# liuyuan-pal/Gen6D

Hardware: AMD Instinct MI355X
Metric: query images/sec (detect+select+3x refine), 64 ref views (higher is better)
Workload: dtype f32

## Files before the change

gen6d_amd/csrc/conv16_direct.hip:

```cpp
#include "g6d_common.h"
#include "conv16w_geom.h"
#include <type_traits>

namespace {

constexpr int C16_BM = 128, C16_BN = 128, C16_BK = 64;
constexpr int C16_STAGE = (C16_BM + C16_BN) * C16_BK * 2;
constexpr int C16_LDS = 2 * C16_STAGE;
constexpr int C16_EP_LD = 68;
constexpr unsigned C16_OOB = 0x80000000u;

struct C16Seg : c16g::Tiling {
  const char* in; char* full; char* pool;
  int H, W, DH;
  int rows;
  int ld_in, ld_full, ld_pool;
  int tw_log2, tiles_x, tile0;
  unsigned in_bytes;
  int back;
};
struct C16Params {
  C16Seg seg[4];
  int nseg, Cin, Cout, kd, D, relu, full_type, pool_type;
  const char* w; unsigned w_bytes; const float* bias;
// ... 383 lines not shown
    const int g = g0 + (r >> tw_log2), x = x0 + (r & (TW - 1));
    unsigned m = 0;
    if (g < sg.rows && x < W) {
      const int y = g % H, z = (g / H) % D;
      unsigned my = (y > 0 ? 1u : 0u) | 2u | (y < H - 1 ? 4u : 0u);
      unsigned mx = (x > 0 ? 1u : 0u) | 2u | (x < W - 1 ? 4u : 0u);
      unsigned m9 = 0;
#pragma unroll
      for (int ky = 0; ky < 3; ++ky) if (my >> ky & 1) m9 |= mx << (3 * ky);
      if (p.kd == 3) {
        if (z > 0) m |= m9;
        m |= m9 << 9;
        if (z < D - 1) m |= m9 << 18;
      } else m = m9;
    }
    a_mask[i] = m;
    a_off[i] = (unsigned)(((long)g * W + x) * sg.ld_in * 2) + slot * 16;
  }
  const __amdgpu_buffer_rsrc_t rs_in = c16_rsrc(sg.in - sg.back, sg.in_bytes);
  typedef __attribute__((address_space(3))) void* lds_ptr;
  const int nchunk = p.Cin / R::BK, nk = nchunk * ntaps;
  const int plane_bytes = p.Cin * 2;

  auto issue_a = [&](int k, int stage) {
    const int c = k / ntaps, tap = k - c * ntaps;
    const int kz = tap / 9, r9 = tap - 9 * kz, ky = r9 / 3, kx = r9 - 3 * ky;
    const unsigned a_k = (unsigned)(((kz * H + ky) * W + kx) * sg.ld_in * 2 + c * (R::BK * 2));
    char* sa = lds + stage * R::STAGE;
#pragma unroll
    for (int i = 0; i < 4; ++i) {
      const int ri = i % NR, pl = i / NR;
      const unsigned vo = (a_mask[ri] >> tap & 1u) ? a_off[ri] + a_k + pl * plane_bytes : C16_OOB;
      __builtin_amdgcn_raw_ptr_buffer_load_lds(rs_in, (lds_ptr)(sa + pl * (C16_BM * R::ROWB) + (32 * wv + R::RPI * ri) * R::ROWB), 16, vo, 0, 0, 0);
    }
  };
  const int wm = wv >> 1, wn = wv & 1;
  constexpr int NB = R::KS * R::NP * 2;
  constexpr int STEP_B = R::KS * R::NP * 4 * 1024;
  const char* wtile = p.w + (long)nt * nk * STEP_B;
  const unsigned b_voff = (2 * wn) * 1024 + lane * 16;
  auto load_b = [&](int k, V8 (&b)[NB]) {
    const char* ws = wtile + (long)k * STEP_B;
#pragma unroll
    for (int q = 0; q < R::KS * R::NP; ++q) {
      const char* wq = ws + q * 4096;
      asm volatile("global_load_dwordx4 %0, %1, %2" : "=v"(b[2 * q]) : "v"(b_voff), "s"(wq) : "memory");
      asm volatile("global_load_dwordx4 %0, %1, %2 offset:1024" : "=v"(b[2 * q + 1]) : "v"(b_voff), "s"(wq) : "memory");
    }
  };

  f32x16 acc[2][2];
#pragma unroll
  for (int a = 0; a < 2; ++a)
#pragma unroll
    for (int b = 0; b < 2; ++b)
#pragma unroll
      for (int r = 0; r < 16; ++r) acc[a][b][r] = 0.f;
  const int frow = lane & 31, fhalf = lane >> 5;
  const int fsw = R::SL == 8 ? (frow >> 1) & 7 : (frow >> 2) & 3;
  const int a_rd = (64 * wm + frow) * R::ROWB;

  auto compute = [&](int stage, const V8 (&b)[NB]) {
    const char* st = lds + stage * R::STAGE;
#pragma unroll
    for (int ks = 0; ks < R::KS; ++ks) {
      const int sl = ((2 * ks + fhalf) ^ fsw) * 16;
      V8 a[R::NP][2];
#pragma unroll
      for (int pl = 0; pl < R::NP; ++pl) {
        a[pl][0] = *reinterpret_cast<const V8*>(st + pl * (C16_BM * R::ROWB) + a_rd + sl);
        a[pl][1] = *reinterpret_cast<const V8*>(st + pl * (C16_BM * R::ROWB) + a_rd + 32 * R::ROWB + sl);
      }
#pragma unroll
      for (int mt = 0; mt < 2; ++mt)
#pragma unroll
        for (int n2 = 0; n2 < 2; ++n2) {
          acc[mt][n2] = c16_mfma<MM>(a[0][mt], b[(ks * R::NP) * 2 + n2], acc[mt][n2]);
          if constexpr (MM == 3) {
            acc[mt][n2] = c16_mfma<MM>(a[0][mt], b[(ks * R::NP + 1) * 2 + n2], acc[mt][n2]);
            acc[mt][n2] = c16_mfma<MM>(a[1][mt], b[(ks * R::NP) * 2 + n2], acc[mt][n2]);
          }
        }
    }
  };

  static_assert(NSTAGE == 3, "the stage arithmetic below assumes three stages");
  V8 b0[NB], b1[NB];
  load_b(0, b0);
  issue_a(0, 0);
  if (nk > 1) { issue_a(1, 1); asm volatile("s_waitcnt vmcnt(4)" ::: "memory"); }
  else asm volatile("s_waitcnt vmcnt(0)" ::: "memory");
  __builtin_amdgcn_s_barrier();
  __builtin_amdgcn_sched_barrier(0);
  int stage = 0;
  auto step = [&](int k, const V8 (&bc)[NB], V8 (&bn)[NB]) {
    if (k + 1 < nk && !((p.ablate & 2) && k > 1)) load_b(k + 1, bn);
    const int s2 = stage >= 1 ? stage - 1 : 2;
    if (k + 2 < nk && !((p.ablate & 1) && k > 1)) issue_a(k + 2, s2);
    compute(stage, bc);
    if (k + 2 < nk && !p.ablate) asm volatile("s_waitcnt vmcnt(4)" ::: "memory");
    else asm volatile("s_waitcnt vmcnt(0)" ::: "memory");
    asm volatile("s_waitcnt lgkmcnt(0)" ::: "memory");
    __builtin_amdgcn_s_barrier();
    __builtin_amdgcn_sched_barrier(0);
    stage = stage == 2 ? 0 : stage + 1;
  };
#pragma unroll 1
  for (int k = 0; k < nk; k += 2) {
    step(k, b0, b1);
    if (k + 1 < nk) step(k + 1, b1, b0);
  }
  c16_epilogue<MM == 3 ? 2 : MM>(p, sg, lds, tid, nt, g0, x0, tw_log2, C16_BM >> tw_log2,
                                 [&](int h, float* ep, int cbase) { c16_write22(p, acc, lane, wv, h, ep, cbase); });
}


#ifndef C16W_ABLATE
#define C16W_ABLATE 0
#endif
template <int MM> struct C16W {
  static constexpr int NP = MM == 3 ? 2 : 1, KS = 2, NI_MAX = 18;
  static constexpr int PLANE = NI_MAX * 1024;
  static constexpr int NT2 = MM == 3 ? 1 : 2;
  static constexpr int NBL = KS * NP * NT2;
  static constexpr int NPX = 64;
  static constexpr int EPW = NPX * C16_EP_LD * 4;
};

struct C16Geom {
  int si, ni;
  c16g::Tile t;
};
__device__ __forceinline__ C16Geom c16w_geom(const C16Params& p, int ptile) {
  C16Geom o;
  int si = 0;
#pragma unroll
  for (int i = 1; i < 4; ++i) if (i < p.nseg && ptile >= p.seg[i].h_tile0) si = i;
  const C16Seg& sg = p.seg[si];
  o.si = si; o.ni = (sg.h_P + 15) >> 4;
  o.t = c16g::tile_of(sg, sg.H, sg.W, ptile - sg.h_tile0);
  return o;
}

template <int BASE, int HI>
__device__ __forceinline__ void c16_wait_vm(int n) {
  if constexpr (HI == 0) {
    asm volatile("s_waitcnt vmcnt(%0)" ::"n"(BASE) : "memory");
  } else {
    if (n >= HI) asm volatile("s_waitcnt vmcnt(%0)" ::"n"(BASE + HI) : "memory");
    else c16_wait_vm<BASE, HI - 1>(n);
  }
}

template <int MM, int WM, int NT2 = C16W<MM>::NT2>
__global__ __launch_bounds__(256, 2) void conv16w_kernel(const C16Params p) {
  typedef typename C16T3<MM>::V V8;
  typedef C16W<MM> R;
  constexpr int WN = 4 / WM, NP = R::NP, KS = R::KS, NBL = KS * NP * NT2, CW = 32 * NT2;
  constexpr bool SINGLE = MM == 3 && WM == 2;
  constexpr int TILE_B = NP * R::PLANE, STAGE = WM * TILE_B;
  extern __shared__ __attribute__((aligned(16))) char lds[];
  const int tid = threadIdx.x, lane = tid & 63, wv = __builtin_amdgcn_readfirstlane(tid >> 6);
  const int xcd = blockIdx.x & 7, jj = blockIdx.x >> 3;
  const int cb = jj % p.nN, tg = (jj / p.nN) * 8 + xcd;
  if (tg * WM >= p.ptiles) return;
  const int wm = wv / WN, wn = wv % WN;
  const int nchunk = p.Cin >> 5;
  typedef __attribute__((address_space(3))) void* lds_ptr;

  constexpr int NPJ = (R::NI_MAX + 3) / 4;
  unsigned poff[WM][NPJ], pmask[WM];
  C16Geom gms[WM];
#pragma unroll
  for (int tl = 0; tl < WM; ++tl) {
    gms[tl] = c16w_geom(p, min(tg * WM + tl, p.ptiles - 1));
    const C16Geom& gm = gms[tl];
    const C16Seg& sg = p.seg[gm.si];
    const unsigned base = c16g::tile_base(sg.W, sg.ld_in, gm.t);
    unsigned pm = 0;
    if (gm.t.interior) {
#pragma unroll
      for (int j = 0; j < NPJ; ++j) {
        const c16g::Piece pc = c16g::piece_of(sg, wv + 4 * j, lane);
        poff[tl][j] = pc.in_patch ? c16g::piece_offset(sg, sg.W, sg.ld_in, base, pc) : C16_OOB;
        if (wv + 4 * j < gm.ni) pm |= 1u << j;
      }
    } else {
#pragma unroll
      for (int j = 0; j < NPJ; ++j) {
        const int ii = wv + 4 * j;
        const c16g::Piece pc = c16g::piece_of(sg, ii, lane);
        const bool ok = c16g::piece_valid(sg, sg.H, sg.W, sg.rows, gm.t, pc);
        poff[tl][j] = ok ? c16g::piece_offset(sg, sg.W, sg.ld_in, base, pc) : C16_OOB;
        if (ii < gm.ni) {
          if (__builtin_amdgcn_ballot_w64(ok) != 0) pm |= 1u << j;
          else {
            const f32x4 z = {0.f, 0.f, 0.f, 0.f};
#pragma unroll
            for (int pl = 0; pl < NP; ++pl) {
              char* dst = lds + tl * TILE_B + pl * R::PLANE + ii * 1024 + lane * 16;
              *reinterpret_cast<f32x4*>(dst) = z;
              if constexpr (!SINGLE) *reinterpret_cast<f32x4*>(dst + STAGE) = z;
            }
          }
        }
      }
    }
    pmask[tl] = __builtin_amdgcn_readfirstlane(pm);
  }
  const unsigned plane_b = (unsigned)(p.Cin * 2);
  auto issue_patch = [&](int c, int stage) {
    if (c >= nchunk) return;
    const unsigned ck = (unsigned)(c * 64);
#pragma unroll
    for (int tl = 0; tl < WM; ++tl) {
      const C16Seg& sg = p.seg[gms[tl].si];
      const __amdgpu_buffer_rsrc_t rs_in = c16_rsrc(sg.in, sg.in_bytes - sg.back);
#pragma unroll
      for (int j = 0; j < NPJ; ++j) {
        if (pmask[tl] >> j & 1) {
          const unsigned vo = poff[tl][j] == C16_OOB ? C16_OOB : poff[tl][j] + ck;
#pragma unroll
          for (int pl = 0; pl < NP; ++pl)
            __builtin_amdgcn_raw_ptr_buffer_load_lds(rs_in, (lds_ptr)(lds + stage * STAGE + tl * TILE_B + pl * R::PLANE + (wv + 4 * j) * 1024), 16,
                                                     vo + pl * plane_b, 0, 0, 0);
        }
      }
    }
  };
  const C16Geom gm = WM == 1 ? gms[0] : gms[wm ? WM - 1 : 0];
  const C16Seg& sgw = p.seg[gm.si];
  const int f_tw_log2 = sgw.h_tw_log2, f_PW = (1 << f_tw_log2) + 2;

  const int chan0 = (cb * WN + wn) * CW;
  const int nkp = (MM == 3 ? nchunk : nchunk >> 1) * 9;
  const char* wtile = p.w + (long)(chan0 >> 7) * nkp * 16384;
  unsigned bvo[KS * NP];
  if constexpr (MM == 3) {
#pragma unroll
    for (int q = 0; q < KS * NP; ++q)
      bvo[q] = ((lane >> 5) * NP + q % NP) * 4096 + ((chan0 >> 5) & 3) * 1024 + (32 * ((lane >> 4) & 1) + 16 * (q / NP) + (lane & 15)) * 16;
  } else {
#pragma unroll
    for (int q = 0; q < KS * NP; ++q) bvo[q] = q * 4096 + ((chan0 >> 5) & 3) * 1024 + lane * 16;
  }
  const char* wp = wtile;
  int wleft = nchunk * 9;
  auto load_b = [&](int c, int t, V8 (&b)[NBL]) {
    const unsigned long wa = (unsigned long)(wleft > 0 ? wp : wtile);
    const char* ws = reinterpret_cast<const char*>((unsigned long)(unsigned)__builtin_amdgcn_readfirstlane((unsigned)wa) |
                                                   ((unsigned long)(unsigned)__builtin_amdgcn_readfirstlane((unsigned)(wa >> 32)) << 32));
#pragma unroll
    for (int q = 0; q < KS * NP; ++q) {
      asm volatile("global_load_dwordx4 %0, %1, %2" : "=v"(b[NT2 * q]) : "v"(bvo[q]), "s"(ws) : "memory");
      if constexpr (NT2 == 2) asm volatile("global_load_dwordx4 %0, %1, %2 offset:1024" : "=v"(b[NT2 * q + 1]) : "v"(bvo[q]), "s"(ws) : "memory");
    }
    --wleft;
    if (t < 8 || MM == 3) wp += 16384;
    else wp += (c & 1) ? 8192 : 8192 - 8 * 16384;
  };

  if constexpr (MM == 3) {
    int qb[8], xs[3];
#pragma unroll
    for (int mt = 0; mt < 8; ++mt) qb[mt] = c16g::frag_pixel(sgw, 16 * mt + (lane & 15)) * 64 + wm * TILE_B;
#pragma unroll
    for (int kx = 0; kx < 3; ++kx) xs[kx] = ((lane >> 4) ^ ((((lane & 15 & ((1 << f_tw_log2) - 1)) + kx) >> sgw.h_swa) & 3)) << 4;
    const int PW64 = f_PW * 64;
    auto tap_off = [&](int t, int stg) { return xs[t % 3] + (stg * STAGE + (t / 3) * PW64 + (t % 3) * 64); };
    auto read_pair = [&](int mp, int off, V8 (&a)[2][NP]) {
#pragma unroll
      for (int i = 0; i < 2; ++i) {
        const int addr = qb[2 * mp + i] + off;
#pragma unroll
        for (int pl = 0; pl < NP; ++pl) a[i][pl] = *reinterpret_cast<const V8*>(lds + pl * R::PLANE + addr);
      }
    };
    f32x4 acc[8][2];
#pragma unroll
    for (int a = 0; a < 8; ++a)
#pragma unroll
      for (int b = 0; b < 2; ++b)
#pragma unroll
        for (int r = 0; r < 4; ++r) acc[a][b][r] = 0.f;
    auto mfmas = [&](int mp, const V8 (&a)[2][NP], const V8 (&b)[NBL]) {
#pragma unroll
      for (int term = 0; term < 3; ++term) {
        const int pa = term == 2 ? 1 : 0, pb = term == 1 ? 1 : 0;
#pragma unroll
        for (int n2 = 0; n2 < 2; ++n2)
#pragma unroll
          for (int i = 0; i < 2; ++i)
            acc[2 * mp + i][n2] = __builtin_amdgcn_mfma_f32_16x16x32_f16(a[i][pa], b[n2 * NP + pb], acc[2 * mp + i][n2], 0, 0, 0);
      }
    };

    V8 bs[3][NBL];
    V8 fa[3][2][NP];
    issue_patch(0, 0);
    load_b(0, 0, bs[0]);
    load_b(0, 1, bs[1]);
    asm volatile("s_waitcnt vmcnt(0) lgkmcnt(0)" ::: "memory");
    __builtin_amdgcn_s_barrier();
    __builtin_amdgcn_sched_barrier(0);
#pragma unroll
    for (int mp = 0; mp < 3; ++mp) read_pair(mp, tap_off(0, 0), fa[mp]);
    int stage = 0;
#pragma unroll 1
    for (int c = 0; c < ((C16W_ABLATE & 8) ? 0 : nchunk); ++c) {
#pragma unroll
      for (int mt = 0; mt < 8; ++mt) asm volatile("" : "+v"(qb[mt]));
#pragma unroll
      for (int kx = 0; kx < 3; ++kx) asm volatile("" : "+v"(xs[kx]));
#pragma unroll
      for (int t = 0; t < 9; ++t) {
        const int t2 = (t + 2) % 9, c2 = c + (t + 2) / 9;
        if (!((C16W_ABLATE & 2) && c > 0)) load_b(c2, t2, bs[(t + 2) % 3]);
        if (t == 0 && !SINGLE && !((C16W_ABLATE & 1) && c > 0)) issue_patch(c + 1, stage ^ 1);
        if (C16W_ABLATE) asm volatile("s_waitcnt vmcnt(0)" ::: "memory");
        else asm volatile("s_waitcnt vmcnt(%0)" ::"n"(2 * NBL) : "memory");
        __builtin_amdgcn_sched_barrier(0);
        const int off = tap_off(t, stage), noff = tap_off(t < 8 ? t + 1 : 0, stage);
#pragma unroll
        for (int mp = 0; mp < 4; ++mp) {
          const int g = 4 * t + mp, gn = g + 3;
          mfmas(mp, fa[g % 3], bs[t % 3]);
          if (gn < 36 && !((C16W_ABLATE & 4) && c > 0)) read_pair(gn % 4, gn / 4 == t ? off : noff, fa[g % 3]);
          __builtin_amdgcn_sched_barrier(0);
        }
        if (t == 8) {
          asm volatile("s_waitcnt vmcnt(0) lgkmcnt(0)" ::: "memory");
          __builtin_amdgcn_s_barrier();
          __builtin_amdgcn_sched_barrier(0);
          if constexpr (SINGLE) {
            issue_patch(c + 1, 0);
            asm volatile("s_waitcnt vmcnt(0)" ::: "memory");
            __builtin_amdgcn_s_barrier();
            __builtin_amdgcn_sched_barrier(0);
          } else stage ^= 1;
          if (c + 1 < nchunk) {
#pragma unroll
            for (int mp = 0; mp < 3; ++mp) read_pair(mp, tap_off(0, stage), fa[mp]);
          }
        }
      }
    }
    asm volatile("s_waitcnt vmcnt(0)" ::: "memory");
    __builtin_amdgcn_s_barrier();
    __builtin_amdgcn_sched_barrier(0);

    if (tg * WM + wm >= p.ptiles) return;
    const C16Seg& sg = p.seg[gm.si];
    float* ep = reinterpret_cast<float*>(lds + wv * R::EPW);
    float bv[2];
#pragma unroll
    for (int n2 = 0; n2 < 2; ++n2) bv[n2] = p.bias ? p.bias[chan0 + 16 * n2 + (lane & 15)] : 0.f;
    constexpr int MTP = R::NPX / 16;
    const float as = ldexpf(p.acc_scale, g6d_exp_in(p.rng));
    unsigned amax = 0;
    double wst[2] = {0.0, 0.0};
    const bool per_pass = c16w_stats_per_pass(p, sg, f_tw_log2);
    auto passes = [&](auto ftc, auto ptc, auto stc, auto spc) {
#pragma unroll
      for (int ps = 0; ps < 8 / MTP; ++ps) {
#pragma unroll
        for (int m = 0; m < MTP; ++m)
#pragma unroll
          for (int n2 = 0; n2 < 2; ++n2)
#pragma unroll
            for (int r = 0; r < 4; ++r) {
              const int px = 16 * m + 4 * (lane >> 4) + r;
              float v = fmaf(acc[ps * MTP + m][n2][r], as, bv[n2]);
              if (p.relu) v = fmaxf(v, 0.f);
              ep[px * C16_EP_LD + 16 * n2 + (lane & 15)] = v;
            }
        c16_epilogue_pass<2, 64, R::NPX, CW, decltype(ftc)::value, decltype(ptc)::value, decltype(stc)::value>(
            p, sg, ep, nullptr, lane, chan0, gm.t.g0, gm.t.x0, f_tw_log2, gm.t.ylim, ps * R::NPX, amax, wst);
        if (decltype(spc)::value > 0 || (decltype(spc)::value < 0 && per_pass))
          c16_stats_flush_pass<CW>(p, sg, lane, chan0, gm.t.g0 + ((ps * R::NPX) >> f_tw_log2), wst);
      }
    };
    typedef std::integral_constant<int, -1> any_;
    typedef std::integral_constant<int, 0> c0_;
    typedef std::integral_constant<int, 1> c1_;
    if (!p.stats && p.full_type == 3 && p.pool_type == 0) passes(std::integral_constant<int, 3>{}, c0_{}, c0_{}, c0_{});
    else if (!p.stats && p.full_type == 0 && p.pool_type == 3) passes(c0_{}, std::integral_constant<int, 3>{}, c0_{}, c0_{});
    else if (!p.stats && p.full_type == 3 && p.pool_type == 3) passes(std::integral_constant<int, 3>{}, std::integral_constant<int, 3>{}, c0_{}, c0_{});
    else if (p.stats && p.full_type == 2 && p.pool_type == 0 && !per_pass) passes(std::integral_constant<int, 2>{}, c0_{}, c1_{}, c0_{});
    else if (p.stats && p.full_type == 2 && p.pool_type == 0) passes(std::integral_constant<int, 2>{}, c0_{}, c1_{}, c1_{});
    else passes(any_{}, any_{}, any_{}, any_{});
    if (p.stats && !per_pass) c16_stats_flush<CW>(p, sg, lane, chan0, gm.t.g0, wst);
    g6d_range_record(p.rng, amax);
  } else {
    const int fhalf = lane >> 5;
    int qb[4], fe[4];
    const int PW64 = f_PW * 64, swa = sgw.h_swa, swd = sgw.h_swd;
#pragma unroll
    for (int mt = 0; mt < 4; ++mt) {
      const int r = 32 * mt + (lane & 31);
      qb[mt] = c16g::frag_pixel(sgw, r) * 64 + wm * TILE_B; fe[mt] = (r & ((1 << f_tw_log2) - 1)) + c16g::frag_row(sgw, r) * swd;
    }
    auto tap_addr = [&](int ky, int kx, int stage, int (&tb)[4]) {
      const int so = stage * STAGE + (ky * PW64 + kx * 64);
#pragma unroll
      for (int mt = 0; mt < 4; ++mt) {
        const int sw = ((fe[mt] + kx) >> swa) + ky * swd;
        tb[mt] = qb[mt] + so + (((fhalf ^ sw) & 3) << 4);
      }
    };
    auto frag_read = [&](int addr, V8 (&a)[NP]) {
#pragma unroll
      for (int pl = 0; pl < NP; ++pl) a[pl] = *reinterpret_cast<const V8*>(lds + pl * R::PLANE + addr);
    };
    f32x16 acc[4][NT2];
#pragma unroll
    for (int a = 0; a < 4; ++a)
#pragma unroll
      for (int b = 0; b < NT2; ++b)
#pragma unroll
        for (int r = 0; r < 16; ++r) acc[a][b][r] = 0.f;
    auto mfmas = [&](int mt, const V8 (&a)[NP], const V8 (&b)[NBL], int ks) {
#pragma unroll
      for (int n2 = 0; n2 < NT2; ++n2) acc[mt][n2] = c16_mfma<MM>(a[0], b[ks * NT2 + n2], acc[mt][n2]);
    };

    V8 bs[3][NBL];
    V8 fa[4][NP];
    int tb[4], ntb[4];
    issue_patch(0, 0);
    load_b(0, 0, bs[0]);
    load_b(0, 1, bs[1]);
    asm volatile("s_waitcnt vmcnt(0) lgkmcnt(0)" ::: "memory");
    __builtin_amdgcn_s_barrier();
    __builtin_amdgcn_sched_barrier(0);
    tap_addr(0, 0, 0, tb);
#pragma unroll
    for (int mt = 0; mt < 4; ++mt) frag_read(tb[mt], fa[mt]);
    int stage = 0;
#pragma unroll 1
    for (int c = 0; c < ((C16W_ABLATE & 8) ? 0 : nchunk); ++c) {
#pragma unroll
      for (int mt = 0; mt < 4; ++mt) asm volatile("" : "+v"(fe[mt]), "+v"(qb[mt]));
#pragma unroll
      for (int t = 0; t < 9; ++t) {
        const int t2 = (t + 2) % 9, c2 = c + (t + 2) / 9;
        if (!((C16W_ABLATE & 2) && c > 0)) load_b(c2, t2, bs[(t + 2) % 3]);
        if (t == 0 && !((C16W_ABLATE & 1) && c > 0)) issue_patch(c + 1, stage ^ 1);
        if (C16W_ABLATE) asm volatile("s_waitcnt vmcnt(0)" ::: "memory");
        else asm volatile("s_waitcnt vmcnt(%0)" ::"n"(2 * NBL) : "memory");
        __builtin_amdgcn_sched_barrier(0);
        if (t < 8) tap_addr((t + 1) / 3, (t + 1) % 3, stage, ntb);
        else tap_addr(0, 0, stage ^ 1, ntb);
#pragma unroll
        for (int mt = 0; mt < 4; ++mt) {
          mfmas(mt, fa[mt], bs[t % 3], 0);
          if (!((C16W_ABLATE & 4) && c > 0)) frag_read(tb[mt] ^ 32, fa[mt]);
          __builtin_amdgcn_sched_barrier(0);
        }
#pragma unroll
        for (int mt = 0; mt < 4; ++mt) {
          mfmas(mt, fa[mt], bs[t % 3], 1);
          if (t < 8 && !((C16W_ABLATE & 4) && c > 0)) frag_read(ntb[mt], fa[mt]);
          __builtin_amdgcn_sched_barrier(0);
        }
#pragma unroll
        for (int mt = 0; mt < 4; ++mt) tb[mt] = ntb[mt];
        if (t == 8) {
          asm volatile("s_waitcnt vmcnt(0) lgkmcnt(0)" ::: "memory");
          __builtin_amdgcn_s_barrier();
          __builtin_amdgcn_sched_barrier(0);
          stage ^= 1;
          if (c + 1 < nchunk) {
#pragma unroll
            for (int mt = 0; mt < 4; ++mt) frag_read(tb[mt], fa[mt]);
          }
        }
      }
    }
    asm volatile("s_waitcnt vmcnt(0)" ::: "memory");
    __builtin_amdgcn_s_barrier();
    __builtin_amdgcn_sched_barrier(0);

    if (tg * WM + wm >= p.ptiles) return;
    const C16Seg& sg = p.seg[gm.si];
    float* ep = reinterpret_cast<float*>(lds + wv * R::EPW);
    float bv[NT2];
#pragma unroll
    for (int n2 = 0; n2 < NT2; ++n2) bv[n2] = p.bias ? p.bias[chan0 + 32 * n2 + (lane & 31)] : 0.f;
    constexpr int MTP = R::NPX / 32;
    const float as = ldexpf(p.acc_scale, g6d_exp_in(p.rng));
    unsigned amax = 0;
    double wst[2] = {0.0, 0.0};
    const bool per_pass = c16w_stats_per_pass(p, sg, f_tw_log2);
// ... 317 lines not shown
        }
    };
    issue_patch(0, 0);
    asm volatile("s_waitcnt vmcnt(0)" ::: "memory");
    __builtin_amdgcn_s_barrier();
#pragma unroll 1
    for (int c = 0; c < nslice; ++c) {
      if (c + 1 < nslice) issue_patch(c + 1, (c + 1) & 1);
      asm volatile("s_waitcnt vmcnt(0)" ::: "memory");
      __builtin_amdgcn_s_barrier();
    }
  } else {
  const int T = K * K;
  const int ntw = (T - wv + NW - 1) / NW;
  const char* wp = p.w + (long)wv * 2048;
  int wtap = wv, wleft = nslice * ntw;
  const unsigned bvo = lane * 16;
  auto load_b = [&](V8 (&b)[2]) {
    const unsigned long wa = (unsigned long)(wleft > 0 ? wp : p.w);
    const char* ws = reinterpret_cast<const char*>((unsigned long)(unsigned)__builtin_amdgcn_readfirstlane((unsigned)wa) |
                                                   ((unsigned long)(unsigned)__builtin_amdgcn_readfirstlane((unsigned)(wa >> 32)) << 32));
    asm volatile("global_load_dwordx4 %0, %1, %2" : "=v"(b[0]) : "v"(bvo), "s"(ws) : "memory");
    asm volatile("global_load_dwordx4 %0, %1, %2 offset:1024" : "=v"(b[1]) : "v"(bvo), "s"(ws) : "memory");
    --wleft;
    wtap += NW;
    if (wtap < T) wp += NW * 2048;
    else { wp += (long)(T - wtap + NW + wv) * 2048; wtap = wv; }
  };

  const int fhalf = lane >> 5;
  int qb[4], fe[4];
#pragma unroll
  for (int mt = 0; mt < 4; ++mt) {
    const int r = 32 * mt + (lane & 31), py = r >> tw_log2, px = r & (TW - 1);
    qb[mt] = (py * PW + px) * 64; fe[mt] = px + py * swd;
  }
  const int PW64 = PW * 64;
  auto tap_addr = [&](int ky, int kx, int stage, int (&tb)[4]) {
    const int so = stage * CORR16_STAGE + ky * PW64 + kx * 64;
#pragma unroll
    for (int mt = 0; mt < 4; ++mt) {
      const int sw = ((fe[mt] + kx) >> swa) + ky * swd;
      tb[mt] = qb[mt] + so + (((fhalf ^ sw) & 3) << 4);
    }
  };
  V8 bs[3][2];
  V8 fa[4][2];
  int tb[4], ntb[4];
  load_b(bs[0]);
  load_b(bs[1]);
  asm volatile("s_waitcnt vmcnt(0)" ::: "memory");
  __builtin_amdgcn_s_barrier();
  __builtin_amdgcn_sched_barrier(0);
  const int ky0 = wv / K, kx0 = wv - ky0 * K;
  int ky = ky0, kx = kx0;
  tap_addr(ky, kx, 0, tb);
#pragma unroll
  for (int mt = 0; mt < 4; ++mt) {
    fa[mt][0] = *reinterpret_cast<const V8*>(lds + tb[mt]);
    fa[mt][1] = *reinterpret_cast<const V8*>(lds + (tb[mt] ^ 32));
  }
  int stage = 0, it = 0, c = 0;
  auto step = [&](const V8 (&bc)[2], V8 (&bfar)[2]) {
    const bool live = c < nslice, last = it == ntw - 1;
    load_b(bfar);
    asm volatile("s_waitcnt vmcnt(4)" ::: "memory");
    __builtin_amdgcn_sched_barrier(0);
    if (!live) return;
    int nky = ky, nkx = kx + NW;
    while (nkx >= K) { nkx -= K; ++nky; }
    if (last) { nky = ky0; nkx = kx0; }
    tap_addr(nky, nkx, last ? stage ^ 1 : stage, ntb);
#pragma unroll
    for (int mt = 0; mt < 4; ++mt) {
      if constexpr (MM == 3) {
        acc[mt] = c16_mfma<MM>(fa[mt][0], bc[0], acc[mt]);
        acc[mt] = c16_mfma<MM>(fa[mt][0], bc[1], acc[mt]);
        acc[mt] = c16_mfma<MM>(fa[mt][1], bc[0], acc[mt]);
      } else {
        acc[mt] = c16_mfma<MM>(fa[mt][0], bc[0], acc[mt]);
        acc[mt] = c16_mfma<MM>(fa[mt][1], bc[1], acc[mt]);
      }
      if (!last) {
        fa[mt][0] = *reinterpret_cast<const V8*>(lds + ntb[mt]);
        fa[mt][1] = *reinterpret_cast<const V8*>(lds + (ntb[mt] ^ 32));
      }
      __builtin_amdgcn_sched_barrier(0);
    }
    ky = nky; kx = nkx;
#pragma unroll
    for (int mt = 0; mt < 4; ++mt) tb[mt] = ntb[mt];
    ++it;
    if (last) {
      asm volatile("s_waitcnt lgkmcnt(0)" ::: "memory");
      __builtin_amdgcn_s_barrier();
      __builtin_amdgcn_sched_barrier(0);
      stage ^= 1; it = 0; ++c;
      if (c < nslice) {
#pragma unroll
        for (int mt = 0; mt < 4; ++mt) {
          fa[mt][0] = *reinterpret_cast<const V8*>(lds + tb[mt]);
          fa[mt][1] = *reinterpret_cast<const V8*>(lds + (tb[mt] ^ 32));
        }
      }
    }
  };
  const int nsteps = nslice * ntw;
#pragma unroll 1
  for (int s_ = 0; s_ < nsteps; s_ += 3) {
    asm volatile("" : "+v"(fe[0]), "+v"(fe[1]), "+v"(fe[2]), "+v"(fe[3]));
    step(bs[0], bs[2]);
    step(bs[1], bs[0]);
    step(bs[2], bs[1]);
  }
  asm volatile("s_waitcnt vmcnt(0)" ::: "memory");
  }
  __builtin_amdgcn_s_barrier();
  __builtin_amdgcn_sched_barrier(0);

  float* red = reinterpret_cast<float*>(lds);
  float sum[8];
#pragma unroll
  for (int e = 0; e < 8; ++e) sum[e] = 0.f;
#pragma unroll 1
  for (int rd = 0; rd < (NW + 3) / 4; ++rd) {
    if (wv < NW && (wv >> 2) == rd) {
      float* mine = red + (wv & 3) * (128 * 33);
#pragma unroll
      for (int mt = 0; mt < 4; ++mt)
#pragma unroll
        for (int r = 0; r < 16; ++r) mine[(32 * mt + (r & 3) + 8 * (r >> 2) + 4 * (lane >> 5)) * 33 + (lane & 31)] = acc[mt][r];
    }
    __syncthreads();
    if (wv < 8)
#pragma unroll
    for (int e = 0; e < 8; ++e) {
      const int o = tid + 512 * e, px = o >> 5, ch = o & 31;
      const int ns = NW - 4 * rd < 4 ? NW - 4 * rd : 4;
      for (int sl = 0; sl < ns; ++sl) sum[e] += red[sl * 128 * 33 + px * 33 + ch];
    }
    __syncthreads();
  }
  const float as = ldexpf(p.acc_scale, g6d_exp_in(p.rng));
  if (wv < 8)
#pragma unroll
  for (int e = 0; e < 8; ++e) {
    const int o = tid + 512 * e, px = o >> 5, ch = o & 31;
    const int y = y0 + (px >> tw_log2), x = x0 + (px & (TW - 1));
    if (y < sg.H && x < sg.W) sg.out[(((long)n * sg.H + y) * sg.W + x) * sg.ld_out + ch] = sum[e] * as;
  }
}


bool c16_halo_tiling(const G6dConv16Seg& s, C16Seg& o, int& tiles, bool pairs) {
  double best = 1e30;
  bool found = false;
  for (int tw = 32; tw >= 4; tw >>= 1) {
    const int th = C16_BM / tw, tx = (s.W + tw - 1) / tw;
    long nt; int tpi, segh, bands;
    if (s.H >= th) { tpi = tx * ((s.H + th - 1) / th); nt = (long)s.N * tpi; segh = th; bands = 1; }
    else {
      if (th % s.H) continue;
      tpi = 0; nt = (long)tx * (((long)s.N * s.H + th - 1) / th); segh = s.H; bands = th / s.H;
    }
    if (bands * (segh + 2) * (tw + 2) > 288) continue;
    const double waste = (double)nt * C16_BM / ((double)s.N * s.H * s.W);
    if (waste < best - 1e-9) {
      best = waste; found = true;
      int l2 = 0; while ((1 << l2) < tw) ++l2;
      int sl2 = 0; while ((1 << sl2) < segh) ++sl2;
      o.h_tw_log2 = l2; o.h_tiles_x = tx; o.h_tpi = tpi; o.h_segh_log2 = sl2; o.h_bands = bands;
      tiles = (int)nt;
      if (pairs) { o.h_swa = tw >= 16 ? 1 : 0; o.h_swd = 0; }
      else { o.h_swa = tw == 32 ? 2 : (tw == 16 ? 1 : 0); o.h_swd = tw <= 8 ? 1 : 0; }
    }
  }
  return found && c16g::finish(o, tiles);
}

int c16_pick_tw(int W, int pool) {
  int best = 8; double bw = 1e9;
  for (int tw = 64; tw >= (pool ? 4 : 4); tw >>= 1) {
    const double waste = (double)((W + tw - 1) / tw * tw) / W;
    if (waste < bw - 1e-9) { bw = waste; best = tw; }
  }
  return best;
}

}

namespace {
int c16_direct(const G6dConv16Seg* segs, int nseg, int Cin, const void* W16, int w_layout, float acc_scale, const float* bias, int Cout, int kd, int relu,
               int full_type, int pool_type, int math_mode, double* stats, int stat_rows_per_group, const G6dRange16* range, g6d_stream_t stream,
               bool plan_only) {
  if (!segs || nseg < 1 || nseg > 4 || !W16) { g6d_set_error("conv16_direct: 1..4 segments and filters expected"); return G6D_EINVAL; }
  if (math_mode < 1 || math_mode > 3 || (w_layout != 0 && w_layout != 1) || (math_mode == 3 && w_layout != 1)) {
    g6d_set_error("conv16_direct: math_mode 1 (bf16) / 2 (fp16) / 3 (fp16 hi-lo pairs, fragment-major filters only)"); return G6D_EINVAL;
  }
  const int bk = math_mode == 3 ? 32 : C16_BK, planes = math_mode == 3 ? 2 : 1;
  const bool half_tile = Cout == 64 && w_layout == 1 && kd == 1;
  if (Cin % bk || (Cout % C16_BN && !half_tile) || (kd != 1 && kd != 3)) { g6d_set_error("conv16_direct: Cin % 64 (32 for pairs), Cout % 128 (64: fragment-major 2-D layers), kd in {1,3} expected"); return G6D_EINVAL; }
  const int t16 = math_mode == 3 ? 3 : 1;
  auto type_ok = [&](int t) { return t == 0 || t == 2 || t == t16; };
  if (!type_ok(full_type) || !type_ok(pool_type) || (!full_type && !pool_type && !stats)) { g6d_set_error("conv16_direct: output types"); return G6D_EINVAL; }
  if (pool_type && kd != 1) { g6d_set_error("conv16_direct: pooling is 2-D only"); return G6D_EINVAL; }
  C16Params p = {};
  p.nseg = nseg; p.Cin = Cin; p.Cout = Cout; p.kd = kd; p.relu = relu; p.full_type = full_type; p.pool_type = pool_type;
  p.w = static_cast<const char*>(W16); p.bias = bias; p.stats = stats; p.stat_rows_per_group = stat_rows_per_group;
  p.acc_scale = acc_scale != 0.f ? acc_scale : 1.f;
  p.ablate = (int)g6d_knob(G6D_KNOB_C16_ABLATE);
  if (range) p.rng = *range;
  const long wb = (long)(half_tile ? 128 : Cout) * 9 * kd * Cin * 2 * planes;
  if (wb >= (1L << 31)) { g6d_set_error("conv16_direct: filters beyond 2 GB"); return G6D_EINVAL; }
  p.w_bytes = (unsigned)wb;
  p.nN = Cout / C16_BN;
  int tiles = 0, D0 = segs[0].D;
  bool pertap_stats_ok = true;
  for (int i = 0; i < nseg; ++i) {
    const G6dConv16Seg& s = segs[i];
    C16Seg& o = p.seg[i];
    if (!s.in || s.N < 1 || s.D < 1 || s.H < 1 || s.W < 1 || s.ld_in < planes * Cin || s.D != D0 || (kd == 1 && s.D != 1)) { g6d_set_error("conv16_direct: bad segment"); return G6D_EINVAL; }
    const int need_full = full_type == 3 ? 2 * Cout : Cout, need_pool = pool_type == 3 ? 2 * Cout : Cout;
    if ((full_type && (!s.out_full || s.ld_full < need_full)) || (pool_type && (!s.out_pool || s.ld_pool < need_pool || (s.H & 1) || (s.W & 1)))) {
      g6d_set_error("conv16_direct: outputs missing / odd map with pooling"); return G6D_EINVAL;
    }
    if (!g6d_aligned16(s.in) || (s.ld_in & 7) || (full_type && (!g6d_aligned16(s.out_full) || (s.ld_full & 7))) || (pool_type && (!g6d_aligned16(s.out_pool) || (s.ld_pool & 7)))) {
      g6d_set_error("conv16_direct: 16-byte aligned rows expected"); return G6D_EINVAL;
    }
    if (32L * s.W * (s.ld_full > s.ld_pool ? s.ld_full : s.ld_pool) * 4 >= (1L << 32)) { g6d_set_error("conv16_direct: 32 output rows beyond 4 GB"); return G6D_EINVAL; }
    o.in = static_cast<const char*>(s.in); o.full = static_cast<char*>(s.out_full); o.pool = static_cast<char*>(s.out_pool);
    o.H = s.H; o.W = s.W; o.DH = s.D * s.H; o.rows = s.N * s.D * s.H;
    o.ld_in = s.ld_in; o.ld_full = s.ld_full; o.ld_pool = s.ld_pool;
    const int tw = c16_pick_tw(s.W, pool_type != 0);
    int l2 = 0; while ((1 << l2) < tw) ++l2;
    o.tw_log2 = l2; o.tiles_x = (s.W + tw - 1) / tw; o.tile0 = tiles;
    const int th = C16_BM / tw;
    if (stats && stat_rows_per_group > 0 && ((long)stat_rows_per_group % ((long)th * s.W) != 0)) pertap_stats_ok = false;
    tiles += o.tiles_x * ((o.rows + th - 1) / th);
    const long back = ((long)(kd == 3 ? s.H * s.W : 0) + s.W + 1) * s.ld_in * 2;
    const long ext = (long)o.rows * s.W * s.ld_in * 2 + back;
    if (ext >= (1L << 31)) { g6d_set_error("conv16_direct: a segment's input beyond 2 GB"); return G6D_EINVAL; }
    o.back = (int)back; o.in_bytes = (unsigned)ext;
  }
  p.D = D0;
  p.ptiles = tiles;
  hipStream_t st = static_cast<hipStream_t>(stream);
  if (w_layout == 1 && kd == 1 && g6d_knob(G6D_KNOB_CONV16_HALO) != 0) {
    bool ok = true, per_pass = false;
    int htiles = 0;
    for (int i = 0; i < nseg && ok; ++i) {
      int nt_ = 0;
      ok = c16_halo_tiling(segs[i], p.seg[i], nt_, math_mode == 3);
      p.seg[i].h_tile0 = htiles; htiles += nt_;
      if (stats && stat_rows_per_group > 0 && ok) {
        const C16Seg& o = p.seg[i];
        const int th = C16_BM >> o.h_tw_log2;
        const long tile_px = (long)th * segs[i].W, pass_px = (long)(C16W<3>::NPX >> o.h_tw_log2) * segs[i].W;
        static_assert(C16W<1>::NPX == C16W<3>::NPX && C16W<2>::NPX == C16W<3>::NPX, "one pass size in every mode");
        ok = (stat_rows_per_group % (segs[i].H * segs[i].W) == 0) &&
             (o.h_tpi > 0 || stat_rows_per_group % tile_px == 0 || (stat_rows_per_group < tile_px && stat_rows_per_group % pass_px == 0));
        per_pass = per_pass || (ok && stat_rows_per_group < tile_px);
      }
    }
    if (!ok && half_tile) { g6d_set_error("conv16_direct: Cout = 64 needs a halo tiling for every segment"); return G6D_EINVAL; }
    if (ok) {
      const int cw = half_tile ? 32 : 32 * (math_mode == 3 ? C16W<3>::NT2 : C16W<2>::NT2);
      const int wm = Cout % (4 * cw) == 0 ? 1 : 2;
      p.ptiles = htiles;
      p.nN = Cout / (cw * (4 / wm));
      if (plan_only) return per_pass ? 2 : 1;
      const int hblocks = ((htiles + wm - 1) / wm + 7) / 8 * 8 * p.nN;
      auto launch = [&](auto kern, int main_lds, int ep_lds) {
        const int bytes = main_lds > ep_lds ? main_lds : ep_lds;
        g6d_allow_lds(reinterpret_cast<const void*>(kern), bytes);
        hipLaunchKernelGGL(kern, dim3(hblocks), dim3(256), bytes, st, p);
      };
#define C16W_LAUNCH(MM_, WM_) launch(&conv16w_kernel<MM_, WM_>, ((MM_ == 3 && WM_ == 2) ? 1 : 2) * WM_ * C16W<MM_>::NP * C16W<MM_>::PLANE, 4 * C16W<MM_>::EPW)
      if (half_tile && math_mode != 3) {
        if (math_mode == 1) launch(&conv16w_kernel<1, 2, 1>, 2 * 2 * C16W<1>::PLANE, 4 * C16W<1>::EPW);
        else launch(&conv16w_kernel<2, 2, 1>, 2 * 2 * C16W<2>::PLANE, 4 * C16W<2>::EPW);
      }
      else if (math_mode == 1) { if (wm == 1) C16W_LAUNCH(1, 1); else C16W_LAUNCH(1, 2); }
      else if (math_mode == 2) { if (wm == 1) C16W_LAUNCH(2, 1); else C16W_LAUNCH(2, 2); }
      else { if (wm == 1) C16W_LAUNCH(3, 1); else C16W_LAUNCH(3, 2); }
#undef C16W_LAUNCH
      return g6d_check_launch("conv16w_direct");
    }
  }
  if (half_tile) { g6d_set_error("conv16_direct: Cout = 64 runs on the halo-patch kernel only (knob conv16_halo, tile shapes)"); return G6D_EINVAL; }
  if (!pertap_stats_ok) { g6d_set_error("conv16_direct: statistics groups must be whole tile rows (small maps: whole 64-pixel epilogue passes)"); return G6D_EINVAL; }
  if (plan_only) return 0;
  const int blocks = (tiles + 7) / 8 * 8 * p.nN;
  if (w_layout == 0) {
    if (math_mode == 1) {
      g6d_allow_lds(reinterpret_cast<const void*>(&conv16_kernel<1>), C16_LDS);
      hipLaunchKernelGGL(conv16_kernel<1>, dim3(blocks), dim3(256), C16_LDS, st, p);
    } else {
      g6d_allow_lds(reinterpret_cast<const void*>(&conv16_kernel<2>), C16_LDS);
      hipLaunchKernelGGL(conv16_kernel<2>, dim3(blocks), dim3(256), C16_LDS, st, p);
    }
    return g6d_check_launch("conv16_direct");
  }
  constexpr int NST = 3, LDSR = NST * 16384;
  if (math_mode == 1) {
    g6d_allow_lds(reinterpret_cast<const void*>(&conv16r_kernel<1, NST>), LDSR);
    hipLaunchKernelGGL((conv16r_kernel<1, NST>), dim3(blocks), dim3(256), LDSR, st, p);
  } else if (math_mode == 2) {
    g6d_allow_lds(reinterpret_cast<const void*>(&conv16r_kernel<2, NST>), LDSR);
    hipLaunchKernelGGL((conv16r_kernel<2, NST>), dim3(blocks), dim3(256), LDSR, st, p);
  } else {
    g6d_allow_lds(reinterpret_cast<const void*>(&conv16r_kernel<3, NST>), LDSR);
    hipLaunchKernelGGL((conv16r_kernel<3, NST>), dim3(blocks), dim3(256), LDSR, st, p);
  }
  return g6d_check_launch("conv16r_direct");
}
}

extern "C" int g6d_conv16_direct_multi_ex(const G6dConv16Seg* segs, int nseg, int Cin, const void* W16, int w_layout, float acc_scale,
                                          const float* bias, int Cout, int kd, int relu, int full_type, int pool_type, int math_mode, double* stats,
                                          int stat_rows_per_group, const G6dRange16* range, g6d_stream_t stream) {
  return c16_direct(segs, nseg, Cin, W16, w_layout, acc_scale, bias, Cout, kd, relu, full_type, pool_type, math_mode, stats, stat_rows_per_group, range,
                    stream, false);
}

extern "C" int g6d_conv16_direct_plan(const G6dConv16Seg* segs, int nseg, int Cin, const void* W16, int w_layout, int Cout, int kd, int full_type,
                                      int pool_type, int math_mode, double* stats, int stat_rows_per_group) {
  return c16_direct(segs, nseg, Cin, W16, w_layout, 1.f, nullptr, Cout, kd, 0, full_type, pool_type, math_mode, stats, stat_rows_per_group, nullptr,
                    nullptr, true);
}

extern "C" int g6d_conv16_direct_multi(const G6dConv16Seg* segs, int nseg, int Cin, const void* W16, int w_layout, float acc_scale,
                                       const float* bias, int Cout, int kd, int relu, int full_type, int pool_type, int math_mode, double* stats,
                                       int stat_rows_per_group, g6d_stream_t stream) {
  return g6d_conv16_direct_multi_ex(segs, nseg, Cin, W16, w_layout, acc_scale, bias, Cout, kd, relu, full_type, pool_type, math_mode, stats,
                                    stat_rows_per_group, nullptr, stream);
}

extern "C" int g6d_corr16_multi_ex(const G6dConv16Seg* segs, int nseg, int Cin, const void* W16, float acc_scale, int Cout, int k, int math_mode,
                                   const G6dRange16* range, g6d_stream_t stream) {
  if (!segs || nseg < 1 || nseg > 4 || !W16) { g6d_set_error("corr16: 1..4 segments and filters expected"); return G6D_EINVAL; }
  if (math_mode < 1 || math_mode > 3 || Cout != 32 || (k != 15 && k != 7) || Cin % 32) {
    g6d_set_error("corr16: math_mode 1 (bf16) / 2 (fp16) / 3 (fp16 pairs), Cout = 32, k in {7, 15}, Cin % 32 == 0 expected"); return G6D_EINVAL;
  }
  const int planes = math_mode == 3 ? 2 : 1;
  Corr16Params p = {};
  p.nseg = nseg; p.Cin = Cin; p.K = k; p.w = static_cast<const char*>(W16); p.acc_scale = acc_scale != 0.f ? acc_scale : 1.f;
  p.nslice = Cin / (math_mode == 3 ? 16 : 32);
  if (range) p.rng = *range;
  int tiles = 0;
  for (int i = 0; i < nseg; ++i) {
    const G6dConv16Seg& s = segs[i];
    Corr16Seg& o = p.seg[i];
    if (!s.in || !s.out_full || s.N < 1 || s.D != 1 || s.H < 1 || s.W < 1 || s.ld_in < planes * Cin || s.ld_full < Cout || (s.ld_in & 7) ||
        !g6d_aligned16(s.in) || !g6d_aligned16(s.out_full)) { g6d_set_error("corr16: bad segment"); return G6D_EINVAL; }
    double best = 1e30; int btw = 0;
    for (int tw = 32; tw >= 4; tw >>= 1) {
      const int th = C16_BM / tw;
      if ((th + k - 1) * (tw + k - 1) > CORR16_STAGE / 64) continue;
      const double waste = (double)((s.W + tw - 1) / tw * tw) * ((s.H + th - 1) / th * th) / ((double)s.W * s.H);
      if (waste < best - 1e-9) { best = waste; btw = tw; }
    }
    if (!btw) { g6d_set_error("corr16: no tile shape fits"); return G6D_EINVAL; }
    int l2 = 0; while ((1 << l2) < btw) ++l2;
    const int th = C16_BM / btw;
    o.in = static_cast<const char*>(s.in); o.out = static_cast<float*>(s.out_full);
    o.H = s.H; o.W = s.W; o.rows = s.N * s.H; o.ld_in = s.ld_in; o.ld_out = s.ld_full;
    o.tw_log2 = l2; o.tiles_x = (s.W + btw - 1) / btw; o.tpi = o.tiles_x * ((s.H + th - 1) / th); o.tile0 = tiles;
    o.swa = btw == 32 ? 2 : (btw == 16 ? 1 : 0); o.swd = btw <= 8 ? 1 : 0;
    const long ext = (long)s.N * s.H * s.W * s.ld_in * 2;
    if (ext >= (1L << 31)) { g6d_set_error("corr16: a segment's input beyond 2 GB"); return G6D_EINVAL; }
    o.in_bytes = (unsigned)ext;
    tiles += s.N * o.tpi;
  }
  p.ptiles = tiles;
  hipStream_t st = static_cast<hipStream_t>(stream);
  constexpr int LDSB = 2 * CORR16_STAGE;
  if (math_mode == 1) {
    g6d_allow_lds(reinterpret_cast<const void*>(&corr16_kernel<1>), LDSB);
    hipLaunchKernelGGL(corr16_kernel<1>, dim3(tiles), dim3(64 * (CORR16_NW + 1)), LDSB, st, p);
  } else if (math_mode == 2) {
    g6d_allow_lds(reinterpret_cast<const void*>(&corr16_kernel<2>), LDSB);
    hipLaunchKernelGGL(corr16_kernel<2>, dim3(tiles), dim3(64 * (CORR16_NW + 1)), LDSB, st, p);
  } else {
    g6d_allow_lds(reinterpret_cast<const void*>(&corr16_kernel<3>), LDSB);
    hipLaunchKernelGGL(corr16_kernel<3>, dim3(tiles), dim3(64 * (CORR16_NW + 1)), LDSB, st, p);
  }
  return g6d_check_launch("corr16");
}

extern "C" int g6d_corr16_multi(const G6dConv16Seg* segs, int nseg, int Cin, const void* W16, float acc_scale, int Cout, int k, int math_mode,
                                g6d_stream_t stream) {
  return g6d_corr16_multi_ex(segs, nseg, Cin, W16, acc_scale, Cout, k, math_mode, nullptr, stream);
}

extern "C" int g6d_product_split16_ex(const float* ref, const float* que, const float* scale, const float* shift, void* out, int qn, int D, int P,
                                      int C, int math_mode, const G6dRange16* range, g6d_stream_t stream) {
  if (!ref || !que || !scale || !shift || !out || qn < 1 || D < 1 || P < 1 || C < 8 || (C & 7) || math_mode < 1 || math_mode > 3 ||
      !g6d_aligned16(ref) || !g6d_aligned16(que) || !g6d_aligned16(scale) || !g6d_aligned16(shift) || !g6d_aligned16(out)) {
    g6d_set_error("product_split16: bad args (C % 8 == 0, 16-byte aligned pointers, math_mode 1..3)"); return G6D_EINVAL;
  }
  const long total = (long)qn * ((D + 7) / 8) * P * (C >> 3);
  const int blocks = (int)((total + 255) / 256 < 256 * 64 ? (total + 255) / 256 : 256 * 64);
  hipStream_t st = static_cast<hipStream_t>(stream);
  char* o = static_cast<char*>(out);
  const G6dRange16 rng = range ? *range : G6dRange16{};
  if (math_mode == 1) hipLaunchKernelGGL(product_split_kernel<1>, dim3(blocks), dim3(256), 0, st, ref, que, scale, shift, o, D, P, C, total, rng);
  else if (math_mode == 2) hipLaunchKernelGGL(product_split_kernel<2>, dim3(blocks), dim3(256), 0, st, ref, que, scale, shift, o, D, P, C, total, rng);
  else hipLaunchKernelGGL(product_split_kernel<3>, dim3(blocks), dim3(256), 0, st, ref, que, scale, shift, o, D, P, C, total, rng);
  return g6d_check_launch("product_split16");
}

extern "C" int g6d_product_split16(const float* ref, const float* que, const float* scale, const float* shift, void* out, int qn, int D, int P, int C,
                                   int math_mode, g6d_stream_t stream) {
  return g6d_product_split16_ex(ref, que, scale, shift, out, qn, D, P, C, math_mode, nullptr, stream);
}

namespace {
char* c16_slice_out(void* out, int C, int ld_out, int plane, int c_off, int math_mode) {
  const bool pairs = math_mode == 3;
  if (!out || !g6d_aligned16(out) || ((ld_out | plane | c_off) & 7) || c_off < 0 || ld_out < 1) return nullptr;
  if (pairs ? (plane < c_off + C || (long)plane + c_off + C > ld_out) : (c_off + C > ld_out)) return nullptr;
  return static_cast<char*>(out) + (long)c_off * 2;
}
}

extern "C" int g6d_affine_split16_to(const float* in, int ld_in, const float* scale, const float* shift, int affine_per_n, int relu, int pool, int N, int H,
                                     int W, int C, void* out, int ld_out, int plane, int c_off, int math_mode, const G6dRange16* range,
                                     g6d_stream_t stream) {
  if (!in || !out || N < 1 || H < 1 || W < 1 || C < 8 || (C & 7) || ld_in < C || (ld_in & 3) || (scale && !shift) || affine_per_n < 0 || math_mode < 1 ||
      math_mode > 3 || (pool && ((H | W) & 1)) || !g6d_aligned16(in) || !g6d_aligned16(out) || (scale && (!g6d_aligned16(scale) || !g6d_aligned16(shift)))) {
    g6d_set_error("affine_split16: bad args (C % 8 == 0, 16-byte aligned rows, even map with pooling, math_mode 1..3)"); return G6D_EINVAL;
  }
  char* o = c16_slice_out(out, C, ld_out, plane, c_off, math_mode);
  if (!o) { g6d_set_error("affine_split16: the channel slice does not fit the output rows (multiples of 8, c_off + C <= plane, plane + c_off + C <= ld_out)"); return G6D_EINVAL; }
  const long total = (long)N * (pool ? H / 2 : H) * (pool ? W / 2 : W) * (C >> 3);
  const int blocks = (int)((total + 255) / 256 < 256 * 64 ? (total + 255) / 256 : 256 * 64);
  hipStream_t st = static_cast<hipStream_t>(stream);
  const G6dRange16 rng = range ? *range : G6dRange16{};
  if (math_mode == 1) hipLaunchKernelGGL(affine_split16_kernel<1>, dim3(blocks), dim3(256), 0, st, in, ld_in, scale, shift, affine_per_n, relu, pool, H, W, C, o, ld_out, plane, total, rng);
  else if (math_mode == 2) hipLaunchKernelGGL(affine_split16_kernel<2>, dim3(blocks), dim3(256), 0, st, in, ld_in, scale, shift, affine_per_n, relu, pool, H, W, C, o, ld_out, plane, total, rng);
  else hipLaunchKernelGGL(affine_split16_kernel<3>, dim3(blocks), dim3(256), 0, st, in, ld_in, scale, shift, affine_per_n, relu, pool, H, W, C, o, ld_out, plane, total, rng);
// ... 50 lines not shown
```

gen6d_amd/csrc/conv16w_geom.h:

```cpp
#pragma once

#if defined(__HIPCC__)
#define C16G_HD __host__ __device__ __forceinline__
#else
#define C16G_HD inline
#endif

namespace c16g {

constexpr int BM = 128;
constexpr int NI_MAX = 18;

C16G_HD unsigned mulhi(unsigned a, unsigned b) {
#if defined(__HIP_DEVICE_COMPILE__)
  return __umulhi(a, b);
#else
  return (unsigned)(((unsigned long long)a * b) >> 32);
#endif
}

C16G_HD unsigned recip31(unsigned d) { return (unsigned)(((1ull << 31) + d - 1) / d); }
C16G_HD bool recip31_ok(unsigned d, unsigned n_max) {
  const unsigned long long e = (unsigned long long)recip31(d) * d - (1ull << 31);
  return n_max < (1u << 31) && (unsigned long long)n_max * e < (1ull << 31);
}
C16G_HD unsigned div31(unsigned n, unsigned m) { return mulhi(n << 1, m); }

C16G_HD unsigned recip16(unsigned d) { return (65536u + d - 1) / d; }
C16G_HD unsigned div16(unsigned n, unsigned m) { return (n * m) >> 16; }

struct Tiling {
  int h_tw_log2, h_tiles_x, h_tile0, h_tpi;
  int h_segh_log2, h_bands;
  int h_swa, h_swd;
  int h_P;
  unsigned h_r_tpi, h_r_tx;
  unsigned h_r_pw, h_r_band;
};

C16G_HD bool finish(Tiling& t, long ntiles) {
  const int TW = 1 << t.h_tw_log2, segh = 1 << t.h_segh_log2;
  t.h_P = t.h_bands * (segh + 2) * (TW + 2);
  t.h_r_pw = recip16((unsigned)(TW + 2)); t.h_r_band = recip16((unsigned)(segh + 2));
  t.h_r_tx = recip31((unsigned)t.h_tiles_x); t.h_r_tpi = t.h_tpi > 0 ? recip31((unsigned)t.h_tpi) : 0u;
  if (ntiles >= (1L << 31)) return false;
  return recip31_ok((unsigned)t.h_tiles_x, (unsigned)ntiles) && (t.h_tpi <= 0 || recip31_ok((unsigned)t.h_tpi, (unsigned)ntiles));
}

struct Tile {
  int g0, x0, y0, ylim;
  int interior;
};
C16G_HD Tile tile_of(const Tiling& tl, int H, int W, int t) {
  Tile o;
  const int TW = 1 << tl.h_tw_log2, TH = BM >> tl.h_tw_log2;
  if (tl.h_tpi > 0) {
    const int n = (int)div31((unsigned)t, tl.h_r_tpi), r = t - n * tl.h_tpi;
    const int ty = (int)div31((unsigned)r, tl.h_r_tx), tx = r - ty * tl.h_tiles_x;
    o.y0 = ty * TH; o.x0 = tx * TW; o.g0 = n * H + o.y0; o.ylim = TH < H - o.y0 ? TH : H - o.y0;
    o.interior = o.y0 >= 1 && o.y0 + TH < H && o.x0 >= 1 && o.x0 + TW < W;
  } else {
    const int ty = (int)div31((unsigned)t, tl.h_r_tx), tx = t - ty * tl.h_tiles_x;
    o.y0 = 0; o.x0 = tx * TW; o.g0 = ty * TH; o.ylim = TH;
    o.interior = 0;
  }
  return o;
}

struct Piece {
  int prow, pcol, band, lr, slot;
  int in_patch;
};
C16G_HD Piece piece_of(const Tiling& tl, int ii, int lane) {
  Piece o;
  const int PW = (1 << tl.h_tw_log2) + 2, bandr = (1 << tl.h_segh_log2) + 2;
  const int q = ii * 16 + (lane >> 2);
  o.prow = (int)div16((unsigned)q, tl.h_r_pw); o.pcol = q - o.prow * PW;
  o.band = (int)div16((unsigned)o.prow, tl.h_r_band); o.lr = o.prow - o.band * bandr - 1;
  o.slot = (lane & 3) ^ (((o.pcol >> tl.h_swa) + o.prow * tl.h_swd) & 3);
  o.in_patch = q < tl.h_P;
  return o;
}
C16G_HD bool piece_valid(const Tiling& tl, int H, int W, int rows, const Tile& t, const Piece& pc) {
  const int g = t.g0 + (pc.band << tl.h_segh_log2) + pc.lr, x = t.x0 + pc.pcol - 1, yimg = t.y0 + pc.lr;
  return pc.in_patch && yimg >= 0 && yimg < H && g < rows && x >= 0 && x < W;
}
C16G_HD unsigned tile_base(int W, int ld_in, const Tile& t) { return (unsigned)(((t.g0 - 1) * W + t.x0 - 1) * ld_in * 2); }
C16G_HD unsigned piece_offset(const Tiling& tl, int W, int ld_in, unsigned base, const Piece& pc) {
  const int yrel = (pc.band << tl.h_segh_log2) + pc.lr + 1;
  return base + (unsigned)((yrel * W + pc.pcol) * ld_in * 2 + pc.slot * 16);
}
C16G_HD int frag_pixel(const Tiling& tl, int r) {
  const int PW = (1 << tl.h_tw_log2) + 2, bandr = (1 << tl.h_segh_log2) + 2;
  const int py = r >> tl.h_tw_log2, px = r & ((1 << tl.h_tw_log2) - 1);
  const int b = py >> tl.h_segh_log2, ly = py & ((1 << tl.h_segh_log2) - 1);
  return (b * bandr + ly) * PW + px;
}
C16G_HD int frag_row(const Tiling& tl, int r) {
  const int py = r >> tl.h_tw_log2;
  return (py >> tl.h_segh_log2) * ((1 << tl.h_segh_log2) + 2) + (py & ((1 << tl.h_segh_log2) - 1));
}

}
```

gen6d_amd/csrc/refiner_volume.hip:

```cpp
#include "g6d_common.h"

#define MAX_RFN 8

namespace {


struct Taps { int o00, o01, o10, o11; float w00, w01, w10, w11; };

__device__ __forceinline__ Taps project_view(int fh, int fw, int C, const float (&P)[12], float vx, float vy,
                                             float vz, float h_in, float w_in) {
  float X = vx * P[0] + vy * P[1] + vz * P[2] + P[3];
  float Y = vx * P[4] + vy * P[5] + vz * P[6] + P[7];
  float Z = vx * P[8] + vy * P[9] + vz * P[10] + P[11];
  if (Z < 1e-4f) Z = 1e-4f;
  float u = X / Z, v = Y / Z;
  float gx = ((u + 0.5f) / w_in - 0.5f) * 2.f;
  float gy = ((v + 0.5f) / h_in - 0.5f) * 2.f;
  float ix = ((gx + 1.f) * fw - 1.f) * 0.5f;
  float iy = ((gy + 1.f) * fh - 1.f) * 0.5f;
  float fx = floorf(ix), fy = floorf(iy);
  fx = fminf(fmaxf(fx, -4.f), (float)fw + 4.f);
  fy = fminf(fmaxf(fy, -4.f), (float)fh + 4.f);
  int x0 = (int)fx, y0 = (int)fy;
  float wx1 = ix - fx, wy1 = iy - fy, wx0 = (fx + 1.f) - ix, wy0 = (fy + 1.f) - iy;
  const bool xv0 = (unsigned)x0 < (unsigned)fw, xv1 = (unsigned)(x0 + 1) < (unsigned)fw;
  const bool yv0 = (unsigned)y0 < (unsigned)fh, yv1 = (unsigned)(y0 + 1) < (unsigned)fh;
  const int xc0 = min(max(x0, 0), fw - 1), xc1 = min(max(x0 + 1, 0), fw - 1);
  const int yc0 = min(max(y0, 0), fh - 1), yc1 = min(max(y0 + 1, 0), fh - 1);
  Taps t;
  t.o00 = (yc0 * fw + xc0) * C; t.o01 = (yc0 * fw + xc1) * C;
  t.o10 = (yc1 * fw + xc0) * C; t.o11 = (yc1 * fw + xc1) * C;
  t.w00 = (yv0 && xv0) ? wx0 * wy0 : 0.f; t.w01 = (yv0 && xv1) ? wx1 * wy0 : 0.f;
  t.w10 = (yv1 && xv0) ? wx0 * wy1 : 0.f; t.w11 = (yv1 && xv1) ? wx1 * wy1 : 0.f;
  return t;
}

__device__ __forceinline__ Taps taps_from(const Taps& t, int src) {
  Taps r;
  r.o00 = __shfl(t.o00, src, 32); r.o01 = __shfl(t.o01, src, 32);
  r.o10 = __shfl(t.o10, src, 32); r.o11 = __shfl(t.o11, src, 32);
  r.w00 = __shfl(t.w00, src, 32); r.w01 = __shfl(t.w01, src, 32);
  r.w10 = __shfl(t.w10, src, 32); r.w11 = __shfl(t.w11, src, 32);
  return r;
}

__device__ __forceinline__ f32x4 gather_view(const float* __restrict__ fmap_c, const Taps& t) {
  const f32x4 v00 = *reinterpret_cast<const f32x4*>(fmap_c + t.o00);
  const f32x4 v01 = *reinterpret_cast<const f32x4*>(fmap_c + t.o01);
  const f32x4 v10 = *reinterpret_cast<const f32x4*>(fmap_c + t.o10);
  const f32x4 v11 = *reinterpret_cast<const f32x4*>(fmap_c + t.o11);
  f32x4 acc = t.w00 * v00;
  acc += t.w01 * v01;
  acc += t.w10 * v10;
  acc += t.w11 * v11;
  return acc;
}

struct VolViews { const float* projs; const float* ref_Ks; const float* ref_poses; const float* K_in; const float* pose_in;
                  const float* rot; int rot_ld; };

__global__ void __launch_bounds__(256, 4) refiner_volume_kernel(const float* __restrict__ feats, const VolViews vw,
                                                             const float* __restrict__ lin, int rfn, int fh, int fw,
                                                             int C, float h_in, float w_in, int sn,
                                                             float* __restrict__ mean_in, float* __restrict__ stdv) {
  const int bq = blockIdx.y;
  const float* __restrict__ rot = vw.rot + bq * 12;
  const int rl = vw.rot_ld;
  const int nvox = sn * sn * sn;
  feats += (size_t)bq * (rfn + 1) * fh * fw * C;
  mean_in += (size_t)bq * nvox * 2 * C; stdv += (size_t)bq * nvox * C;
  int half = (blockIdx.x * blockDim.x + threadIdx.x) >> 5;
  const int l32 = threadIdx.x & 31;
  const bool live = half < nvox;
  if (!live) half = nvox - 1;
  const int k = half % sn, j = (half / sn) % sn, i = half / (sn * sn);
  const float g0 = lin[i], g1 = lin[j], g2 = lin[k];
  const float vx = g0 * rot[0] + g1 * rot[rl] + g2 * rot[2 * rl];
  const float vy = g0 * rot[1] + g1 * rot[rl + 1] + g2 * rot[2 * rl + 1];
  const float vz = g0 * rot[2] + g1 * rot[rl + 2] + g2 * rot[2 * rl + 2];
  const size_t fsz = (size_t)fh * fw * C;
  const float inv_n = 1.f / (float)rfn, inv_n1 = 1.f / (float)(rfn > 1 ? rfn - 1 : 1);
  const int myview = l32 <= rfn ? l32 : rfn;
  float P[12];
  if (vw.projs) {
#pragma unroll
    for (int e = 0; e < 12; ++e) P[e] = vw.projs[myview * 12 + e];
  } else {
    const float* K = myview < rfn ? vw.ref_Ks + (bq * rfn + myview) * 9 : vw.K_in + bq * 9;
    const float* T = myview < rfn ? vw.ref_poses + (bq * rfn + myview) * 12 : vw.pose_in + bq * 12;
#pragma unroll
    for (int r = 0; r < 3; ++r)
#pragma unroll
      for (int c = 0; c < 4; ++c) P[r * 4 + c] = K[r * 3] * T[c] + K[r * 3 + 1] * T[4 + c] + K[r * 3 + 2] * T[8 + c];
  }
  const Taps mine = project_view(fh, fw, C, P, vx, vy, vz, h_in, w_in);
  for (int c0 = 0; c0 < C; c0 += 128) {
    const int c_mine = c0 + l32 * 4;
    const bool c_in = c_mine < C;
    const int c = c_in ? c_mine : C - 4;
    f32x4 s[MAX_RFN];
    f32x4 sum = {0.f, 0.f, 0.f, 0.f};
#pragma unroll
    for (int r = 0; r < MAX_RFN; ++r)
      if (r < rfn) { s[r] = gather_view(feats + r * fsz + c, taps_from(mine, r)); sum += s[r]; }
    const f32x4 mean = sum * inv_n;
    f32x4 var = {0.f, 0.f, 0.f, 0.f};
#pragma unroll
    for (int r = 0; r < MAX_RFN; ++r)
      if (r < rfn) { f32x4 d = s[r] - mean; var += d * d; }
    var = var * inv_n1;
    f32x4 sd = {sqrtf(var[0]), sqrtf(var[1]), sqrtf(var[2]), sqrtf(var[3])};
    const f32x4 q = gather_view(feats + rfn * fsz + c, taps_from(mine, rfn));
    if (!live || !c_in) continue;
    *reinterpret_cast<f32x4*>(mean_in + (size_t)half * 2 * C + c) = mean;
    *reinterpret_cast<f32x4*>(mean_in + (size_t)half * 2 * C + C + c) = q;
    *reinterpret_cast<f32x4*>(stdv + (size_t)half * C + c) = sd;
  }
}

}

extern "C" int g6d_refiner_volume(const float* feats, const float* projs, const float* rot_in,
                                  const float* lin, int rfn, int fh, int fw, int C, int h_in, int w_in, int sn,
                                  float* mean_in, float* stdv, g6d_stream_t stream) {
  if (!feats || !projs || !rot_in || !lin || !mean_in || !stdv || rfn < 1 || rfn > MAX_RFN || C < 4 || (C & 3) ||
      fh <= 0 || fw <= 0 || h_in <= 0 || w_in <= 0 || sn < 1 || sn > 256 || !g6d_aligned16(feats) || !g6d_aligned16(mean_in) ||
      !g6d_aligned16(stdv)) {
    g6d_set_error("refiner_volume: bad args (1 <= rfn <= 8, C a positive multiple of 4, positive map and image sizes)"); return G6D_EINVAL;
  }
  const long long threads = (long long)sn * sn * sn * 32;
  const VolViews vw = {projs, nullptr, nullptr, nullptr, nullptr, rot_in, 3};
  hipLaunchKernelGGL(refiner_volume_kernel, dim3((unsigned)((threads + 255) / 256)), dim3(256), 0,
                     reinterpret_cast<hipStream_t>(stream), feats, vw, lin, rfn, fh, fw, C, (float)h_in, (float)w_in, sn,
                     mean_in, stdv);
  return g6d_check_launch("refiner_volume");
}

extern "C" int g6d_refiner_volume_kp(const float* feats, const float* ref_Ks, const float* ref_poses, const float* K_in,
                                     const float* pose_in, const float* lin, int rfn, int fh, int fw, int C, int h_in, int w_in, int sn,
                                     float* mean_in, float* stdv, int batch, g6d_stream_t stream) {
  if (!feats || !ref_Ks || !ref_poses || !K_in || !pose_in || !lin || !mean_in || !stdv || rfn < 1 || rfn > MAX_RFN || C < 4 || (C & 3) ||
      fh <= 0 || fw <= 0 || h_in <= 0 || w_in <= 0 || sn < 1 || sn > 256 || batch < 1 || batch > 65535 || !g6d_aligned16(feats) ||
      !g6d_aligned16(mean_in) || !g6d_aligned16(stdv)) {
    g6d_set_error("refiner_volume_kp: bad args (1 <= rfn <= 8, C a positive multiple of 4, positive map and image sizes)"); return G6D_EINVAL;
  }
  const long long threads = (long long)sn * sn * sn * 32;
  const VolViews vw = {nullptr, ref_Ks, ref_poses, K_in, pose_in, pose_in, 4};
  hipLaunchKernelGGL(refiner_volume_kernel, dim3((unsigned)((threads + 255) / 256), batch), dim3(256), 0,
                     reinterpret_cast<hipStream_t>(stream), feats, vw, lin, rfn, fh, fw, C, (float)h_in, (float)w_in, sn,
                     mean_in, stdv);
  return g6d_check_launch("refiner_volume_kp");
}
```

gen6d_amd/lib.py:

```python
import ctypes as C
import os

_HERE = os.path.dirname(os.path.abspath(__file__))
LIB_PATH = os.path.join(_HERE, "libgen6d_hip.so")

G6D_ERRORS = {-1: "G6D_EINVAL", -2: "G6D_ENOSPC", -3: "G6D_ELAUNCH"}


class G6dWinoSeg(C.Structure):
    _fields_ = [("in_", C.c_void_p), ("out_full", C.c_void_p), ("out_pool", C.c_void_p),
                ("N", C.c_int32), ("H", C.c_int32), ("W", C.c_int32), ("ld_in", C.c_int32), ("ld_full", C.c_int32), ("ld_pool", C.c_int32)]


class G6dConv16Seg(C.Structure):
    _fields_ = [("in_", C.c_void_p), ("out_full", C.c_void_p), ("out_pool", C.c_void_p),
                ("N", C.c_int32), ("D", C.c_int32), ("H", C.c_int32), ("W", C.c_int32), ("ld_in", C.c_int32), ("ld_full", C.c_int32),
                ("ld_pool", C.c_int32)]


class G6dRange16(C.Structure):
    _fields_ = [("exps", C.c_void_p), ("rec", C.c_void_p), ("slot_in", C.c_int32), ("slot_out", C.c_int32)]


class G6dCorrSeg(C.Structure):
    _fields_ = [("in_", C.c_void_p), ("out", C.c_void_p), ("H", C.c_int32), ("W", C.c_int32), ("ld_in", C.c_int32), ("ld_out", C.c_int32),
                ("N", C.c_int32), ("reserved_", C.c_int32)]


class G6dFrame(C.Structure):
    _fields_ = [("plane0", C.c_void_p), ("plane1", C.c_void_p), ("pitch0", C.c_int32), ("pitch1", C.c_int32), ("width", C.c_int32),
                ("height", C.c_int32), ("format", C.c_int32), ("rotate", C.c_int32), ("matrix", C.c_int32), ("slot", C.c_int32),
                ("out_w", C.c_int32), ("out_h", C.c_int32), ("K", C.c_float * 9)]


class G6dMesh(C.Structure):
    _fields_ = [("nodes", C.c_void_p), ("nx", C.c_int32), ("ny", C.c_int32), ("step_log2", C.c_int32), ("reserved", C.c_int32)]


class G6dSink(C.Structure):
    _fields_ = [("plane0", C.c_void_p), ("plane1", C.c_void_p), ("pitch0", C.c_int32), ("pitch1", C.c_int32), ("width", C.c_int32),
                ("height", C.c_int32), ("format", C.c_int32), ("matrix", C.c_int32), ("slot", C.c_int32), ("pic_w", C.c_int32),
                ("pic_h", C.c_int32), ("thickness", C.c_int32), ("dot_radius", C.c_int32), ("line_rgb", C.c_int32), ("dot_rgb", C.c_int32),
                ("box", C.c_int32)]


class G6dConv(C.Structure):
    _fields_ = [
        ("in_", C.c_void_p), ("mul", C.c_void_p), ("in_scale", C.c_void_p), ("in_shift", C.c_void_p),
        ("weight", C.c_void_p), ("bias", C.c_void_p), ("out", C.c_void_p), ("stats", C.c_void_p),
        ("workspace", C.c_void_p), ("workspace_bytes", C.c_size_t),
        ("N", C.c_int32), ("Di", C.c_int32), ("Hi", C.c_int32), ("Wi", C.c_int32), ("Cin", C.c_int32), ("ld_in", C.c_int32),
        ("Do", C.c_int32), ("Ho", C.c_int32), ("Wo", C.c_int32), ("Cout", C.c_int32), ("ld_out", C.c_int32),
        ("kd", C.c_int32), ("kh", C.c_int32), ("kw", C.c_int32),
        ("sd", C.c_int32), ("sh", C.c_int32), ("sw", C.c_int32),
        ("pd", C.c_int32), ("ph", C.c_int32), ("pw", C.c_int32),
        ("in_relu", C.c_int32), ("in_affine_per_n", C.c_int32), ("out_act", C.c_int32),
        ("stat_rows_per_group", C.c_int32), ("split_k", C.c_int32), ("math_mode", C.c_int32),
        ("weight_wino", C.c_void_p),
        ("fin_scale", C.c_void_p), ("fin_shift", C.c_void_p), ("fin_counter", C.c_void_p),
        ("fin_count", C.c_double), ("fin_eps", C.c_double), ("fin_groups", C.c_int32),
        ("in_image_mod", C.c_int32), ("mul_group_images", C.c_int32), ("reserved_", C.c_int32),
        ("weight_wino16", C.c_void_p), ("weight_wino43", C.c_void_p),
    ]


_P, _I, _F, _D = C.c_void_p, C.c_int, C.c_float, C.c_double

SIGNATURES = {
    "g6d_marker": [_I, _P],
    "g6d_conv_igemm": [C.POINTER(G6dConv), _P],
    "g6d_conv_plan": [C.POINTER(G6dConv)],
    "g6d_corr2d_patch": [_P, _I, _I, _I, _I, _P, _I, _I, _I, _P, _I, _P, C.c_size_t, _I, _P],
    "g6d_corr2d_patch_multi": [_P, _I, _I, _P, _I, _I, _I, _P, C.c_size_t, _I, _P],
    "g6d_corr2d_wino_multi": [_P, _I, _I, _P, _I, _I, _P, C.c_size_t, _P],
    "g6d_corr2d_patch16_multi": [_P, _I, _I, _P, _I, _I, _I, _P, C.c_size_t, _I, _P],
    "g6d_stats_finalize": [_P, _I, _D, _D, _P, _P, _P],
    "g6d_affine_act_pool": [_P, _I, _P, _P, _I, _I, _I, _I, _I, _I, _I, _P, _I, _P],
    "g6d_upsample_bilinear": [_P, _I, _P, _P, _I, _I, _I, _I, _I, _I, _P, _I, _P],
    "g6d_bias_relu_pool_nchw": [_P, _P, _I, _I, _I, _I, _I, _I, _P, _P],
    "g6d_vgg_conv1_pool": [_P, _I, _I, _I, _P, _P, _I, _I, _P, _P],
    "g6d_vgg_conv1_pool_nhwc": [_P, _I, _I, _I, _P, _P, _I, _I, _P, _P],
    "g6d_vgg_conv1_pool_nhwc16": [_P, _I, _I, _I, _P, _P, _I, _I, _P, _P, _P, _I, _P],
    "g6d_conv16_direct_multi": [_P, _I, _I, _P, _I, _F, _P, _I, _I, _I, _I, _I, _I, _P, _I, _P],
    "g6d_corr16_multi": [_P, _I, _I, _P, _F, _I, _I, _I, _P],
    "g6d_product_split16": [_P, _P, _P, _P, _P, _I, _I, _I, _I, _I, _P],
    "g6d_affine_split16": [_P, _I, _P, _P, _I, _I, _I, _I, _I, _I, _I, _P, _I, _P],
    "g6d_vgg_conv1_pool_nhwc16_ex": [_P, _I, _I, _I, _P, _P, _I, _I, _P, _P, _P, _I, _P, _P],
    "g6d_conv16_direct_multi_ex": [_P, _I, _I, _P, _I, _F, _P, _I, _I, _I, _I, _I, _I, _P, _I, _P, _P],
    "g6d_corr16_multi_ex": [_P, _I, _I, _P, _F, _I, _I, _I, _P, _P],
    "g6d_product_split16_ex": [_P, _P, _P, _P, _P, _I, _I, _I, _I, _I, _P, _P],
    "g6d_affine_split16_ex": [_P, _I, _P, _P, _I, _I, _I, _I, _I, _I, _I, _P, _I, _P, _P],
    "g6d_conv16_direct_plan": [_P, _I, _I, _P, _I, _I, _I, _I, _I, _I, _P, _I],
    "g6d_affine_split16_to": [_P, _I, _P, _P, _I, _I, _I, _I, _I, _I, _I, _P, _I, _I, _I, _I, _P, _P],
    "g6d_upsample_bilinear_split16": [_P, _I, _P, _P, _I, _I, _I, _I, _I, _I, _P, _I, _I, _I, _I, _P, _P],
    "g6d_l2norm_split16": [_P, _I, _I, _I, _P, _I, _P, _P],
    "g6d_vgg_conv1_pool_nhwc_norm": [_P, _I, _I, _I, _P, _P, _I, _I, _P, _P, _P, _P],
    "g6d_wino_conv3x3": [_P, _I, _I, _I, _I, _I, _P, _P, _I, _I, _P, _I, _P, _I, _P, C.c_size_t, _P],
    "g6d_wino_conv3x3_multi": [_P, _I, _I, _P, _P, _I, _I, _P, C.c_size_t, _P],
    "g6d_wino16_conv3x3_multi": [_P, _I, _I, _P, _P, _I, _I, _I, _P, C.c_size_t, _P],
    "g6d_wino43_conv3x3_multi": [_P, _I, _I, _P, _P, _I, _I, _P, C.c_size_t, _P],
    "g6d_corr2d_wino43_multi": [_P, _I, _I, _P, _I, _I, _P, C.c_size_t, _P],
    "g6d_l2norm_rows": [_P, _I, _I, _I, _P],
    "g6d_nchw_to_nhwc": [_P, _I, _I, _I, _I, _I, _P, _I, _P],
    "g6d_selector_ref_sums": [_P, _I, _I, _I, _P, _P, _P],
    "g6d_selector_prod_affine": [_P, _P, _P, _I, _I, _I, _D, _P, _P, _P],
    "g6d_selector_scan": [_P, _P, _I, _I, _I, _P, _P, _P],
    "g6d_selector_levels": [_I, _I, _P, _P, _P, _P, _P, _I, _I, _I, _D, _P, _P, _P, _P, _P],
    "g6d_refiner_volume": [_P, _P, _P, _P, _I, _I, _I, _I, _I, _I, _I, _P, _P, _P],
    "g6d_refiner_volume_kp": [_P, _P, _P, _P, _P, _P, _I, _I, _I, _I, _I, _I, _I, _P, _P, _I, _P],
    "g6d_detector_assemble": [_P, _P, _P, _I, _I, _I, C.POINTER(C.c_float), _F, _I, _I, _I, _I, _P, _I, _P],
    "g6d_detector_score_mlp_max": [_P, _I, _I, _I, _P, _P, _P, _P, _P, _P],
    "g6d_detector_decode": [_P, _I, _P, _I, _P, _I, _I, _I, _I, _P, _I, _P],
    "g6d_resize_bilinear_pyramid": [_P, _I, _I, _I, _I, C.POINTER(C.c_int), C.POINTER(C.c_int), C.POINTER(C.c_void_p), _P],
    "g6d_zero_bytes": [_P, C.c_size_t, _P],
    "g6d_vps_norm": [_P, _I, _P, _I, _I, _I, _P],
    "g6d_max_an_add": [_P, _I, _I, _I, _I, _P, _P, _I, _I, _P],
    "g6d_attention": [_P, _P, _P, _I, _I, _I, _I, _P, _I, _I, _P],
    "g6d_layernorm": [_P, _I, _I, _I, _P, _P, _F, _P, _I, _P],
    "g6d_affine_act_add": [_P, _I, _P, _P, _I, _P, _I, _I, _I, _P, _I, _I, _P],
    "g6d_linear_gemv": [_P, _I, _I, _P, _P, _I, _I, _P, _P],
    "g6d_linear_gemv_batch": [_P, _I, _I, _P, _P, _I, _I, _P, _P, C.c_size_t, _P],
    "g6d_chain_crop_from_detection": [_P, _F, _P, _I, _P],
    "g6d_chain_pose_from_selection": [_P, _P, _P, _I, _P, _P, _P, _P, _P, _P, _I, _P],
    "g6d_chain_refine_prepare": [_P, _P, _P, _F, _F, _P, _P, _I, _I, _P, _P, _F, _P, _I, _P],
    "g6d_chain_refine_update": [_P, _P, _P, _P, _I, _P, _P, _I, _P],
    "g6d_warp_batch": [_P, _P, _P, _I, _I, _I, _I, _P, _P, _I, _I, _P],
    "g6d_warp_perspective": [_P, _I, _I, _I, C.POINTER(C.c_float), _P, _I, _I, _I, _F, _P],
    "g6d_track_gather": [_P, _P, _P, _P, _I, _P],
    "g6d_track_commit": [_P, _P, _P, _I, _P, _I, _F, _P, _P, _P, _P, _P, _I, _P],
    "g6d_track_gate": [_P, _P, _P, _P, _I, _P],
    "g6d_track_health": [_P, _P, _P, _P, _I, _I, _P, _I, _P, _D, _I, _D, _D, _D, _D, _D, _D, _P, _P, _P, _P, _I, _P],
    "g6d_track_verify": [_P, _P, _P, _P, _P, _D, _D, _D, _D, _I, _P, _P, _I, _P],
    "g6d_frame_ingest": [_P, _I, _P, _I, _I, _I, _P, _P],
    "g6d_sizeof_frame_desc": [],
    "g6d_frame_ingest_mesh": [_P, _P, _I, _P, _I, _I, _I, _P, _P],
    "g6d_sizeof_mesh_desc": [],
    "g6d_track_corners": [_P, _P, _P, _P, _P, _P, _I, _P],
    "g6d_frame_emit": [_P, _I, _P, _I, _I, _I, _P, _P, _P],
    "g6d_sizeof_sink_desc": [],
    "g6d_frame_emit_source": [_P, _I, _P, _I, _P, _P, _I, _I, _I, _I, _P],
}

_lib = None


def load():
    global _lib
    if _lib is not None:
        return _lib
    if not os.path.exists(LIB_PATH):
        raise RuntimeError(f"{LIB_PATH} is missing: build it with `python __graft_entry__.py` "
                           "(make -C gen6d_amd/csrc). There is no fallback path.")
    import torch
    lib = C.CDLL(LIB_PATH)
    for name, args in SIGNATURES.items():
        fn = getattr(lib, name)
        fn.argtypes = args
        fn.restype = C.c_int
    lib.g6d_abi_version.restype = C.c_int
    lib.g6d_sizeof_conv_desc.restype = C.c_int
    if lib.g6d_sizeof_conv_desc() != C.sizeof(G6dConv):
        raise RuntimeError("libgen6d_hip.so: G6dConv layout differs from the ctypes binding (stale build?)")
    if lib.g6d_sizeof_frame_desc() != C.sizeof(G6dFrame):
        raise RuntimeError("libgen6d_hip.so: G6dFrame layout differs from the ctypes binding (stale build?)")
    if lib.g6d_sizeof_mesh_desc() != C.sizeof(G6dMesh):
        raise RuntimeError("libgen6d_hip.so: G6dMesh layout differs from the ctypes binding (stale build?)")
    if lib.g6d_sizeof_sink_desc() != C.sizeof(G6dSink):
        raise RuntimeError("libgen6d_hip.so: G6dSink layout differs from the ctypes binding (stale build?)")
    lib.g6d_last_error.restype = C.c_char_p
    lib.g6d_set_knob.argtypes, lib.g6d_set_knob.restype = [C.c_char_p, C.c_double], C.c_int
    lib.g6d_get_knob.argtypes, lib.g6d_get_knob.restype = [C.c_char_p], C.c_double
    lib.g6d_reset_knobs.argtypes, lib.g6d_reset_knobs.restype = [], None
    _lib = lib
    return lib


def set_knob(name, value):
    check(load().g6d_set_knob(name.encode(), float(value)), f"g6d_set_knob({name})")


def get_knob(name):
    return load().g6d_get_knob(name.encode())


def reset_knobs():
    load().g6d_reset_knobs()


def check(rc, what):
    if rc != 0:
        msg = load().g6d_last_error().decode()
        raise RuntimeError(f"{what} failed: {G6D_ERRORS.get(rc, rc)} ({msg})")
```

gen6d_amd/network/params.py:

```python
import torch
import torch.nn as nn

from .. import ops, specs


class ConvW(tuple):

    def __new__(cls, w, b, u=None, u43=None):
        t = super().__new__(cls, (w, b))
        t.u, t.u43, t._w16 = u, u43, {}
        return t

    def w16(self, mode):
        if mode not in self._w16:
            self._w16[mode] = ops.conv16_pack(self[0], mode, layout=1)
        return self._w16[mode]


class ParamBank(nn.Module):
    def __init__(self, rows):
        super().__init__()
        self._roles = {}
        for key, shape, role in specs.expand(rows):
            *path, leaf = key.split(".")
            mod = self
            for name in path:
                if name not in mod._modules:
                    mod.add_module(name, nn.Module())
                mod = mod._modules[name]
            if role in ("weight", "bias", "gamma", "beta"):
                init = torch.ones(shape) if role == "gamma" else torch.zeros(shape)
                mod.register_parameter(leaf, nn.Parameter(init, requires_grad=False))
            elif role == "count":
                mod.register_buffer(leaf, torch.zeros((), dtype=torch.long))
            else:
                mod.register_buffer(leaf, torch.ones(shape) if role == "rvar" else torch.zeros(shape))
            self._roles[key] = role
        self._packed = None

    sharded = False

    def _reset_derived(self):
        self._packed = None
        self.__dict__.pop("_range_seen", None)
        t = self.__dict__.get("_range")
        if t is not None:
            t.reset()

    def load_state_dict(self, *a, **k):
        self._reset_derived()
        return super().load_state_dict(*a, **k)

    def _apply(self, fn, *a, **k):
        self._reset_derived()
        return super()._apply(fn, *a, **k)

    @property
    def pairs_on(self):
        return not (self.cfg.get("fp32_cores") or self.__dict__.get("_pairs_off", False))

    @property
    def range_fallbacks(self):
        return self.__dict__.get("_range_fallbacks", 0)

    def range_table(self):
        t = self.__dict__.get("_range")
        if t is None or t.device != self.device_():
            t = self._range = ops.RangeTable(self.device_())
        return t

    def _pair_rng(self):
        return self.range_table() if (self.pairs_on and not ops.MATH_MODE and self.device_().type == "cuda") else None

    def range_check(self):
        t = self.__dict__.get("_range")
        if t is None or not t.names:
            return False
        a = t.read()
        t.clear()
        self._range_seen = {n: max(v, self.__dict__.get("_range_seen", {}).get(n, 0.0)) if v == v else v for n, v in a.items()}
        bad = {n: v for n, v in a.items() if ops.pair_out_of_window(v, t.e[t.names[n]])}
        if not bad:
            return False
        if self.sharded:
            raise RuntimeError(f"{type(self).__name__}: fp16 pair maps left the representable window in the reference-sharded mode "
                               f"({', '.join(f'{n}: max |v| = {v:g}' for n, v in bad.items())}); a per-rank fp32 recompute would desynchronise "
                               "the collectives")
        t.set_exponents({n: ops.pair_exponent(v, t.e[t.names[n]]) for n, v in bad.items()})
        self._range_fallbacks = self.range_fallbacks + 1
        return True

    def range_guarded(self, fn):
        return range_guarded((self,), fn)

    def _range_fallback(self):
        """Hook: drop state derived from a call whose pair maps left the window (before its recompute)."""

    def range_report(self):
        t = self.__dict__.get("_range")
        if t is None:
            return {}
        seen = self.__dict__.get("_range_seen", {})
        return {n: {"A": seen.get(n, 0.0), "e": t.e[i]} for n, i in t.names.items()}

    def p(self, key):
        *path, leaf = key.split(".")
        mod = self
        for name in path:
            mod = mod._modules[name]
        t = mod._parameters.get(leaf)
        return (t if t is not None else mod._buffers[leaf]).detach()

    def device_(self):
        return next(self.parameters()).device

    def conv_w(self, prefix, cin_pad=None, wino_kd=0, f43=False):
        w = self.p(prefix + ".weight")
        co, ci = w.shape[:2]
        w = w.reshape(co, ci, -1).permute(0, 2, 1)
        if cin_pad is not None and cin_pad != ci:
            w = torch.nn.functional.pad(w, (0, cin_pad - ci))
        w = w.contiguous()
        u = u43 = None
        if wino_kd and ci % 8 == 0 and co % 32 == 0 and w.shape[1] == 9 * wino_kd:
            from .backbone import winograd_filters_taps, winograd43_filters_taps
            u = winograd_filters_taps(w, wino_kd)
            if f43 and co % 64 == 0:
                u43 = winograd43_filters_taps(w, wino_kd)
        return ConvW(w, self.p(prefix + ".bias").contiguous(), u, u43)


def fold_vgg(bank, prefix):
    out = []
    for i in specs.VGG11_BN_CONVS:
        w, b = bank.p(f"{prefix}.{i}.weight"), bank.p(f"{prefix}.{i}.bias")
        g, beta = bank.p(f"{prefix}.{i + 1}.weight"), bank.p(f"{prefix}.{i + 1}.bias")
        mu, var = bank.p(f"{prefix}.{i + 1}.running_mean"), bank.p(f"{prefix}.{i + 1}.running_var")
        s = g / torch.sqrt(var + 1e-5)
        out.append(((w * s.view(-1, 1, 1, 1)).contiguous(), ((b - mu) * s + beta).contiguous()))
    return out


def range_guarded(nets, fn, recompute=None):
    nets = [n for n in nets if n is not None]
    for n in nets:
        t = n.__dict__.get("_range")
        if t is not None and t.names:
            t.clear()
    out = fn()
    left = [n for n in nets if n.range_check()]
    if left:
        for n in left:
            n._range_fallback()
            n._pairs_off = True
        try:
            out = (recompute or fn)()
        finally:
            for n in left:
                n._pairs_off = False
    return out
```

gen6d_amd/network/refiner.py:

```python
import numpy as np
import torch
import torch.nn.functional as F

from .. import ops, specs
from .backbone import pack_trunk, trunk_features
from .operator import pose_apply_th
from .params import ParamBank, fold_vgg

F43_MIN_QUERIES = 4
FEATNET_F43_LAYERS = {("conv1", 0), ("conv_out", 0), ("conv_out", 3)}
FEATNET_PAIR_BRANCHES = ("conv0", "conv1", "conv2", "conv_out")
VOLUME_F43_LAYERS = ("conv0",)
MAX_BATCH = 32
_K3, _P3 = (3, 3, 3), (1, 1, 1)
_K2, _P2 = (1, 3, 3), (0, 1, 1)


_LIN = {}


def _linspace(sn, dev):
    key = (sn, str(dev))
    if key not in _LIN:
        _LIN[key] = torch.linspace(-1, 1, sn, dtype=torch.float32, device=dev)
    return _LIN[key]


class RefFeatureCache:

    def __init__(self, max_entries=2048):
        from collections import OrderedDict
        self.store, self.max_entries = OrderedDict(), max_entries
        self.hits = self.misses = 0

    def get(self, key):
        f = self.store.get(key)
        if f is None:
            self.misses += 1
            return None
        self.store.move_to_end(key)
        self.hits += 1
        return f

    def put(self, key, feat):
        self.store[key] = feat
        while len(self.store) > self.max_entries:
            self.store.popitem(last=False)

    def clear(self):
        self.store.clear()
        self.hits = self.misses = 0

    @property
    def hit_rate(self):
        return self.hits / max(1, self.hits + self.misses)


class VolumeRefiner(ParamBank):
    default_cfg = {"refiner_sample_num": 32, "ref_feat_cache_deg": 0.0, "lowp_keep_fp32": (), "lowp_only": None}

    def __init__(self, cfg):
        self.cfg = {**self.default_cfg, **cfg}
        super().__init__(specs.refiner_rows())
        self.ref_database = None
        self.ref_ids = None
        self.feat_cache = RefFeatureCache()

    def load_state_dict(self, *a, **k):
        self.feat_cache.clear()
        return super().load_state_dict(*a, **k)

    def _mm(self, *names):
        only = self.cfg.get("lowp_only")
        keep = self.cfg.get("lowp_keep_fp32") or ()
        fp32 = (not any(n in only for n in names)) if only is not None else any(n in keep for n in names)
        return ops.math_mode("fp32" if fp32 else None, inherit_if_none=True)

    def angle_step(self):
        return float(np.radians(self.cfg.get("ref_feat_cache_deg") or 0.0))

    def cached_ref_feats(self, keys, make_imgs):
        with ops.math_mode(self.cfg.get("math_mode"), inherit_if_none=True):
            keys = [(k, ops.MATH_MODE) for k in keys]
            got = [self.feat_cache.get(k) for k in keys]
            miss = [i for i, f in enumerate(got) if f is None]
            feats = self.run_feature_net(make_imgs(miss), f43=False) if miss else None
        if miss:
            for j, i in enumerate(miss):
                got[i] = feats[j].clone()
                self.feat_cache.put(keys[i], got[i])
        return torch.stack(got, 0)

    def _pack(self):
        if self._packed is None:
            pk = {"vgg": pack_trunk(fold_vgg(self, "feature_net.backbone.features"))}
            for name in ("conv0", "conv1", "conv2", "conv_out"):
                pk[name] = [self.conv_w(f"feature_net.{name}.{i}", wino_kd=1, f43=(name, i) in FEATNET_F43_LAYERS) for i in (0, 3)]
            for name in ("mean_embed", "var_embed", "conv5"):
                pk["v_" + name] = [self.conv_w(f"volume_net.{name}.{i}", wino_kd=0 if name == "conv5" else 3, f43=True) for i in (0, 3)]
            for name in ("conv0", "conv1", "conv2", "conv3", "conv4"):
                pk["v_" + name] = self.conv_w(f"volume_net.{name}.0", wino_kd=3 if name in ("conv0", "conv2", "conv4") else 0,
                                              f43=name in VOLUME_F43_LAYERS)
            w = self.p("regressor.fc.0.0.weight")
            pk["fc0"] = (w.reshape(512, 512, 64).permute(0, 2, 1).reshape(512, 32768).contiguous(),
                         self.p("regressor.fc.0.0.bias").contiguous())
            pk["fc1"] = (self.p("regressor.fc.1.0.weight").contiguous(), self.p("regressor.fc.1.0.bias").contiguous())
            heads = ("fcr", "fct", "fcs")
            pk["heads"] = (torch.cat([self.p(f"regressor.{h}.weight") for h in heads], 0).contiguous(),
                           torch.cat([self.p(f"regressor.{h}.bias") for h in heads], 0).contiguous())
            self._packed = pk
        return self._packed

    def run_feature_net(self, imgs, f43=None):
        pk = self._pack()
        n, _, h, w = imgs.shape
        dev = imgs.device
        big = (n >= F43_MIN_QUERIES * 7) if f43 is None else bool(f43)
        rng = self._pair_rng()
        on16 = self._featnet_pair_branches(n, h, w) if (big and rng is not None) else ()
        with self._mm("trunk"):
            f3, f5, f7 = trunk_features(pk["vgg"], imgs, ("c3", "c5", "c7_pre"), False, f43=big, rng=rng, pairs=self.pairs_on)

        def tap(name, f, slot):
            if name in on16:
                return ops.l2norm_split16(f[:, 0], 3, rng=(rng, rng.slot(slot)))
            ops.l2norm_rows(f)
            return f

        def pair(name, x):
            if name in on16:
                return pair16(name, x)
            (w0, b0), (w1, b1) = pk[name]
            u0, u1 = pk[name][0].u, pk[name][1].u
            v0, v1 = (pk[name][0].u43, pk[name][1].u43) if big else (None, None)
            _, _, hh, ww, _ = x.shape
            y0 = torch.empty((n, 1, hh, ww, w0.shape[0]), dtype=torch.float32, device=dev)
            s0 = ops.new_stats(n, w0.shape[0], dev)
            y1 = torch.empty((n, 1, hh, ww, w1.shape[0]), dtype=torch.float32, device=dev)
            s1 = ops.new_stats(n, w1.shape[0], dev)
            sc0, sh0 = ops.conv(x, w0, b0, y0, ksize=_K2, pad=_P2, stats=s0, rows_per_group=hh * ww, w_wino=u0, w_wino43=v0, finalize=hh * ww)
            sc1, sh1 = ops.conv(y0, w1, b1, y1, ksize=_K2, pad=_P2, in_scale=sc0, in_shift=sh0, in_relu=True, per_n=True,
                                stats=s1, rows_per_group=hh * ww, w_wino=u1, w_wino43=v1, finalize=hh * ww)
            return y1, sc1, sh1

        def pair16(name, x):
            _, hh, ww, _, _ = x.shape

            def conv16(layer, xin):
                co = layer[0].shape[0]
                y = torch.empty((n, 1, hh, ww, co), dtype=torch.float32, device=dev)
                st = ops.new_stats(n, co, dev)
                ops.conv16_direct_multi([xin], layer.w16(3), layer[1], relu=False, full=torch.float32, stats=st, rows_per_group=hh * ww,
                                        out_full=[y[:, 0]])
                return (y,) + ops.stats_finalize(st, hh * ww)

            y0, sc0, sh0 = conv16(pk[name][0], x)
            mid = ops.affine_split16(y0, sc0, sh0, 1, True, False, 3, rng=(rng, rng.slot(f"featnet.{name}.mid")))
            return conv16(pk[name][1], mid)

        hq, wq = h // 4, w // 4
        cat16 = "conv_out" in on16
        cat = ops.new_map16(n, hq, wq, 192, 3, dev, rng=(rng, rng.slot("featnet.cat"))) if cat16 else \
            torch.empty((n, 1, hq, wq, 192), dtype=torch.float32, device=dev)

        def branch(name, f, slot, c_off, factor):
            y, sc, sh = pair(name, tap(name, f, slot))
            if cat16:
                if factor == 1:
                    ops.affine_split16_to(y, sc, sh, 1, False, 3, cat, c_off)
                else:
                    ops.upsample_bilinear_split16(y, cat, c_off, factor, sc, sh, 1, 3)
            elif factor == 1:
                ops.affine_act_pool(y, cat[..., c_off:c_off + 64], sc, sh, per_n=True)
            else:
                ops.upsample_bilinear(y, cat[..., c_off:c_off + 64], factor, sc, sh, per_n=True)

        with self._mm("featnet"):
            ops.fork_join([lambda: branch("conv0", f3, "featnet.f3", 0, 1), lambda: branch("conv1", f5, "featnet.f5", 64, 2),
                           lambda: branch("conv2", f7, "featnet.f7", 128, 4)], dev)
            y, sc, sh = pair("conv_out", cat)
        out = torch.empty((n, 1, hq, wq, 128), dtype=torch.float32, device=dev)
        ops.affine_act_pool(y, out, sc, sh, per_n=True)
        return out.view(n, hq, wq, 128)

    def _featnet_pair_branches(self, n, h, w):
        key = (n, h, w)
        memo = self.__dict__.setdefault("_featnet16", {})
        if key not in memo:
            shapes = {"conv0": (4, 256, 64, 64), "conv1": (8, 512, 256, 64), "conv2": (16, 512, 256, 64), "conv_out": (4, 192, 128, 128)}

            def fits(name):
                d, ci, cm, co = shapes[name]
                hh, ww = h // d, w // d
                return all(ops.conv16_direct_plan(n, hh, ww, a, b, 3, stats_rows=hh * ww) in (1, 2) for a, b in ((ci, cm), (cm, co)))
            memo[key] = tuple(name for name in FEATNET_PAIR_BRANCHES if h % 16 == 0 and w % 16 == 0 and fits(name))
        return memo[key]

    def run_volume_net(self, mean_in, std, sn):
        pk = self._pack()
        dev = mean_in.device
        batched = mean_in.dim() == 3
        qn = mean_in.shape[0] if batched else 1
        pn = 1 if qn > 1 else 0

        def c3(x, wb, out, stride=1, aff=None, stats_c=None, count=None):
            st = ops.new_stats(qn, stats_c, dev) if stats_c else None
            sc, sh = aff if aff is not None else (None, None)
            return ops.conv(x, wb[0], wb[1], out, ksize=_K3, stride=(stride,) * 3, pad=_P3, in_scale=sc, in_shift=sh,
                            in_relu=aff is not None, per_n=pn if aff is not None else 0, stats=st,
                            rows_per_group=pn * (count or 0) if stats_c else 0,
                            w_wino=getattr(wb, "u", None) if stride == 1 else None,
                            w_wino43=getattr(wb, "u43", None) if (stride == 1 and qn >= F43_MIN_QUERIES) else None,
                            finalize=count if stats_c else None)

        def buf(s, c):
            return torch.empty((qn, s, s, s, c), dtype=torch.float32, device=dev)

        vox = sn ** 3
        cat = buf(sn, 128)
        def embed(name, x, sl):
            y = buf(sn, 64)
            aff = c3(x, pk[name][0], y, stats_c=64, count=vox)
            c3(y, pk[name][1], cat[..., sl], aff=aff)

        with self._mm("embed"):
            embed("v_mean_embed", mean_in.view(qn, sn, sn, sn, 256), slice(0, 64))
            embed("v_var_embed", std.view(qn, sn, sn, sn, 128), slice(64, 128))
        x, aff, s = cat, None, sn
        with self._mm("stack"):
            for name, co, stride in (("v_conv0", 64, 1), ("v_conv1", 128, 2), ("v_conv2", 128, 1), ("v_conv3", 256, 2),
                                     ("v_conv4", 256, 1)):
                s = s // stride
                y = buf(s, co)
                x, aff = y, c3(x, pk[name], y, stride=stride, aff=aff, stats_c=co, count=s ** 3)
        s = s // 2
        y = buf(s, 512)
        with self._mm("tail"):
            aff = c3(x, pk["v_conv5"][0], y, stride=2, aff=aff, stats_c=512, count=s ** 3)
            code = buf(s, 512)
            c3(y, pk["v_conv5"][1], code, aff=aff)
        return code.view(qn, s ** 3, 512) if batched else code.view(s ** 3, 512)

    def run_regressor(self, code):
        pk = self._pack()
        qn = code.shape[0] if code.dim() == 3 else 1
        x = ops.linear_gemv(code.reshape(qn, -1), pk["fc0"][0], pk["fc0"][1], act=2)
        x = ops.linear_gemv(x, pk["fc1"][0], pk["fc1"][1], act=2)
        o = ops.linear_gemv(x, pk["heads"][0], pk["heads"][1])
        ops.l2norm_rows(o[:, 0:4])
        return o[:, 0:4], o[:, 4:6], o[:, 6:7]

    def _step(self, *a, **k):
        with ops.math_mode(self.cfg.get("math_mode"), inherit_if_none=True):
            return self._step_fp(*a, **k)

    def _step_fp(self, que_img, K_in, pose_in, ref_imgs, ref_Ks, ref_poses, ref_feats=None):
        sn = self.cfg["refiner_sample_num"]
        dev = que_img.device
        ops.stats_arena_begin(dev)
        if ref_feats is not None:
            return self._step_from_feats(que_img, K_in, pose_in, ref_feats, ref_Ks, ref_poses)
        batched = ref_imgs.dim() == 5
        qn = ref_imgs.shape[0] if batched else 1
        rfn = ref_imgs.shape[-4]
        h_in, w_in = ref_imgs.shape[-2:]
        if batched:
            imgs = torch.cat([ref_imgs, que_img[:, None]], 1).reshape(qn * (rfn + 1), *ref_imgs.shape[-3:])
        else:
            imgs = torch.cat([ref_imgs, que_img], 0)
        feats = self.run_feature_net(imgs)
        lin = _linspace(sn, dev)
        C = feats.shape[-1]
        lead = (qn,) if batched else ()
        mean_in = torch.empty(lead + (sn ** 3, 2 * C), dtype=torch.float32, device=dev)
        std = torch.empty(lead + (sn ** 3, C), dtype=torch.float32, device=dev)
        feats = feats.contiguous()
        if batched:
            feats = feats.view(qn, rfn + 1, *feats.shape[1:])
        ops.refiner_volume_kp(feats, ref_Ks.contiguous(), ref_poses.contiguous(), K_in.contiguous(), pose_in.contiguous(),
                              lin, h_in, w_in, mean_in, std)
        return self.run_regressor(self.run_volume_net(mean_in, std, sn))

    def _step_from_feats(self, que_img, K_in, pose_in, ref_feats, ref_Ks, ref_poses):
        sn = self.cfg["refiner_sample_num"]
        dev = que_img.device
        h_in, w_in = que_img.shape[-2:]
        batched = ref_feats.dim() == 5
        qf = self.run_feature_net(que_img)
        if batched:
            feats = torch.cat([ref_feats, qf[:, None]], 1).contiguous()
            lead = (ref_feats.shape[0],)
        else:
            feats = torch.cat([ref_feats, qf], 0).contiguous()
            lead = ()
        lin = _linspace(sn, dev)
        C = feats.shape[-1]
        mean_in = torch.empty(lead + (sn ** 3, 2 * C), dtype=torch.float32, device=dev)
        std = torch.empty(lead + (sn ** 3, C), dtype=torch.float32, device=dev)
        ops.refiner_volume_kp(feats, ref_Ks.contiguous(), ref_poses.contiguous(), K_in.contiguous(), pose_in.contiguous(),
                              lin, h_in, w_in, mean_in, std)
        return self.run_regressor(self.run_volume_net(mean_in, std, sn))

    def forward(self, data):
        is_inference = data["inference"] if "inference" in data else False
        que, ref = data["que_imgs_info"], data["ref_imgs_info"]
        qn_all = que["imgs"].shape[0]
        if qn_all == 1:
            outs = [self._step(que["imgs"], que["Ks_in"][0], que["poses_in"][0], ref["imgs"][0], ref["Ks"][0], ref["poses"][0])]
        else:
            outs = [self._step(que["imgs"][q0:q0 + MAX_BATCH], que["Ks_in"][q0:q0 + MAX_BATCH], que["poses_in"][q0:q0 + MAX_BATCH],
                               ref["imgs"][q0:q0 + MAX_BATCH], ref["Ks"][q0:q0 + MAX_BATCH], ref["poses"][q0:q0 + MAX_BATCH])
                    for q0 in range(0, qn_all, MAX_BATCH)]
        out = {"rotation": ops.cat1([o[0] for o in outs], 0), "offset": ops.cat1([o[1] for o in outs], 0),
               "scale": ops.cat1([o[2] for o in outs], 0)}
        if not is_inference:
            sn = self.cfg["refiner_sample_num"]
            g = torch.linspace(-1, 1, sn, dtype=torch.float32, device=que["imgs"].device)
            V = torch.stack(torch.meshgrid(g, g, g, indexing="ij"), -1).reshape(1, sn ** 3, 3) @ que["poses_in"][:, :3, :3]
            out["grids"] = pose_apply_th(que["poses_in"], V)
        return out

    def load_ref_imgs(self, ref_database, ref_ids):
        cache = getattr(self, "image_cache", None)
        if ref_database is not self.ref_database and cache is not None and not cache.holds(ref_database):
            cache.clear()
        if ref_database is not self.ref_database:
            self.feat_cache.clear()
        self.ref_database = ref_database
        self.ref_ids = ref_ids

    def refine_que_imgs(self, que_img, que_K, in_pose, size=128, ref_num=6, ref_even=False):
        from .. import estimator as E
        from .. import geometry as G
        margin, even_num = 0.05, min(128, len(self.ref_ids))
        dev = self.device_()
        cache = getattr(self, "image_cache", None)
        if cache is None:
            cache = self.image_cache = E.DeviceImageCache(dev)
        db = E.NormalizedDatabase(self.ref_database)
        in_pose = G.normalize_pose(np.asarray(in_pose, np.float64), db.scale, db.offset)
        center, diameter = db.object_center, db.object_diameter
        que_K = np.asarray(que_K, np.float64)
        _, new_f = G.let_me_look_at(in_pose, que_K, center)
        in_dist = np.linalg.norm(G.pose_inverse(in_pose)[:, 3] - center)
        scale = size * (1 - margin) / diameter * in_dist / new_f
        position = G.project_points(center[None], in_pose, que_K)[0][0]
        K_warp, pose_warp, pose_rect, H = G.look_at_crop_params(que_K, in_pose, position, 0, scale, size, size)
        if not torch.is_tensor(que_img):
            que_img = torch.from_numpy(np.ascontiguousarray(que_img)).to(dev)
        que_warp = ops.warp_perspective(que_img, H, size, size)
        ref_ids = E.select_reference_img_ids_refinement(db, center, self.ref_ids, pose_warp, ref_num, ref_even, even_num, cache)
        f = lambda a: torch.from_numpy(np.ascontiguousarray(a, dtype=np.float32)).to(dev)
        que_t = que_warp.float().div_(255).permute(2, 0, 1)[None].contiguous()
        step = self.angle_step()
        with torch.no_grad():
            out = self.range_guarded(lambda: self._refine_step(step, db, ref_ids, size, margin, pose_warp, K_warp, cache, que_t, f))
        quat, offset, scale_pr = out[:4], out[4:6], 2 ** out[6]
        pose_sim = G.compose_sim_pose(scale_pr, quat, offset, pose_warp, center)
        pose_pr = G.pose_sim_to_pose_rigid(pose_sim, pose_warp, K_warp, K_warp, center)
        pose_pr = G.pose_compose(pose_pr, G.pose_inverse(pose_rect))
        return G.denormalize_pose(pose_pr, db.scale, db.offset)

    def _range_fallback(self):
        self.feat_cache.clear()

    def _refine_step(self, step, db, ref_ids, size, margin, pose_warp, K_warp, cache, que_t, f):
        from .. import estimator as E
        if step > 0:
            ref_Ks, ref_poses, Hs, buckets = E.reference_view_params(db, ref_ids, size, margin, True, pose_warp, K_warp, angle_step=step)
            keys = [(id(self.ref_database), str(i), int(b), int(size)) for i, b in zip(ref_ids, buckets)]
            make = lambda miss: torch.stack([ops.warp_perspective(cache.get(db, ref_ids[k]), Hs[k], size, size) for k in miss], 0) \
                .float().div_(255).permute(0, 3, 1, 2).contiguous()
            ref_feats = self.cached_ref_feats(keys, make)
            rot, off, scl = self._step(que_t, f(K_warp), f(pose_warp), None, f(ref_Ks), f(ref_poses), ref_feats=ref_feats)
        else:
            ref_imgs, _, ref_Ks, ref_poses, _ = E.normalize_reference_views(db, ref_ids, size, margin, cache, True, pose_warp, K_warp,
                                                                         with_masks=False)
            rot, off, scl = self._step(que_t, f(K_warp), f(pose_warp), ref_imgs.float().div_(255).permute(0, 3, 1, 2).contiguous(),
                                       f(ref_Ks), f(ref_poses))
        return torch.cat([rot[0], off[0], scl[0]]).cpu().numpy()

    def refine_step_tensors(self, que_img_u8, K_in, pose_in, ref_imgs_u8, ref_Ks, ref_poses):
        dev = self.device_()
        f = lambda a: torch.from_numpy(np.ascontiguousarray(a, dtype=np.float32)).to(dev)
        q = torch.from_numpy(np.ascontiguousarray(que_img_u8)).to(dev).float().div_(255).permute(2, 0, 1)[None].contiguous()
        r = torch.from_numpy(np.ascontiguousarray(ref_imgs_u8)).to(dev).float().div_(255).permute(0, 3, 1, 2).contiguous()
        with torch.no_grad():
            rot, off, scl = self._step(q, f(K_in), f(pose_in), r, f(ref_Ks), f(ref_poses))
        return rot[0].cpu().numpy(), 2 ** scl[0].cpu().numpy(), off[0].cpu().numpy()
```

gen6d_amd/ops.py:

```python
import ctypes as C
import math

import numpy as np
import torch

from . import lib as _lib

_WS = {}
WORKSPACE_BYTES = 96 << 20
MATH_MODE = 0
_MATH_NAMES = {"fp32": 0, "f32": 0, "bf16": 1, "fp16": 2, "f16": 2, 0: 0, 1: 1, 2: 2, None: 0}


class math_mode:

    def __init__(self, mode, inherit_if_none=False):
        self.mode = None if (mode is None and inherit_if_none) else _MATH_NAMES[mode]

    def __enter__(self):
        global MATH_MODE
        self.prev = MATH_MODE
        if self.mode is not None:
            MATH_MODE = self.mode
        return self
# ... 466 lines not shown
    return ys, yps


def corr2d_wino43_multi(xs, U43, outs, kblocks=5, k_true=None):
    _need_gpu(U43, *xs, *outs)
    if not 1 <= len(xs) <= 4 or len(outs) != len(xs):
        raise ValueError("corr2d_wino43_multi: 1..4 map sizes")
    Cin, Cout = xs[0].shape[4], outs[0].shape[4]
    if tuple(U43.shape) != w43_shape(kblocks * kblocks * (Cin // 8), Cout) or not U43.is_contiguous():
        raise ValueError(f"corr2d_wino43_multi: U43 must be contiguous {w43_shape(kblocks * kblocks * (Cin // 8), Cout)}")
    k = 3 * kblocks
    segs, flops, sizes = _corr_table("corr2d_wino43_multi", "corr2d_wino43", xs, outs, Cin, Cout, k)
    kt = k_true or k
    ws = workspace(U43.device)
    _timed(PROFILE is not None,
           lambda: _lib.check(_lib.load().g6d_corr2d_wino43_multi(segs, len(xs), Cin, _ptr(U43), Cout, int(kblocks), _ptr(ws), ws.numel() * 4, _stream()),
                              "g6d_corr2d_wino43_multi"),
           lambda e0, e1: PROFILE.append((flops / 4, e0, e1, f"wino3x3 F43 corr multi in={sizes}x{Cin} out={Cout} k={kt}x{kt} ({kblocks}x{kblocks} blocks of 3x3)",
                                          4.0 * (_numel(xs, outs) + U43.numel()), flops * kt * kt / (k * k))))
    return outs


def wino16_conv3x3_multi(xs, U16, bias, relu=True, full=True, pool=False):
    _need_gpu(U16, bias, *xs)
    mm = {torch.bfloat16: 1, torch.float16: 2}.get(U16.dtype)
    Cout = U16.shape[2]
    segs, Cin, ys, yps, flops, describe = _wino_table("wino16_conv3x3_multi", xs, Cout, full, pool)
    if mm is None or tuple(U16.shape) != (Cin // 16, 16, Cout, 16) or not U16.is_contiguous() or bias.numel() != Cout:
        raise ValueError(f"wino16_conv3x3_multi: U16 must be contiguous bfloat16 / float16 {(Cin // 16, 16, Cout, 16)}")
    ws = workspace(xs[0].device)
    _timed(PROFILE is not None,
           lambda: _lib.check(_lib.load().g6d_wino16_conv3x3_multi(segs, len(xs), Cin, _ptr(U16), _ptr(bias), Cout, int(relu), mm, _ptr(ws), ws.numel() * 4,
                                                                  _stream()), "g6d_wino16_conv3x3_multi"),
           _wino_book(flops / 2.25, "bf16 " if mm == 1 else "fp16 ", describe, U16.numel() / 2))
    return ys, yps


PAIR_KEEP = (2.0 ** -4, 2.0 ** 14)
PAIR_LIMIT = (2.0 ** -4, 2.0 ** 15)
PAIR_EXP_MAX = 100


def pair_exponent(a, e=0):
    if not math.isfinite(a):
        return e
    if a == 0.0 or PAIR_KEEP[0] <= a < PAIR_KEEP[1]:
        return 0
    return max(-PAIR_EXP_MAX, min(PAIR_EXP_MAX, math.frexp(a)[1] - 1))


def pair_out_of_window(a, e):
    if not math.isfinite(a):
        return True
    if a == 0.0:
        return False
    s = math.ldexp(a, -e)
    return s >= PAIR_LIMIT[1] or s < PAIR_LIMIT[0]


def bits_to_float(bits):
    return np.asarray(bits, dtype=np.int64).astype(np.uint32).view(np.float32).astype(np.float64)


class RangeTable:
    CAP = 64

    def __init__(self, device):
        self.device = device
        self.exps = torch.zeros(self.CAP, dtype=torch.int32, device=device)
        self.rec = torch.zeros(self.CAP, dtype=torch.int32, device=device)
        self.e = [0] * self.CAP
        self.names = {}

    def slot(self, name):
        if name not in self.names:
            if len(self.names) == self.CAP:
                raise RuntimeError("RangeTable: out of slots")
            self.names[name] = len(self.names)
        return self.names[name]

    def arg(self, slot_in=-1, slot_out=-1):
        return _lib.G6dRange16(exps=self.exps.data_ptr(), rec=self.rec.data_ptr(), slot_in=int(slot_in), slot_out=int(slot_out))

    def clear(self):
        _lib.check(_lib.load().g6d_zero_bytes(_ptr(self.rec), self.rec.numel() * 4, _stream()), "g6d_zero_bytes")

    def reset(self):
        self.e = [0] * self.CAP
        self.set_exponents({})
        self.clear()

    def read(self):
        a = bits_to_float(self.rec.cpu().numpy())
        return {n: float(a[i]) for n, i in self.names.items()}

    def set_exponents(self, es):
        for n, e in es.items():
            self.e[self.slot(n)] = int(e)
        self.exps.copy_(torch.tensor(self.e, dtype=torch.int32), non_blocking=False)


class PairMap:
    __slots__ = ("data", "table", "slot")

    def __init__(self, data, table, slot):
        self.data, self.table, self.slot = data, table, slot

    @property
    def shape(self):
        return self.data.shape

    def __getitem__(self, idx):
        return PairMap(self.data[idx], self.table, self.slot)

    def view(self, *shape):
        return PairMap(self.data.view(*shape), self.table, self.slot)


def _pair_inputs(xs):
    maps = [x for x in xs if isinstance(x, PairMap)]
    if not maps:
        return list(xs), None, -1
    if len(maps) != len(xs) or len({(id(m.table), m.slot) for m in maps}) != 1:
        raise ValueError("pair inputs of one launch must all be PairMaps of one slot")
    return [m.data for m in maps], maps[0].table, maps[0].slot


def _range_arg(table_in, slot_in, rng):
    table = rng[0] if rng is not None else table_in
    if table is None:
        return None
    if table_in is not None and table_in is not table:
        raise ValueError("pair input and output belong to different range tables")
    return C.byref(table.arg(slot_in, rng[1] if rng is not None else -1))


def _wrap(t, rng):
    return PairMap(t, rng[0], rng[1]) if (rng is not None and t is not None) else t


class Conv16Filters:

    def __init__(self, data, layout, mode, acc_scale, Cout, taps, Cin):
        self.data, self.layout, self.mode, self.acc_scale, self.Cout, self.taps, self.Cin = data, layout, mode, acc_scale, Cout, taps, Cin


def _split_hi_lo(w_taps):
    S = 2.0 ** min(14, math.floor(math.log2(2048.0 / max(float(w_taps.abs().max()), 1e-30))))
    w = w_taps.double() * S
    hi = w.to(torch.float16)
    return hi, (w - hi.double()).to(torch.float16), 1.0 / S


def conv16_pack(w_taps, mode, layout=1):
    co, taps, ci = w_taps.shape
    bk = 32 if mode == 3 else 64
    co_true = co
    if co == 64 and layout == 1 and taps == 9:
        w_taps = torch.cat([w_taps, torch.zeros_like(w_taps)], 0)
        co = 128
    if co % 128 or ci % bk:
        raise ValueError("conv16_pack: Cout % 128 == 0 (pairs, 2-D: also 64) and Cin % 64 (pairs: 32) == 0 expected")
    acc_scale = 1.0
    if mode == 3:
        hi, lo, acc_scale = _split_hi_lo(w_taps)
        planes = torch.stack([hi, lo], 0)
    else:
        planes = w_taps.to(_T16[mode])[None]
    if layout == 0:
        if mode == 3:
            raise ValueError("conv16_pack: pairs need the fragment-major layout")
        return Conv16Filters(planes[0].contiguous(), 0, mode, 1.0, co, taps, ci)
    P, ks = planes.shape[0], bk // 16
    x = planes.reshape(P, co // 128, 4, 32, taps, ci // bk, ks, 2, 8)
    x = x.permute(1, 5, 4, 6, 0, 2, 7, 3, 8).contiguous()
    return Conv16Filters(x.reshape(-1), 1, mode, acc_scale, co_true, taps, ci)


def product_split16(ref, que, scale, shift, mode, rng=None):
    if rng is not None and mode != 3:
        raise ValueError("product_split16: a range applies to pairs (mode 3) only")
    _need_gpu(ref, que, scale, shift)
    D, P, Cc = ref.shape
    qn = que.shape[0]
    if tuple(que.shape) != (qn, P, Cc) or tuple(scale.shape) != (qn, Cc) or tuple(shift.shape) != (qn, Cc) or not all(
            t.is_contiguous() and t.dtype == torch.float32 for t in (ref, que, scale, shift)):
        raise ValueError("product_split16: dense fp32 ref [D,P,C], que [qn,P,C], scale / shift [qn,C] expected")
    out = torch.empty((qn * D, P, 2, Cc) if mode == 3 else (qn * D, P, Cc), dtype=_T16[mode], device=ref.device)
    nbytes = 4.0 * (ref.numel() + que.numel()) + 2.0 * out.numel()
    ra = _range_arg(None, -1, rng)
    _timed_hbm("product_split16", nbytes, lambda: _lib.check(_lib.load().g6d_product_split16_ex(
        _ptr(ref), _ptr(que), _ptr(scale), _ptr(shift), _ptr(out), qn, D, P, Cc, int(mode), ra, _stream()), "g6d_product_split16"))
    return _wrap(out, rng)


def affine_split16(x, scale, shift, per_n, relu, pool, mode, rng=None):
    if rng is not None and mode != 3:
        raise ValueError("affine_split16: a range applies to pairs (mode 3) only")
    _need_gpu(x)
    N, D, H, W, Cc, ld_in = _cl5(x, "affine_split16.x")
    if D != 1:
        raise ValueError("affine_split16: 2-D maps expected")
    Ho, Wo = (H // 2, W // 2) if pool else (H, W)
    out = torch.empty((N, Ho, Wo, 2, Cc) if mode == 3 else (N, Ho, Wo, Cc), dtype=_T16[mode], device=x.device)
    ra = _range_arg(None, -1, rng)
    _timed_hbm("affine_split16", 4.0 * N * H * W * Cc + 2.0 * out.numel(), lambda: _lib.check(_lib.load().g6d_affine_split16_ex(
        _ptr(x), ld_in, _ptr(scale), _ptr(shift), int(per_n), int(bool(relu)), int(bool(pool)), N, H, W, Cc, _ptr(out), int(mode), ra, _stream()),
        "g6d_affine_split16"))
    return _wrap(out, rng)


def new_map16(N, H, W, Cc, mode, device, rng=None):
    if rng is not None and mode != 3:
        raise ValueError("new_map16: a range applies to pairs (mode 3) only")
    return _wrap(torch.empty((N, H, W, 2, Cc) if mode == 3 else (N, H, W, Cc), dtype=_T16[mode], device=device), rng)


def _slice16(out, N, Ho, Wo, Cc, c_off, mode, what):
    table, slot = (out.table, out.slot) if isinstance(out, PairMap) else (None, -1)
    t = out.data if isinstance(out, PairMap) else out
    if table is not None and mode != 3:
        raise ValueError(f"{what}: a PairMap output needs mode 3")
    _need_gpu(t)
    Ct = t.shape[-1]
    want = (N, Ho, Wo, 2, Ct) if mode == 3 else (N, Ho, Wo, Ct)
    if t.dtype != _T16[mode] or not t.is_contiguous() or tuple(t.shape) != want or c_off < 0 or c_off % 8 or Ct % 8 or c_off + Cc > Ct:
        raise ValueError(f"{what}: out must be a dense {_T16[mode]} map of shape {want[:-1]} + (C,) that holds channels [{c_off}, {c_off + Cc})")
    return t, (2 * Ct if mode == 3 else Ct), Ct, (C.byref(table.arg(-1, slot)) if table is not None else None)


def affine_split16_to(x, scale, shift, per_n, relu, mode, out, c_off=0):
    _need_gpu(x)
    N, D, H, W, Cc, ld_in = _cl5(x, "affine_split16_to.x")
    if D != 1:
        raise ValueError("affine_split16_to: 2-D maps expected")
    t, ld_out, plane, ra = _slice16(out, N, H, W, Cc, c_off, mode, "affine_split16_to")
    _timed_hbm("affine_split16", (4.0 + (4.0 if mode == 3 else 2.0)) * N * H * W * Cc, lambda: _lib.check(_lib.load().g6d_affine_split16_to(
        _ptr(x), ld_in, _ptr(scale), _ptr(shift), int(per_n), int(bool(relu)), 0, N, H, W, Cc, _ptr(t), ld_out, plane, int(c_off), int(mode), ra,
        _stream()), "g6d_affine_split16_to"))
    return out


def upsample_bilinear_split16(x, out, c_off, factor, scale, shift, per_n, mode):
    _need_gpu(x)
    N, D, H, W, Cc, ld_in = _cl5(x, "upsample_bilinear_split16.x")
    if D != 1:
        raise ValueError("upsample_bilinear_split16: 2-D maps expected")
    Ho, Wo = H * int(factor), W * int(factor)
    t, ld_out, plane, ra = _slice16(out, N, Ho, Wo, Cc, c_off, mode, "upsample_bilinear_split16")
    _timed_hbm("upsample_split16", 4.0 * N * H * W * Cc + (4.0 if mode == 3 else 2.0) * N * Ho * Wo * Cc, lambda: _lib.check(
        _lib.load().g6d_upsample_bilinear_split16(_ptr(x), ld_in, _ptr(scale), _ptr(shift), int(per_n), N, H, W, Cc, int(factor), _ptr(t), ld_out,
                                                  plane, int(c_off), int(mode), ra, _stream()), "g6d_upsample_bilinear_split16"))
    return out


def l2norm_split16(x, mode, rng=None):
    if rng is not None and mode != 3:
        raise ValueError("l2norm_split16: a range applies to pairs (mode 3) only")
    _need_gpu(x)
    if x.dtype != torch.float32 or not x.is_contiguous() or x.dim() != 4:
        raise ValueError("l2norm_split16: a dense float32 [N,H,W,C] tap expected")
    N, H, W, Cc = x.shape
    out = torch.empty((N, H, W, 2, Cc) if mode == 3 else (N, H, W, Cc), dtype=_T16[mode], device=x.device)
    ra = _range_arg(None, -1, rng)
    _timed_hbm("l2norm_split16", 4.0 * x.numel() + 2.0 * out.numel(), lambda: _lib.check(_lib.load().g6d_l2norm_split16(
        _ptr(x), Cc, N * H * W, Cc, _ptr(out), int(mode), ra, _stream()), "g6d_l2norm_split16"))
    return _wrap(out, rng)


def vgg_conv1_pool_nhwc16(x, w_oihw, bias, out=None, norm=None, mode=None, rng=None):
    _need_gpu(x, w_oihw, bias)
    mode = MATH_MODE if mode is None else mode
    if mode not in _T16:
        raise RuntimeError("vgg_conv1_pool_nhwc16: mode 1 (bf16), 2 (fp16) or 3 (fp16 pairs)")
    if rng is not None and mode != 3:
        raise ValueError("vgg_conv1_pool_nhwc16: a range applies to pairs (mode 3) only")
    N, Cin, H, W = x.shape
    Cout = w_oihw.shape[0]
    shape = (N, H // 2, W // 2, 2, Cout) if mode == 3 else (N, H // 2, W // 2, Cout)
    if out is None:
        out = torch.empty(shape, dtype=_T16[mode], device=x.device)
    if out.dtype != _T16[mode] or not out.is_contiguous() or tuple(out.shape) != shape:
        raise ValueError(f"vgg_conv1_pool_nhwc16: out must be a dense {_T16[mode]} tensor of shape {shape}")
    mean = std = None
    if norm is not None:
        mean, std = (C.c_float * 3)(*norm[0]), (C.c_float * 3)(*norm[1])
    _lib.check(_lib.load().g6d_vgg_conv1_pool_nhwc16_ex(_ptr(x.contiguous()), N, H, W, _ptr(w_oihw.contiguous()), _ptr(bias), Cin, Cout,
                                                        mean, std, _ptr(out), int(mode), _range_arg(None, -1, rng), _stream()),
               "g6d_vgg_conv1_pool_nhwc16")
    return _wrap(out, rng)


def conv16_direct_multi(xs, filt, bias, relu=True, full=None, pool=None, kd=1, stats=None, rows_per_group=0, out_full=None, rng=None):
    xs, table_in, slot_in = _pair_inputs(xs)
    if (table_in is not None or rng is not None) and filt.mode != 3:
        raise ValueError("conv16_direct_multi: ranges apply to pairs (mode 3) only")
    ra = _range_arg(table_in, slot_in, rng)
    _need_gpu(filt.data, *xs)
    mode = filt.mode
    t16 = _T16[mode]
    Cout, taps, Cin = filt.Cout, filt.taps, filt.Cin
    if taps != 9 * kd:
        raise ValueError("conv16_direct_multi: filters / kd mismatch")
    pair = mode == 3
    code = {None: 0, "t16": 3 if pair else 1, torch.float32: 2}
    if full not in code or pool not in code:
        raise ValueError('conv16_direct_multi: output types are None, torch.float32 or "t16"')
    segs = (_lib.G6dConv16Seg * len(xs))()
    fulls, pools, flops, sizes, nbytes = [], [], 0.0, [], 2.0 * filt.data.numel()
    nd = (4 if kd == 1 else 5) + (1 if pair else 0)
    for i, x in enumerate(xs):
        if x.dtype != t16 or not x.is_contiguous() or x.dim() != nd or x.shape[-1] != Cin or (pair and x.shape[-2] != 2):
            raise ValueError(f"conv16_direct_multi: input {i} must be a dense {t16} channels-last tensor with {Cin} channels{' in hi / lo planes' if pair else ''}")
        N, D, H, W = (x.shape[0], 1, x.shape[1], x.shape[2]) if kd == 1 else tuple(x.shape[:4])
        lead = (N, H, W) if kd == 1 else (N, D, H, W)

        def alloc(kind, lead_):
            if kind is None:
                return None
            if kind == "t16":
                return torch.empty(lead_ + ((2, Cout) if pair else (Cout,)), dtype=t16, device=x.device)
            return torch.empty(lead_ + (Cout,), dtype=torch.float32, device=x.device)
        q = alloc(pool, (N, H // 2, W // 2))
        ld_f = None
        if out_full is not None:
            f = out_full[i]
            want_t = torch.float32 if full is torch.float32 else t16
            nel = N * D * H * W * Cout * (2 if (pair and full == "t16") else 1)
            if full is None or f.dtype != want_t or f.numel() != nel or f.stride(-1) != 1:
                raise ValueError("conv16_direct_multi: out_full must hold the outputs' type and size")
            if not f.is_contiguous():
                ld_f = f.stride(-2)
                if full is not torch.float32 or f.shape[-1] != Cout or any(f.stride(d) != f.stride(d + 1) * f.shape[d + 1] for d in range(f.dim() - 2)):
                    raise ValueError("conv16_direct_multi: a strided out_full must be an fp32 channel slice of dense rows")
        else:
            f = alloc(full, lead)
        fulls.append(f); pools.append(q)
        ld = lambda t_: (2 * Cout if t_.dtype != torch.float32 and pair else Cout)
        segs[i] = _lib.G6dConv16Seg(in_=x.data_ptr(), out_full=f.data_ptr() if f is not None else None,
                                    out_pool=q.data_ptr() if q is not None else None, N=N, D=D, H=H, W=W, ld_in=(2 if pair else 1) * Cin,
                                    ld_full=(ld_f or ld(f)) if f is not None else 0, ld_pool=ld(q) if q is not None else 0)
        flops += 2.0 * N * D * H * W * Cout * taps * Cin
        nbytes += x.numel() * 2.0 + sum(t.numel() * t.element_size() for t in (f, q) if t is not None)
        sizes.append("x".join(str(v) for v in lead))
    _timed(PROFILE is not None,
           lambda: _lib.check(_lib.load().g6d_conv16_direct_multi_ex(
               segs, len(xs), Cin, _ptr(filt.data), int(filt.layout), float(filt.acc_scale), _ptr(bias), Cout, int(kd), int(bool(relu)), code[full],
               code[pool], int(mode), _ptr(stats), int(rows_per_group), ra, _stream()), "g6d_conv16_direct_multi"),
           lambda e0, e1: PROFILE.append((flops, e0, e1, f"{'conv16x3' if pair else 'conv16'} direct in={'+'.join(sizes)}x{Cin} out={Cout} k={'3x' if kd == 3 else ''}3x3"
                                          f"{' full' if full is not None else ''}{' pool' if pool is not None else ''}{' stats' if stats is not None else ''}", nbytes, flops)))
    if rng is not None:
        fulls = [_wrap(f, rng) if full == "t16" else f for f in fulls]
        pools = [_wrap(q, rng) if pool == "t16" else q for q in pools]
    return fulls, pools


def conv16_direct_plan(N, H, W, Cin, Cout, mode, stats_rows=0, full=torch.float32):
    pair = mode == 3
    code = {None: 0, "t16": 3 if pair else 1, torch.float32: 2}[full]
    any_ = 1 << 12
    ldf = 2 * Cout if code == 3 else Cout
    seg = (_lib.G6dConv16Seg * 1)(_lib.G6dConv16Seg(in_=any_, out_full=any_ if code else None, out_pool=None, N=N, D=1, H=H, W=W,
                                                    ld_in=(2 if pair else 1) * Cin, ld_full=ldf if code else 0, ld_pool=0))
    rc = _lib.load().g6d_conv16_direct_plan(seg, 1, Cin, C.c_void_p(any_), 1, Cout, 1, code, 0, int(mode), C.c_void_p(any_ if stats_rows else 0),
                                            int(stats_rows))
    return rc if rc >= 0 else None


def corr16_pack(w_taps, mode):
    co, taps, ci = w_taps.shape
    if co != 32 or ci % 32:
        raise ValueError("corr16_pack: 32 references and Cin % 32 == 0 expected")
    acc_scale = 1.0
    if mode == 3:
        hi, lo, acc_scale = _split_hi_lo(w_taps)
        x = torch.stack([hi, lo], 0).reshape(2, 32, taps, ci // 16, 2, 8)
        x = x.permute(3, 2, 0, 4, 1, 5).contiguous()
    else:
        x = w_taps.to(_T16[mode]).reshape(32, taps, ci // 32, 2, 2, 8)
        x = x.permute(2, 1, 3, 4, 0, 5).contiguous()
    k = int(round(taps ** 0.5))
    f = Conv16Filters(x.reshape(-1), 1, mode, acc_scale, co, taps, ci)
    f.k = k
    return f


def corr16_multi(xs, filt, outs):
    xs, table_in, slot_in = _pair_inputs(xs)
    if table_in is not None and filt.mode != 3:
        raise ValueError("corr16_multi: PairMaps need pair filters (mode 3)")
    ra = _range_arg(table_in, slot_in, None)
    _need_gpu(filt.data, *xs, *outs)
    mode, Cin = filt.mode, filt.Cin
    pair = mode == 3
    segs = (_lib.G6dConv16Seg * len(xs))()
    flops, sizes, nbytes = 0.0, [], 2.0 * filt.data.numel()
    for i, (x, o) in enumerate(zip(xs, outs)):
        if x.dtype != _T16[mode] or not x.is_contiguous() or x.dim() != (5 if pair else 4) or x.shape[-1] != Cin or not o.is_contiguous() \
                or o.dtype != torch.float32 or o.shape[-1] != 32:
            raise ValueError("corr16_multi: dense 16-bit channels-last inputs and dense fp32 outputs with 32 channels expected")
        N, H, W = x.shape[0], x.shape[1], x.shape[2]
        if o.numel() != N * H * W * 32:
            raise ValueError("corr16_multi: output shape mismatch")
        segs[i] = _lib.G6dConv16Seg(in_=x.data_ptr(), out_full=o.data_ptr(), out_pool=None, N=N, D=1, H=H, W=W, ld_in=(2 if pair else 1) * Cin,
                                    ld_full=32, ld_pool=0)
        flops += 2.0 * N * H * W * 32 * filt.taps * Cin
        nbytes += x.numel() * 2.0 + o.numel() * 4.0
        sizes.append(f"{N}x{H}x{W}")
    _timed(PROFILE is not None,
           lambda: _lib.check(_lib.load().g6d_corr16_multi_ex(segs, len(xs), Cin, _ptr(filt.data), float(filt.acc_scale), 32, int(filt.k), int(mode), ra,
                                                             _stream()), "g6d_corr16_multi"),
           lambda e0, e1: PROFILE.append((flops, e0, e1, f"{'conv16x3' if pair else 'conv16'} corr in={'+'.join(sizes)}x{Cin} out=32 k={filt.k}x{filt.k}",
                                          nbytes, flops)))
    return outs


def l2norm_rows(x):
    _need_gpu(x)
    Cc = x.shape[-1]
    if x.dtype == torch.float32 and x.dim() == 2 and x.stride(1) == 1 and not x.is_contiguous():
        _lib.check(_lib.load().g6d_l2norm_rows(_ptr(x), x.shape[0], Cc, x.stride(0), _stream()), "g6d_l2norm_rows")
        return x
    if x.dtype != torch.float32 or not x.is_contiguous():
        raise ValueError("l2norm_rows: contiguous float32 expected")
    _lib.check(_lib.load().g6d_l2norm_rows(_ptr(x), x.numel() // Cc, Cc, Cc, _stream()), "g6d_l2norm_rows")
    return x


def nchw_to_nhwc(x, out, l2norm):
    _need_gpu(x, out)
    if not x.is_contiguous() or x.dtype != torch.float32:
        raise ValueError("nchw_to_nhwc: x must be contiguous float32 NCHW")
    N, Cc, H, W = x.shape
    _, _, Ho, Wo, Co, ld_out = _cl5(out, "nchw_to_nhwc.out")
    if (Ho, Wo, Co) != (H, W, Cc):
        raise ValueError("nchw_to_nhwc: shape mismatch")
    _lib.check(_lib.load().g6d_nchw_to_nhwc(_ptr(x), N, Cc, H, W, int(l2norm), _ptr(out), ld_out, _stream()), "g6d_nchw_to_nhwc")
    return out


def selector_ref_sums(refs):
    _need_gpu(refs)
    D, HW, Cc = refs.shape
    r1 = torch.empty((HW, Cc), dtype=torch.float64, device=refs.device)
    r2 = torch.empty_like(r1)
    _lib.check(_lib.load().g6d_selector_ref_sums(_ptr(refs.contiguous()), D, HW, Cc, _ptr(r1), _ptr(r2), _stream()),
               "g6d_selector_ref_sums")
    return r1, r2


def selector_prod_affine(que, r1, r2, D, eps=1e-5):
    _need_gpu(que, r1, r2)
    HW, Cc = que.shape
    scale = torch.empty((1, Cc), dtype=torch.float32, device=que.device)
    shift = torch.empty_like(scale)
    _lib.check(_lib.load().g6d_selector_prod_affine(_ptr(que), _ptr(r1), _ptr(r2), D, HW, Cc, float(eps), _ptr(scale),
                                                   _ptr(shift), _stream()), "g6d_selector_prod_affine")
    return scale, shift


def selector_scan(que, refs):
    _need_gpu(que, refs)
    D, HW, Cc = refs.shape
    if not (que.is_contiguous() and refs.is_contiguous()):
        raise ValueError("selector_scan: operands must be contiguous")
    smap = torch.empty((D, HW), dtype=torch.float32, device=que.device)
    vps = torch.empty((D,), dtype=torch.float32, device=que.device)
    _timed_hbm("selector_scan", 4.0 * (D * HW * Cc + HW * Cc + 2 * D * HW + D),
               lambda: _lib.check(_lib.load().g6d_selector_scan(_ptr(que), _ptr(refs), D, HW, Cc, _ptr(smap), _ptr(vps),
                                                                _stream()), "g6d_selector_scan"))
    return smap, vps


def selector_levels(ques, refs, sums, Dg, eps=1e-5, want_maps=False, _out=None):
    L = len(ques)
    _need_gpu(*ques, *refs)
    single = ques[0].dim() == 2
    if single:
        ques = [q.unsqueeze(0) for q in ques]
    qn = ques[0].shape[0]
    D, _, Cc = refs[0].shape
    dev = ques[0].device
    if qn > 8:
        vps = torch.empty((qn, L, D), dtype=torch.float32, device=dev)
        scale = torch.empty((qn, L, Cc), dtype=torch.float32, device=dev)
        shift = torch.empty_like(scale)
        maps = [torch.empty((qn, D, r.shape[1]), dtype=torch.float32, device=dev) for r in refs] if want_maps else None
        for i in range(0, qn, 8):
            selector_levels([q[i:i + 8] for q in ques], refs, sums, Dg, eps, want_maps,
                            _out=(vps[i:i + 8], scale[i:i + 8], shift[i:i + 8], [m[i:i + 8] for m in maps] if want_maps else None))
        return vps, scale, shift, maps
    for q, r in zip(ques, refs):
        if not (q.is_contiguous() and r.is_contiguous()) or r.shape[0] != D or r.shape[2] != Cc or tuple(q.shape) != (qn,) + tuple(r.shape[1:]):
            raise ValueError("selector_levels: operands must be contiguous [qn,HW,C] / [D,HW,C]")
    if _out is not None:
        vps, scale, shift, maps = _out
    else:
        vps = torch.empty((qn, L, D), dtype=torch.float32, device=dev)
        scale = torch.empty((qn, L, Cc), dtype=torch.float32, device=dev)
        shift = torch.empty_like(scale)
        maps = None
    if maps is None:
        maps = [torch.empty((qn, D, r.shape[1]), dtype=torch.float32, device=dev) for r in refs]
    arr = lambda ts: (C.c_void_p * L)(*[t.data_ptr() if t is not None else None for t in ts])
    hw = (C.c_int * L)(*[r.shape[1] for r in refs])
    nbytes = sum(4.0 * (D * r.shape[1] * Cc + qn * (r.shape[1] * Cc + 2 * D * r.shape[1] + D)) + 16.0 * qn * r.shape[1] * Cc for r in refs)
    _timed_hbm("selector_levels", nbytes,
               lambda: _lib.check(_lib.load().g6d_selector_levels(L, qn, arr(ques), arr(refs), arr([s_[0] for s_ in sums]), arr([s_[1] for s_ in sums]),
                                                                  hw, D, int(Dg), Cc, float(eps), arr(maps), _ptr(vps),
                                                                  _ptr(scale), _ptr(shift), _stream()), "g6d_selector_levels"))
    if single:
        return vps[0], scale[0], shift[0], ([m[0] for m in maps] if want_maps else None)
    return vps, scale, shift, (maps if want_maps else None)


def refiner_volume(feats, projs, rot_in, lin, h_in, w_in, mean_in, std):
    _need_gpu(feats, projs, rot_in, lin, mean_in, std)
    V, fh, fw, Cc = feats.shape
    sn = lin.numel()
    for t in (feats, projs, rot_in, lin, mean_in, std):
        if not t.is_contiguous() or t.dtype != torch.float32:
            raise ValueError("refiner_volume: operands must be contiguous float32")
    if tuple(mean_in.shape) != (sn ** 3, 2 * Cc) or tuple(std.shape) != (sn ** 3, Cc) or tuple(projs.shape) != (V, 3, 4):
        raise ValueError("refiner_volume: shape mismatch")
    _timed_hbm("refiner_volume", 4.0 * (V * fh * fw * Cc + 3 * sn ** 3 * Cc),
               lambda: _lib.check(_lib.load().g6d_refiner_volume(_ptr(feats), _ptr(projs), _ptr(rot_in), _ptr(lin), V - 1, fh,
                                                                 fw, Cc, int(h_in), int(w_in), sn, _ptr(mean_in), _ptr(std),
                                                                 _stream()), "g6d_refiner_volume"))
    return mean_in, std


def refiner_volume_kp(feats, ref_Ks, ref_poses, K_in, pose_in, lin, h_in, w_in, mean_in, std):
    _need_gpu(feats, ref_Ks, ref_poses, K_in, pose_in, lin, mean_in, std)
    batched = feats.dim() == 5
    B = feats.shape[0] if batched else 1
    V, fh, fw, Cc = feats.shape[-4:]
    sn = lin.numel()
    for t in (feats, ref_Ks, ref_poses, K_in, pose_in, lin, mean_in, std):
        if not t.is_contiguous() or t.dtype != torch.float32:
            raise ValueError("refiner_volume_kp: operands must be contiguous float32")
    lead = (B,) if batched else ()
    if (tuple(mean_in.shape) != lead + (sn ** 3, 2 * Cc) or tuple(std.shape) != lead + (sn ** 3, Cc) or tuple(ref_Ks.shape) != lead + (V - 1, 3, 3) or
            tuple(ref_poses.shape) != lead + (V - 1, 3, 4) or tuple(K_in.shape) != lead + (3, 3) or tuple(pose_in.shape) != lead + (3, 4)):
        raise ValueError("refiner_volume_kp: shape mismatch")
    _timed_hbm("refiner_volume", 4.0 * B * (V * fh * fw * Cc + 3 * sn ** 3 * Cc),
               lambda: _lib.check(_lib.load().g6d_refiner_volume_kp(_ptr(feats), _ptr(ref_Ks), _ptr(ref_poses), _ptr(K_in), _ptr(pose_in),
                                                                    _ptr(lin), V - 1, fh, fw, Cc, int(h_in), int(w_in), sn, _ptr(mean_in),
                                                                    _ptr(std), B, _stream()), "g6d_refiner_volume_kp"))
    return mean_in, std


def cat1(ts, dim=0):
    return ts[0] if len(ts) == 1 else torch.cat(ts, dim)


def resize_bilinear_pyramid(imgs, sizes):
    _need_gpu(imgs)
    if imgs.dim() != 4 or imgs.dtype != torch.float32 or not imgs.is_contiguous():
        raise ValueError("resize_bilinear_pyramid: imgs must be contiguous float32 [N,C,H,W]")
    N, Cc, H, W = imgs.shape
    todo = [i for i, (h, w) in enumerate(sizes) if (h, w) != (H, W)]
    if len(todo) > 4:
        raise ValueError("resize_bilinear_pyramid: at most 4 destination sizes")
    outs = [imgs] * len(sizes)
    if not todo:
        return outs
    buf = torch.empty(sum(N * Cc * sizes[i][0] * sizes[i][1] for i in todo), dtype=torch.float32, device=imgs.device)
    o = 0
    dst = []
    for i in todo:
        h, w = sizes[i]
        dst.append(buf[o:o + N * Cc * h * w].view(N, Cc, h, w)); o += N * Cc * h * w
        outs[i] = dst[-1]
    hs = (C.c_int * len(todo))(*[sizes[i][0] for i in todo])
    ws_ = (C.c_int * len(todo))(*[sizes[i][1] for i in todo])
    ptrs = (C.c_void_p * len(todo))(*[d.data_ptr() for d in dst])
    _lib.check(_lib.load().g6d_resize_bilinear_pyramid(_ptr(imgs), N * Cc, H, W, len(todo), hs, ws_, ptrs, _stream()), "g6d_resize_bilinear_pyramid")
    return outs


def detector_assemble(s0, s1, s2, hc, wc, mu_sigma, clip, hs, ws, scale_idx, stacked, batch=1):
    _need_gpu(s0, s1, s2, stacked)
    rfn = s0.shape[1]
    P, rfn2, nch = stacked.shape
    if P != batch * hs * ws or rfn2 != rfn or not stacked.is_contiguous() or not (s0.is_contiguous() and s1.is_contiguous() and s2.is_contiguous()):
        raise ValueError("detector_assemble: stacked shape mismatch")
    if s0.shape[0] != batch * hc * wc or s1.shape[0] != batch * (hc // 2) * (wc // 2) or s2.shape[0] != batch * (hc // 4) * (wc // 4):
        raise ValueError("detector_assemble: level map sizes do not match")
    ms = (C.c_float * 6)(*[float(v) for pair in mu_sigma for v in pair])
    _lib.check(_lib.load().g6d_detector_assemble(_ptr(s0), _ptr(s1), _ptr(s2), hc, wc, rfn, ms, float(clip), hs, ws,
                                                int(scale_idx), nch, _ptr(stacked), int(batch), _stream()), "g6d_detector_assemble")
    return stacked


def detector_score_mlp_max(stacked, w0, b0, w1, b1):
    _need_gpu(stacked, w0, b0, w1, b1)
    P, rfn, nch = stacked.shape
    out = torch.empty((P, 64), dtype=torch.float32, device=stacked.device)
    _lib.check(_lib.load().g6d_detector_score_mlp_max(_ptr(stacked), P, rfn, nch, _ptr(w0), _ptr(b0), _ptr(w1), _ptr(b1),
                                                     _ptr(out), _stream()), "g6d_detector_score_mlp_max")
    return out


def detector_decode(scores, offset, scale, hs, ws, pool_ratio, batch=1):
    _need_gpu(scores, offset, scale)
    if scores.shape[0] != batch * hs * ws:
        raise ValueError("detector_decode: row count mismatch")
    res = torch.empty((batch, 5), dtype=torch.float32, device=scores.device)
    _lib.check(_lib.load().g6d_detector_decode(_ptr(scores), scores.stride(0), _ptr(offset), offset.stride(0), _ptr(scale),
                                              scale.stride(0), hs, ws, int(pool_ratio), _ptr(res), int(batch), _stream()),
               "g6d_detector_decode")
    return res[0] if batch == 1 else res


def vps_norm(vps, feats, c_off):
    _need_gpu(vps, feats)
    batch = vps.shape[0] if vps.dim() == 3 else 1
    D = vps.shape[-1]
    if feats.shape[0] != batch * D:
        raise ValueError("vps_norm: feats rows != batch * D")
    _lib.check(_lib.load().g6d_vps_norm(_ptr(vps.contiguous()), D, _ptr(feats), feats.stride(0), int(c_off), batch, _stream()),
               "g6d_vps_norm")
    return feats


def max_an_add(x, rfn, an, embed, out, batch=1):
    _need_gpu(x, embed, out)
    Cc = x.shape[1]
    if x.shape[0] != batch * rfn * an or out.shape[0] != batch * rfn:
        raise ValueError("max_an_add: row count mismatch")
    _lib.check(_lib.load().g6d_max_an_add(_ptr(x), x.stride(0), rfn, an, Cc, _ptr(embed.contiguous()), _ptr(out),
                                         out.stride(0), int(batch), _stream()), "g6d_max_an_add")
    return out


def attention(q, k, v, heads, out, batch=1):
    _need_gpu(q, k, v, out)
    rows, Cc = q.shape
    if not (q.stride(0) == k.stride(0) == v.stride(0)) or rows % batch:
        raise ValueError("attention: q/k/v must share the row stride; rows = batch * n")
    _lib.check(_lib.load().g6d_attention(_ptr(q), _ptr(k), _ptr(v), q.stride(0), rows // batch, Cc, heads, _ptr(out), out.stride(0),
                                        int(batch), _stream()), "g6d_attention")
    return out


def layernorm(x, gamma, beta, out, eps=1e-5):
    _need_gpu(x, gamma, beta, out)
    n, Cc = x.shape
    _lib.check(_lib.load().g6d_layernorm(_ptr(x), x.stride(0), n, Cc, _ptr(gamma), _ptr(beta), float(eps), _ptr(out),
                                        out.stride(0), _stream()), "g6d_layernorm")
    return out


def affine_act_add(x, out, scale=None, shift=None, relu=False, residual=None, rows_per_group=0):
    _need_gpu(x, out)
    n, Cc = x.shape
    _lib.check(_lib.load().g6d_affine_act_add(_ptr(x), x.stride(0), _ptr(scale), _ptr(shift), int(relu), _ptr(residual),
                                             residual.stride(0) if residual is not None else 0, n, Cc, _ptr(out),
                                             out.stride(0), int(rows_per_group), _stream()), "g6d_affine_act_add")
    return out


def linear_gemv(x, W, bias, act=0):
    _need_gpu(x, W)
    B, K = x.shape
    O = W.shape[0]
    out = torch.empty((B, O), dtype=torch.float32, device=x.device)
    x = x.contiguous()
    ws = workspace(x.device)
    _timed_hbm("linear_gemv" if O * K >= (1 << 22) else "linear_gemv_small", 4.0 * (O * K + B * K + B * O),
               lambda: _lib.check(_lib.load().g6d_linear_gemv_batch(_ptr(x), B, K, _ptr(W), _ptr(bias), O, int(act), _ptr(out), _ptr(ws),
                                                                    ws.numel() * 4, _stream()), "g6d_linear_gemv_batch"))
    return out


def warp_perspective(src_u8, H, dh, dw, out_float=False):
    _need_gpu(src_u8)
    if src_u8.dtype != torch.uint8 or src_u8.dim() != 3 or not src_u8.is_contiguous():
        raise ValueError("warp_perspective: src must be a contiguous uint8 [H,W,C] tensor")
    H = np.asarray(H, dtype=np.float64)
    if H.shape == (2, 3):
        H = np.concatenate([H, [[0.0, 0.0, 1.0]]], 0)
    hinv = np.linalg.inv(H).astype(np.float32).reshape(-1)
    sh, sw, ch = src_u8.shape
    dst = torch.empty((dh, dw, ch), dtype=torch.float32 if out_float else torch.uint8, device=src_u8.device)
    _lib.check(_lib.load().g6d_warp_perspective(_ptr(src_u8), sh, sw, ch, (C.c_float * 9)(*hinv.tolist()), _ptr(dst), dh, dw,
                                               int(out_float), 1.0 / 255.0, _stream()), "g6d_warp_perspective")
    return dst


def _f32c(*ts):
    for t in ts:
        if t.dtype != torch.float32 or not t.is_contiguous():
            raise ValueError("chain ops: contiguous float32 device tensors expected")


def chain_crop_from_detection(det, size):
    _need_gpu(det); _f32c(det)
    B = det.shape[0] if det.dim() == 2 else 1
    hinv = torch.empty((B, 9), dtype=torch.float32, device=det.device)
    _lib.check(_lib.load().g6d_chain_crop_from_detection(_ptr(det), float(size), _ptr(hinv), B, _stream()), "g6d_chain_crop_from_detection")
    return hinv


# ... 264 lines not shown
```

include/gen6d_hip.h:

```cpp
#ifndef GEN6D_HIP_H
#define GEN6D_HIP_H

#include <stddef.h>
#include <stdint.h>

#ifdef __cplusplus
extern "C" {
#endif

typedef void* g6d_stream_t;

enum {
  G6D_OK = 0,
  G6D_EINVAL = -1,
  G6D_ENOSPC = -2,
  G6D_ELAUNCH = -3
};

int g6d_abi_version(void);
const char* g6d_last_error(void);

int g6d_set_knob(const char* name, double value);
double g6d_get_knob(const char* name);
void g6d_reset_knobs(void);
// ... 16 lines not shown
  int32_t N, Di, Hi, Wi, Cin, ld_in;
  int32_t Do, Ho, Wo, Cout, ld_out;
  int32_t kd, kh, kw;
  int32_t sd, sh, sw;
  int32_t pd, ph, pw;
  int32_t in_relu;
  int32_t in_affine_per_n;
  int32_t out_act;
  int32_t stat_rows_per_group;
  int32_t split_k;
  int32_t math_mode;
  const float* weight_wino;
  float* fin_scale;
  float* fin_shift;
  int32_t* fin_counter;
  double fin_count, fin_eps;
  int32_t fin_groups;
  int32_t in_image_mod;
  int32_t mul_group_images;
  int32_t reserved_;
  const void* weight_wino16;
  const float* weight_wino43;
} G6dConv;

int g6d_conv_igemm(const G6dConv* desc, g6d_stream_t stream);
int g6d_conv_plan(const G6dConv* desc);
int g6d_sizeof_conv_desc(void);

int g6d_corr2d_patch(const float* in, int H, int W, int Cin, int ld_in, const float* wgt, int Cout, int kh, int kw,
                     float* out, int ld_out, float* workspace, size_t workspace_bytes, int math_mode ,
                     g6d_stream_t stream);
typedef struct G6dCorrSeg {
  const float* in;
  float* out;
  int32_t H, W, ld_in, ld_out;
  int32_t N, reserved_;
} G6dCorrSeg;
int g6d_corr2d_patch_multi(const G6dCorrSeg* segs, int nseg, int Cin, const float* wgt, int Cout, int kh, int kw,
                           float* workspace, size_t workspace_bytes, int math_mode, g6d_stream_t stream);
int g6d_corr2d_patch16_multi(const G6dCorrSeg* segs, int nseg, int Cin, const void* w16, int Cout, int kh, int kw,
                             float* workspace, size_t workspace_bytes, int math_mode, g6d_stream_t stream);

int g6d_corr2d_wino_multi(const G6dCorrSeg* segs, int nseg, int Cin, const float* U, int Cout, int kblocks, float* workspace,
                          size_t workspace_bytes, g6d_stream_t stream);

int g6d_corr2d_wino43_multi(const G6dCorrSeg* segs, int nseg, int Cin, const float* U43, int Cout, int kblocks, float* workspace,
                            size_t workspace_bytes, g6d_stream_t stream);

int g6d_stats_finalize(const double* stats, int n, double count, double eps, float* scale, float* shift, g6d_stream_t stream);

int g6d_affine_act_pool(const float* in, int ld_in, const float* scale, const float* shift, int affine_per_n, int relu,
                        int pool, int N, int H, int W, int C, float* out, int ld_out, g6d_stream_t stream);

int g6d_upsample_bilinear(const float* in, int ld_in, const float* scale, const float* shift, int affine_per_n,
                          int N, int H, int W, int C, int factor, float* out, int ld_out, g6d_stream_t stream);

int g6d_bias_relu_pool_nchw(const float* in, const float* bias, int N, int C, int H, int W, int relu, int pool, float* out,
                            g6d_stream_t stream);

int g6d_vgg_conv1_pool(const float* in, int N, int H, int W, const float* w_oihw, const float* bias, int Cin, int Cout,
                       float* out, g6d_stream_t stream);

int g6d_vgg_conv1_pool_nhwc(const float* in, int N, int H, int W, const float* w_oihw, const float* bias, int Cin, int Cout,
                            float* out, g6d_stream_t stream);
int g6d_vgg_conv1_pool_nhwc_norm(const float* in, int N, int H, int W, const float* w_oihw, const float* bias, int Cin, int Cout,
                                 const float* mean_host, const float* std_host, float* out, g6d_stream_t stream);
int g6d_vgg_conv1_pool_nhwc16(const float* in, int N, int H, int W, const float* w_oihw, const float* bias, int Cin, int Cout,
                              const float* mean_host, const float* std_host, void* out16, int math_mode, g6d_stream_t stream);


int g6d_wino_conv3x3(const float* in, int N, int H, int W, int Cin, int ld_in, const float* U, const float* bias, int Cout,
                     int relu, float* out_full, int ld_full, float* out_pool, int ld_pool, float* workspace,
                     size_t workspace_bytes, g6d_stream_t stream);

typedef struct G6dWinoSeg {
  const float* in;
  float* out_full;
  float* out_pool;
  int32_t N, H, W, ld_in, ld_full, ld_pool;
} G6dWinoSeg;
int g6d_wino_conv3x3_multi(const G6dWinoSeg* segs, int nseg, int Cin, const float* U, const float* bias, int Cout, int relu,
                           float* workspace, size_t workspace_bytes, g6d_stream_t stream);

int g6d_wino16_conv3x3_multi(const G6dWinoSeg* segs, int nseg, int Cin, const void* U16, const float* bias, int Cout, int relu,
                             int math_mode, float* workspace, size_t workspace_bytes, g6d_stream_t stream);

typedef struct G6dConv16Seg {
  const void* in;
  void* out_full;
  void* out_pool;
  int32_t N, D, H, W, ld_in, ld_full, ld_pool;
} G6dConv16Seg;
int g6d_conv16_direct_multi(const G6dConv16Seg* segs, int nseg, int Cin, const void* W16, int w_layout, float acc_scale, const float* bias,
                            int Cout, int kd, int relu, int full_type, int pool_type, int math_mode, double* stats, int stat_rows_per_group,
                            g6d_stream_t stream);

int g6d_product_split16(const float* ref, const float* que, const float* scale, const float* shift, void* out, int qn, int D, int P, int C,
                        int math_mode, g6d_stream_t stream);

int g6d_affine_split16(const float* in, int ld_in, const float* scale, const float* shift, int affine_per_n, int relu, int pool, int N, int H, int W,
                       int C, void* out, int math_mode, g6d_stream_t stream);

int g6d_corr16_multi(const G6dConv16Seg* segs, int nseg, int Cin, const void* W16, float acc_scale, int Cout, int k, int math_mode,
                     g6d_stream_t stream);

typedef struct G6dRange16 {
  const int32_t* exps;
  uint32_t* rec;
  int32_t slot_in, slot_out;
} G6dRange16;
int g6d_conv16_direct_multi_ex(const G6dConv16Seg* segs, int nseg, int Cin, const void* W16, int w_layout, float acc_scale, const float* bias,
                               int Cout, int kd, int relu, int full_type, int pool_type, int math_mode, double* stats, int stat_rows_per_group,
                               const G6dRange16* range, g6d_stream_t stream);
int g6d_conv16_direct_plan(const G6dConv16Seg* segs, int nseg, int Cin, const void* W16, int w_layout, int Cout, int kd, int full_type, int pool_type,
                           int math_mode, double* stats, int stat_rows_per_group);
int g6d_corr16_multi_ex(const G6dConv16Seg* segs, int nseg, int Cin, const void* W16, float acc_scale, int Cout, int k, int math_mode,
                        const G6dRange16* range, g6d_stream_t stream);
int g6d_product_split16_ex(const float* ref, const float* que, const float* scale, const float* shift, void* out, int qn, int D, int P, int C,
                           int math_mode, const G6dRange16* range, g6d_stream_t stream);
int g6d_affine_split16_ex(const float* in, int ld_in, const float* scale, const float* shift, int affine_per_n, int relu, int pool, int N, int H,
                          int W, int C, void* out, int math_mode, const G6dRange16* range, g6d_stream_t stream);
int g6d_vgg_conv1_pool_nhwc16_ex(const float* in, int N, int H, int W, const float* w_oihw, const float* bias, int Cin, int Cout,
                                 const float* mean_host, const float* std_host, void* out16, int math_mode, const G6dRange16* range,
                                 g6d_stream_t stream);

int g6d_affine_split16_to(const float* in, int ld_in, const float* scale, const float* shift, int affine_per_n, int relu, int pool, int N, int H,
                          int W, int C, void* out, int ld_out, int plane, int c_off, int math_mode, const G6dRange16* range, g6d_stream_t stream);
int g6d_upsample_bilinear_split16(const float* in, int ld_in, const float* scale, const float* shift, int affine_per_n, int N, int H, int W, int C,
                                  int factor, void* out, int ld_out, int plane, int c_off, int math_mode, const G6dRange16* range,
                                  g6d_stream_t stream);
int g6d_l2norm_split16(const float* in, int ld_in, int rows, int C, void* out, int math_mode, const G6dRange16* range, g6d_stream_t stream);

int g6d_wino43_conv3x3_multi(const G6dWinoSeg* segs, int nseg, int Cin, const float* U43, const float* bias, int Cout, int relu,
                             float* workspace, size_t workspace_bytes, g6d_stream_t stream);

int g6d_l2norm_rows(float* x, int rows, int C, int ld, g6d_stream_t stream);

int g6d_nchw_to_nhwc(const float* in, int N, int C, int H, int W, int l2norm, float* out, int ld_out, g6d_stream_t stream);

int g6d_selector_ref_sums(const float* refs, int D, int HW, int C, double* r1, double* r2, g6d_stream_t stream);
int g6d_selector_prod_affine(const float* que, const double* r1, const double* r2, int D, int HW, int C, double eps,
                             float* scale, float* shift, g6d_stream_t stream);
int g6d_selector_scan(const float* que, const float* refs, int D, int HW, int C, float* score_map, float* vps,
                      g6d_stream_t stream);
int g6d_selector_levels(int nlev, int qn, const float* const* que, const float* const* refs, const double* const* r1,
                        const double* const* r2, const int* HW, int D, int Dg, int C, double eps, float* const* score_maps,
                        float* vps, float* scale, float* shift, g6d_stream_t stream);

int g6d_refiner_volume(const float* feats, const float* projs, const float* rot_in, const float* lin, int rfn, int fh,
                       int fw, int C, int h_in, int w_in, int sn, float* mean_in, float* std, g6d_stream_t stream);
int g6d_refiner_volume_kp(const float* feats, const float* ref_Ks, const float* ref_poses, const float* K_in, const float* pose_in,
                          const float* lin, int rfn, int fh, int fw, int C, int h_in, int w_in, int sn, float* mean_in, float* stdv,
                          int batch, g6d_stream_t stream);

int g6d_detector_assemble(const float* s0, const float* s1, const float* s2, int hc, int wc, int rfn,
                          const float* mu_sigma , float clip, int hs, int ws,
                          int scale_idx, int nch, float* stacked, int batch, g6d_stream_t stream);

int g6d_detector_score_mlp_max(const float* stacked, int P, int rfn, int nch, const float* w0, const float* b0,
                               const float* w1, const float* b1, float* out, g6d_stream_t stream);

int g6d_detector_decode(const float* scores, int ld_s, const float* offset, int ld_o, const float* scale, int ld_c,
                        int hs, int ws, int pool_ratio, float* result, int batch, g6d_stream_t stream);
int g6d_resize_bilinear_pyramid(const float* src, int planes, int H, int W, int nscale, const int* hs, const int* ws,
                                float* const* dsts, g6d_stream_t stream);
int g6d_zero_bytes(void* ptr, size_t bytes, g6d_stream_t stream);

int g6d_vps_norm(const float* vps, int D, float* feats, int ld, int c_off, int batch, g6d_stream_t stream);
int g6d_max_an_add(const float* in, int ld_in, int rfn, int an, int C, const float* embed, float* out, int ld_out, int batch,
                   g6d_stream_t stream);
int g6d_attention(const float* q, const float* k, const float* v, int ld, int n, int C, int heads, float* out,
                  int ld_out, int batch, g6d_stream_t stream);
int g6d_layernorm(const float* in, int ld_in, int n, int C, const float* gamma, const float* beta, float eps,
                  float* out, int ld_out, g6d_stream_t stream);
int g6d_affine_act_add(const float* in, int ld_in, const float* scale, const float* shift, int relu,
                       const float* residual, int ld_res, int n, int C, float* out, int ld_out, int rows_per_group,
                       g6d_stream_t stream);

int g6d_warp_perspective(const unsigned char* src, int sh, int sw, int ch, const float* hinv, void* dst, int dh, int dw,
                         int out_float, float out_scale, g6d_stream_t stream);

int g6d_chain_crop_from_detection(const float* det, float size, float* hinv, int batch, g6d_stream_t stream);
int g6d_chain_pose_from_selection(const float* det, const float* logits, const float* angles, int rfn, const float* ref_poses,
                                  const float* ref_Ks, const float* que_K, const float* center, float* pose_out, float* sel_out,
                                  int batch, g6d_stream_t stream);
int g6d_chain_refine_prepare(const float* pose_in, const float* que_K, const float* norm, float size, float margin,
                             const float* sub_poses, const float* sub_Ks, int n_sub, int ref_num, float* geo, int* ref_idx,
                             float angle_step, int* ref_bucket, int batch, g6d_stream_t stream);
int g6d_chain_refine_update(const float* rot, const float* off, const float* scl, const float* geo, int geo_floats ,
                            const float* norm, float* pose_out, int batch, g6d_stream_t stream);
int g6d_warp_batch(const unsigned char* stack, const unsigned char* single, const int* idx, int B, int sh, int sw, int ch,
                   const float* hinv, float* dst, int dh, int dw, g6d_stream_t stream);

int g6d_linear_gemv(const float* x, int B, int K, const float* W, const float* bias, int O, int act, float* out,
                    g6d_stream_t stream);

int g6d_linear_gemv_batch(const float* x, int B, int K, const float* W, const float* bias, int O, int act, float* out, float* workspace,
                          size_t workspace_bytes, g6d_stream_t stream);

int g6d_track_gather(const float* pose_table, const int* slot_stream, const float* parking_pose, float* pose_out, int batch,
                     g6d_stream_t stream);
#define G6D_TRACK_MAX_NUM 64
int g6d_track_commit(const float* pose, const float* K, const int* slot_stream, int reset, const float* box, int num, float std,
                     float* pose_table, double* hist, int* hist_count, float* smooth_table, float* out, int batch, g6d_stream_t stream);

enum { G6D_TRACK_NONE = 0, G6D_TRACK_TRACKING = 1, G6D_TRACK_SUSPECT = 2, G6D_TRACK_LOST = 3 };
enum { G6D_TRACK_NONFINITE = 1, G6D_TRACK_BEHIND = 2, G6D_TRACK_SMALL = 4, G6D_TRACK_LARGE = 8, G6D_TRACK_OUTSIDE = 16, G6D_TRACK_ROT = 32,
       G6D_TRACK_SHIFT = 64, G6D_TRACK_SCALE = 128, G6D_TRACK_VERIFY_POS = 256, G6D_TRACK_VERIFY_SCALE = 512 };
int g6d_track_gate(const float* pose_table, int32_t* health, const int* slot_stream, int* slot_eff, int batch, g6d_stream_t stream);
int g6d_track_health(const float* pose_prev, const float* pose_new, const float* K, const int32_t* pic, int W, int H, const int* slot_eff,
                     int reset, const float* center, double diameter, int patience, double min_px, double max_px, double margin,
                     double max_rot_deg, double max_shift, double max_log2_scale, int32_t* health, float* measures, int* slot_commit,
                     int* slot_draw, int batch, g6d_stream_t stream);
int g6d_track_verify(const float* det, const float* pose_table, const float* K, const int* slot_commit, const float* center,
                     double diameter, double ref_px, double verify_shift, double verify_log2_scale, int verify_patience, int32_t* health,
                     float* measures, int batch, g6d_stream_t stream);

enum { G6D_FMT_RGB24 = 0, G6D_FMT_BGR24 = 1, G6D_FMT_RGBA32 = 2, G6D_FMT_BGRA32 = 3, G6D_FMT_NV12 = 4 };
typedef struct G6dFrame {
  const void* plane0;
  const void* plane1;
  int32_t pitch0, pitch1;
  int32_t width, height;
  int32_t format;
  int32_t rotate;
  int32_t matrix;
  int32_t slot;
  int32_t out_w, out_h;
  float   K[9];
} G6dFrame;
int g6d_frame_ingest(const G6dFrame* frames, int n, uint8_t* out, int B, int H, int W, float* K_out, g6d_stream_t stream);
int g6d_sizeof_frame_desc(void);

typedef struct G6dMesh {
  const int32_t* nodes;
  int32_t nx, ny;
  int32_t step_log2;
  int32_t reserved;
} G6dMesh;
int g6d_frame_ingest_mesh(const G6dFrame* frames, const G6dMesh* meshes, int n, uint8_t* out, int B, int H, int W, float* K_out,
                          g6d_stream_t stream);
int g6d_sizeof_mesh_desc(void);

int g6d_track_corners(const float* table, const float* K, const int* slot_stream, const float* box, int32_t* pts, int32_t* valid,
                      int batch, g6d_stream_t stream);
typedef struct G6dSink {
  void* plane0;
  void* plane1;
  int32_t pitch0, pitch1;
  int32_t width, height;
  int32_t format;
  int32_t matrix;
  int32_t slot;
  int32_t pic_w, pic_h;
  int32_t thickness, dot_radius;
  int32_t line_rgb, dot_rgb;
  int32_t box;
} G6dSink;
int g6d_frame_emit(const G6dSink* sinks, int n, const uint8_t* imgs, int B, int H, int W, const int32_t* pts, const int32_t* valid,
                   g6d_stream_t stream);
int g6d_sizeof_sink_desc(void);

int g6d_frame_emit_source(const G6dSink* sinks, int n, const G6dFrame* frames, int nf, const int32_t* pts, const int32_t* valid, int sets,
                          int B, int max_w, int max_h, g6d_stream_t stream);

#ifdef __cplusplus
}
#endif
#endif
```

Measured before the change: 338.1.

## Fold 3-D conv depth taps into fp16-pair halo kernel and emit pair volumes

```diff
diff --git a/gen6d_amd/csrc/conv16_direct.hip b/gen6d_amd/csrc/conv16_direct.hip
--- a/gen6d_amd/csrc/conv16_direct.hip
+++ b/gen6d_amd/csrc/conv16_direct.hip
@@ -559,10 +559,11 @@
   }
 }
 
-template <int MM, int WM, int NT2 = C16W<MM>::NT2>
+template <int MM, int WM, int NT2 = C16W<MM>::NT2, int KD = 1>
 __global__ __launch_bounds__(256, 2) void conv16w_kernel(const C16Params p) {
   typedef typename C16T3<MM>::V V8;
   typedef C16W<MM> R;
+  static_assert(KD == 1 || (KD == 3 && MM == 3), "depth taps fold into the pair kernel's reduction only");
   constexpr int WN = 4 / WM, NP = R::NP, KS = R::KS, NBL = KS * NP * NT2, CW = 32 * NT2;
   constexpr bool SINGLE = MM == 3 && WM == 2;
   constexpr int TILE_B = NP * R::PLANE, STAGE = WM * TILE_B;
@@ -572,7 +573,7 @@
   const int cb = jj % p.nN, tg = (jj / p.nN) * 8 + xcd;
   if (tg * WM >= p.ptiles) return;
   const int wm = wv / WN, wn = wv % WN;
-  const int nchunk = p.Cin >> 5;
+  const int nchunk = KD == 1 ? p.Cin >> 5 : 3 * (p.Cin >> 5);
   typedef __attribute__((address_space(3))) void* lds_ptr;
 
   constexpr int NPJ = (R::NI_MAX + 3) / 4;
@@ -615,18 +616,40 @@
     }
     pmask[tl] = __builtin_amdgcn_readfirstlane(pm);
   }
+  int c_lo_ = 0, c_hi_ = nchunk;
+  [[maybe_unused]] int zt[WM];
+  [[maybe_unused]] const int ncs = p.Cin >> 5;
+  if constexpr (KD == 3) {
+    bool first = true, last = true;
+#pragma unroll
+    for (int tl = 0; tl < WM; ++tl) {
+      zt[tl] = (int)((unsigned)gms[tl].t.img % (unsigned)p.D);
+      first = first && zt[tl] == 0; last = last && zt[tl] == p.D - 1;
+    }
+    c_lo_ = first ? ncs : 0; c_hi_ = last ? 2 * ncs : 3 * ncs;
+  }
+  const int c_lo = c_lo_, c_hi = c_hi_;
   const unsigned plane_b = (unsigned)(p.Cin * 2);
   auto issue_patch = [&](int c, int stage) {
-    if (c >= nchunk) return;
-    const unsigned ck = (unsigned)(c * 64);
+    if (c >= c_hi) return;
+    [[maybe_unused]] int dz = 1;
+    unsigned ck;
+    if constexpr (KD == 3) { dz = (c >= ncs ? 1 : 0) + (c >= 2 * ncs ? 1 : 0); ck = (unsigned)((c - dz * ncs) * 64); }
+    else ck = (unsigned)(c * 64);
 #pragma unroll
     for (int tl = 0; tl < WM; ++tl) {
       const C16Seg& sg = p.seg[gms[tl].si];
       const __amdgpu_buffer_rsrc_t rs_in = c16_rsrc(sg.in, sg.in_bytes - sg.back);
+      unsigned ckt = ck;
+      bool pad = false;
+      if constexpr (KD == 3) {
+        ckt = ck + (unsigned)((dz - 1) * (sg.H * sg.W * sg.ld_in * 2));
+        pad = (unsigned)(zt[tl] + dz - 1) >= (unsigned)p.D;
+      }
 #pragma unroll
       for (int j = 0; j < NPJ; ++j) {
         if (pmask[tl] >> j & 1) {
-          const unsigned vo = poff[tl][j] == C16_OOB ? C16_OOB : poff[tl][j] + ck;
+          const unsigned vo = (poff[tl][j] == C16_OOB || pad) ? C16_OOB : poff[tl][j] + ckt;
 #pragma unroll
           for (int pl = 0; pl < NP; ++pl)
             __builtin_amdgcn_raw_ptr_buffer_load_lds(rs_in, (lds_ptr)(lds + stage * STAGE + tl * TILE_B + pl * R::PLANE + (wv + 4 * j) * 1024), 16,
@@ -651,8 +674,8 @@
 #pragma unroll
     for (int q = 0; q < KS * NP; ++q) bvo[q] = q * 4096 + ((chan0 >> 5) & 3) * 1024 + lane * 16;
   }
-  const char* wp = wtile;
-  int wleft = nchunk * 9;
+  const char* wp = KD == 1 ? wtile : wtile + (long)c_lo * (9 * 16384);
+  int wleft = (c_hi - c_lo) * 9;
   auto load_b = [&](int c, int t, V8 (&b)[NBL]) {
     const unsigned long wa = (unsigned long)(wleft > 0 ? wp : wtile);
     const char* ws = reinterpret_cast<const char*>((unsigned long)(unsigned)__builtin_amdgcn_readfirstlane((unsigned)wa) |
@@ -704,7 +727,7 @@
 
     V8 bs[3][NBL];
     V8 fa[3][2][NP];
-    issue_patch(0, 0);
+    issue_patch(c_lo, 0);
     load_b(0, 0, bs[0]);
     load_b(0, 1, bs[1]);
     asm volatile("s_waitcnt vmcnt(0) lgkmcnt(0)" ::: "memory");
@@ -714,7 +737,7 @@
     for (int mp = 0; mp < 3; ++mp) read_pair(mp, tap_off(0, 0), fa[mp]);
     int stage = 0;
 #pragma unroll 1
-    for (int c = 0; c < ((C16W_ABLATE & 8) ? 0 : nchunk); ++c) {
+    for (int c = c_lo; c < ((C16W_ABLATE & 8) ? 0 : c_hi); ++c) {
 #pragma unroll
       for (int mt = 0; mt < 8; ++mt) asm volatile("" : "+v"(qb[mt]));
 #pragma unroll
@@ -745,7 +768,7 @@
             __builtin_amdgcn_s_barrier();
             __builtin_amdgcn_sched_barrier(0);
           } else stage ^= 1;
-          if (c + 1 < nchunk) {
+          if (c + 1 < c_hi) {
 #pragma unroll
             for (int mp = 0; mp < 3; ++mp) read_pair(mp, tap_off(0, stage), fa[mp]);
           }
@@ -1369,7 +1392,7 @@
 }
 
 
-bool c16_halo_tiling(const G6dConv16Seg& s, C16Seg& o, int& tiles, bool pairs) {
+bool c16_halo_tiling(const G6dConv16Seg& s, C16Seg& o, int& tiles, bool pairs, bool in_image = false) {
   double best = 1e30;
   bool found = false;
   for (int tw = 32; tw >= 4; tw >>= 1) {
@@ -1377,7 +1400,7 @@
     long nt; int tpi, segh, bands;
     if (s.H >= th) { tpi = tx * ((s.H + th - 1) / th); nt = (long)s.N * tpi; segh = th; bands = 1; }
     else {
-      if (th % s.H) continue;
+      if (th % s.H || in_image) continue;
       tpi = 0; nt = (long)tx * (((long)s.N * s.H + th - 1) / th); segh = s.H; bands = th / s.H;
     }
     if (bands * (segh + 2) * (tw + 2) > 288) continue;
@@ -1411,11 +1434,12 @@
                int full_type, int pool_type, int math_mode, double* stats, int stat_rows_per_group, const G6dRange16* range, g6d_stream_t stream,
                bool plan_only) {
   if (!segs || nseg < 1 || nseg > 4 || !W16) { g6d_set_error("conv16_direct: 1..4 segments and filters expected"); return G6D_EINVAL; }
-  if (math_mode < 1 || math_mode > 3 || (w_layout != 0 && w_layout != 1) || (math_mode == 3 && w_layout != 1)) {
+  const bool folded = w_layout == 2;
+  if (math_mode < 1 || math_mode > 3 || w_layout < 0 || w_layout > 2 || (math_mode == 3 && w_layout == 0) || (folded && (math_mode != 3 || kd != 3))) {
     g6d_set_error("conv16_direct: math_mode 1 (bf16) / 2 (fp16) / 3 (fp16 hi-lo pairs, fragment-major filters only)"); return G6D_EINVAL;
   }
   const int bk = math_mode == 3 ? 32 : C16_BK, planes = math_mode == 3 ? 2 : 1;
-  const bool half_tile = Cout == 64 && w_layout == 1 && kd == 1;
+  const bool half_tile = Cout == 64 && ((w_layout == 1 && kd == 1) || folded);
   if (Cin % bk || (Cout % C16_BN && !half_tile) || (kd != 1 && kd != 3)) { g6d_set_error("conv16_direct: Cin % 64 (32 for pairs), Cout % 128 (64: fragment-major 2-D layers), kd in {1,3} expected"); return G6D_EINVAL; }
   const int t16 = math_mode == 3 ? 3 : 1;
   auto type_ok = [&](int t) { return t == 0 || t == 2 || t == t16; };
@@ -1462,11 +1486,19 @@
   p.D = D0;
   p.ptiles = tiles;
   hipStream_t st = static_cast<hipStream_t>(stream);
-  if (w_layout == 1 && kd == 1 && g6d_knob(G6D_KNOB_CONV16_HALO) != 0) {
+  if (((w_layout == 1 && kd == 1) || folded) && g6d_knob(G6D_KNOB_CONV16_HALO) != 0) {
     bool ok = true, per_pass = false;
     int htiles = 0;
     for (int i = 0; i < nseg && ok; ++i) {
       int nt_ = 0;
+      if (folded) {
+        G6dConv16Seg planes_ = segs[i];
+        planes_.N = segs[i].N * segs[i].D; planes_.D = 1;
+        ok = (long)segs[i].N * segs[i].D < (1L << 31) && c16_halo_tiling(planes_, p.seg[i], nt_, true, true);
+        p.seg[i].h_tile0 = htiles; htiles += nt_;
+        if (stats && stat_rows_per_group > 0 && ok) ok = stat_rows_per_group % ((long)segs[i].D * segs[i].H * segs[i].W) == 0;
+        continue;
+      }
       ok = c16_halo_tiling(segs[i], p.seg[i], nt_, math_mode == 3);
       p.seg[i].h_tile0 = htiles; htiles += nt_;
       if (stats && stat_rows_per_group > 0 && ok) {
@@ -1497,6 +1529,10 @@
         if (math_mode == 1) launch(&conv16w_kernel<1, 2, 1>, 2 * 2 * C16W<1>::PLANE, 4 * C16W<1>::EPW);
         else launch(&conv16w_kernel<2, 2, 1>, 2 * 2 * C16W<2>::PLANE, 4 * C16W<2>::EPW);
       }
+      else if (folded) {
+        if (wm == 1) launch(&conv16w_kernel<3, 1, 1, 3>, 2 * C16W<3>::NP * C16W<3>::PLANE, 4 * C16W<3>::EPW);
+        else launch(&conv16w_kernel<3, 2, 1, 3>, 2 * C16W<3>::NP * C16W<3>::PLANE, 4 * C16W<3>::EPW);
+      }
       else if (math_mode == 1) { if (wm == 1) C16W_LAUNCH(1, 1); else C16W_LAUNCH(1, 2); }
       else if (math_mode == 2) { if (wm == 1) C16W_LAUNCH(2, 1); else C16W_LAUNCH(2, 2); }
       else { if (wm == 1) C16W_LAUNCH(3, 1); else C16W_LAUNCH(3, 2); }
@@ -1504,6 +1540,7 @@
       return g6d_check_launch("conv16w_direct");
     }
   }
+  if (folded) { g6d_set_error("conv16_direct: depth-folded filters run on the halo-patch kernel only (planes at least one tile high, statistics groups of whole volumes)"); return G6D_EINVAL; }
   if (half_tile) { g6d_set_error("conv16_direct: Cout = 64 runs on the halo-patch kernel only (knob conv16_halo, tile shapes)"); return G6D_EINVAL; }
   if (!pertap_stats_ok) { g6d_set_error("conv16_direct: statistics groups must be whole tile rows (small maps: whole 64-pixel epilogue passes)"); return G6D_EINVAL; }
   if (plan_only) return 0;
diff --git a/gen6d_amd/csrc/conv16w_geom.h b/gen6d_amd/csrc/conv16w_geom.h
--- a/gen6d_amd/csrc/conv16w_geom.h
+++ b/gen6d_amd/csrc/conv16w_geom.h
@@ -50,6 +50,7 @@
 struct Tile {
   int g0, x0, y0, ylim;
   int interior;
+  int img;
 };
 C16G_HD Tile tile_of(const Tiling& tl, int H, int W, int t) {
   Tile o;
@@ -59,10 +60,12 @@
     const int ty = (int)div31((unsigned)r, tl.h_r_tx), tx = r - ty * tl.h_tiles_x;
     o.y0 = ty * TH; o.x0 = tx * TW; o.g0 = n * H + o.y0; o.ylim = TH < H - o.y0 ? TH : H - o.y0;
     o.interior = o.y0 >= 1 && o.y0 + TH < H && o.x0 >= 1 && o.x0 + TW < W;
+    o.img = n;
   } else {
     const int ty = (int)div31((unsigned)t, tl.h_r_tx), tx = t - ty * tl.h_tiles_x;
     o.y0 = 0; o.x0 = tx * TW; o.g0 = ty * TH; o.ylim = TH;
     o.interior = 0;
+    o.img = 0;
   }
   return o;
 }
diff --git a/gen6d_amd/csrc/refiner_volume.hip b/gen6d_amd/csrc/refiner_volume.hip
--- a/gen6d_amd/csrc/refiner_volume.hip
+++ b/gen6d_amd/csrc/refiner_volume.hip
@@ -1,4 +1,5 @@
 #include "g6d_common.h"
+#include <type_traits>
 
 #define MAX_RFN 8
 
@@ -59,16 +60,36 @@
 struct VolViews { const float* projs; const float* ref_Ks; const float* ref_poses; const float* K_in; const float* pose_in;
                   const float* rot; int rot_ld; };
 
+struct VolPairs { G6dRange16 mean, stdv; };
+
+__device__ __forceinline__ void store_pair4(_Float16* hi_p, int plane, f32x4 v, int e, unsigned& amax) {
+  typedef _Float16 h4 __attribute__((ext_vector_type(4)));
+  h4 hi, lo;
+#pragma unroll
+  for (int i = 0; i < 4; ++i) {
+    amax = max(amax, g6d_abs_bits(v[i]));
+    const float u = ldexpf(v[i], -e);
+    hi[i] = (_Float16)u; lo[i] = (_Float16)(u - (float)hi[i]);
+  }
+  *reinterpret_cast<h4*>(hi_p) = hi;
+  *reinterpret_cast<h4*>(hi_p + plane) = lo;
+}
+
+template <bool PAIRS>
 __global__ void __launch_bounds__(256, 4) refiner_volume_kernel(const float* __restrict__ feats, const VolViews vw,
                                                              const float* __restrict__ lin, int rfn, int fh, int fw,
                                                              int C, float h_in, float w_in, int sn,
-                                                             float* __restrict__ mean_in, float* __restrict__ stdv) {
+                                                             typename std::conditional<PAIRS, _Float16, float>::type* __restrict__ mean_in,
+                                                             typename std::conditional<PAIRS, _Float16, float>::type* __restrict__ stdv,
+                                                             const VolPairs vp) {
   const int bq = blockIdx.y;
   const float* __restrict__ rot = vw.rot + bq * 12;
   const int rl = vw.rot_ld;
   const int nvox = sn * sn * sn;
   feats += (size_t)bq * (rfn + 1) * fh * fw * C;
-  mean_in += (size_t)bq * nvox * 2 * C; stdv += (size_t)bq * nvox * C;
+  mean_in += (size_t)bq * nvox * (PAIRS ? 4 : 2) * C; stdv += (size_t)bq * nvox * (PAIRS ? 2 : 1) * C;
+  [[maybe_unused]] const int e_mean = PAIRS ? g6d_exp_out(vp.mean) : 0, e_std = PAIRS ? g6d_exp_out(vp.stdv) : 0;
+  [[maybe_unused]] unsigned amax_mean = 0, amax_std = 0;
   int half = (blockIdx.x * blockDim.x + threadIdx.x) >> 5;
   const int l32 = threadIdx.x & 31;
   const bool live = half < nvox;
@@ -112,9 +133,20 @@
     f32x4 sd = {sqrtf(var[0]), sqrtf(var[1]), sqrtf(var[2]), sqrtf(var[3])};
     const f32x4 q = gather_view(feats + rfn * fsz + c, taps_from(mine, rfn));
     if (!live || !c_in) continue;
-    *reinterpret_cast<f32x4*>(mean_in + (size_t)half * 2 * C + c) = mean;
-    *reinterpret_cast<f32x4*>(mean_in + (size_t)half * 2 * C + C + c) = q;
-    *reinterpret_cast<f32x4*>(stdv + (size_t)half * C + c) = sd;
+    if constexpr (PAIRS) {
+      store_pair4(mean_in + (size_t)half * 4 * C + c, 2 * C, mean, e_mean, amax_mean);
+      store_pair4(mean_in + (size_t)half * 4 * C + C + c, 2 * C, q, e_mean, amax_mean);
+      store_pair4(stdv + (size_t)half * 2 * C + c, C, sd, e_std, amax_std);
+    } else {
+      *reinterpret_cast<f32x4*>(mean_in + (size_t)half * 2 * C + c) = mean;
+      *reinterpret_cast<f32x4*>(mean_in + (size_t)half * 2 * C + C + c) = q;
+      *reinterpret_cast<f32x4*>(stdv + (size_t)half * C + c) = sd;
+    }
+  }
+  if constexpr (PAIRS) {
+    g6d_range_record_block<4>(vp.mean, amax_mean);
+    __syncthreads();
+    g6d_range_record_block<4>(vp.stdv, amax_std);
   }
 }
 
@@ -130,9 +162,9 @@
   }
   const long long threads = (long long)sn * sn * sn * 32;
   const VolViews vw = {projs, nullptr, nullptr, nullptr, nullptr, rot_in, 3};
-  hipLaunchKernelGGL(refiner_volume_kernel, dim3((unsigned)((threads + 255) / 256)), dim3(256), 0,
+  hipLaunchKernelGGL(refiner_volume_kernel<false>, dim3((unsigned)((threads + 255) / 256)), dim3(256), 0,
                      reinterpret_cast<hipStream_t>(stream), feats, vw, lin, rfn, fh, fw, C, (float)h_in, (float)w_in, sn,
-                     mean_in, stdv);
+                     mean_in, stdv, VolPairs{});
   return g6d_check_launch("refiner_volume");
 }
 
@@ -146,8 +178,29 @@
   }
   const long long threads = (long long)sn * sn * sn * 32;
   const VolViews vw = {nullptr, ref_Ks, ref_poses, K_in, pose_in, pose_in, 4};
-  hipLaunchKernelGGL(refiner_volume_kernel, dim3((unsigned)((threads + 255) / 256), batch), dim3(256), 0,
+  hipLaunchKernelGGL(refiner_volume_kernel<false>, dim3((unsigned)((threads + 255) / 256), batch), dim3(256), 0,
                      reinterpret_cast<hipStream_t>(stream), feats, vw, lin, rfn, fh, fw, C, (float)h_in, (float)w_in, sn,
-                     mean_in, stdv);
+                     mean_in, stdv, VolPairs{});
   return g6d_check_launch("refiner_volume_kp");
 }
+
+extern "C" int g6d_refiner_volume_kp_pairs(const float* feats, const float* ref_Ks, const float* ref_poses, const float* K_in,
+                                           const float* pose_in, const float* lin, int rfn, int fh, int fw, int C, int h_in, int w_in, int sn,
+                                           void* mean_in16, void* std16, int batch, const G6dRange16* range_mean, const G6dRange16* range_std,
+                                           g6d_stream_t stream) {
+  if (!feats || !ref_Ks || !ref_poses || !K_in || !pose_in || !lin || !mean_in16 || !std16 || rfn < 1 || rfn > MAX_RFN || C < 4 || (C & 3) ||
+      fh <= 0 || fw <= 0 || h_in <= 0 || w_in <= 0 || sn < 1 || sn > 256 || batch < 1 || batch > 65535 || !g6d_aligned16(feats) ||
+      !g6d_aligned16(mean_in16) || !g6d_aligned16(std16)) {
+    g6d_set_error("refiner_volume_kp_pairs: bad args (1 <= rfn <= 8, C a positive multiple of 4, positive map and image sizes)"); return G6D_EINVAL;
+  }
+  const long long threads = (long long)sn * sn * sn * 32;
+  const VolViews vw = {nullptr, ref_Ks, ref_poses, K_in, pose_in, pose_in, 4};
+  VolPairs vp = {};
+  vp.mean.slot_in = vp.mean.slot_out = vp.stdv.slot_in = vp.stdv.slot_out = -1;
+  if (range_mean) vp.mean = *range_mean;
+  if (range_std) vp.stdv = *range_std;
+  hipLaunchKernelGGL(refiner_volume_kernel<true>, dim3((unsigned)((threads + 255) / 256), batch), dim3(256), 0,
+                     reinterpret_cast<hipStream_t>(stream), feats, vw, lin, rfn, fh, fw, C, (float)h_in, (float)w_in, sn,
+                     static_cast<_Float16*>(mean_in16), static_cast<_Float16*>(std16), vp);
+  return g6d_check_launch("refiner_volume_kp_pairs");
+}
diff --git a/gen6d_amd/lib.py b/gen6d_amd/lib.py
--- a/gen6d_amd/lib.py
+++ b/gen6d_amd/lib.py
@@ -108,6 +108,7 @@
     "g6d_selector_levels": [_I, _I, _P, _P, _P, _P, _P, _I, _I, _I, _D, _P, _P, _P, _P, _P],
     "g6d_refiner_volume": [_P, _P, _P, _P, _I, _I, _I, _I, _I, _I, _I, _P, _P, _P],
     "g6d_refiner_volume_kp": [_P, _P, _P, _P, _P, _P, _I, _I, _I, _I, _I, _I, _I, _P, _P, _I, _P],
+    "g6d_refiner_volume_kp_pairs": [_P, _P, _P, _P, _P, _P, _I, _I, _I, _I, _I, _I, _I, _P, _P, _I, _P, _P, _P],
     "g6d_detector_assemble": [_P, _P, _P, _I, _I, _I, C.POINTER(C.c_float), _F, _I, _I, _I, _I, _P, _I, _P],
     "g6d_detector_score_mlp_max": [_P, _I, _I, _I, _P, _P, _P, _P, _P, _P],
     "g6d_detector_decode": [_P, _I, _P, _I, _P, _I, _I, _I, _I, _P, _I, _P],
diff --git a/gen6d_amd/network/params.py b/gen6d_amd/network/params.py
--- a/gen6d_amd/network/params.py
+++ b/gen6d_amd/network/params.py
@@ -11,10 +11,11 @@
         t.u, t.u43, t._w16 = u, u43, {}
         return t
 
-    def w16(self, mode):
-        if mode not in self._w16:
-            self._w16[mode] = ops.conv16_pack(self[0], mode, layout=1)
-        return self._w16[mode]
+    def w16(self, mode, layout=1):
+        key = mode if layout == 1 else (mode, layout)
+        if key not in self._w16:
+            self._w16[key] = ops.conv16_pack(self[0], mode, layout=layout)
+        return self._w16[key]
 
 
 class ParamBank(nn.Module):
diff --git a/gen6d_amd/network/refiner.py b/gen6d_amd/network/refiner.py
--- a/gen6d_amd/network/refiner.py
+++ b/gen6d_amd/network/refiner.py
@@ -10,6 +10,7 @@
 F43_MIN_QUERIES = 4
 FEATNET_F43_LAYERS = {("conv1", 0), ("conv_out", 0), ("conv_out", 3)}
 FEATNET_PAIR_BRANCHES = ("conv0", "conv1", "conv2", "conv_out")
+VOLUME_PAIR_LAYERS = ("mean_embed", "var_embed", "conv0", "conv2")
 VOLUME_F43_LAYERS = ("conv0",)
 MAX_BATCH = 32
 _K3, _P3 = (3, 3, 3), (1, 1, 1)
@@ -196,10 +197,35 @@
             memo[key] = tuple(name for name in FEATNET_PAIR_BRANCHES if h % 16 == 0 and w % 16 == 0 and fits(name))
         return memo[key]
 
+    def volume_pair_route(self, qn, sn):
+        if qn < F43_MIN_QUERIES or self._pair_rng() is None or not {"mean_embed", "var_embed"} <= set(VOLUME_PAIR_LAYERS):
+            return False
+        memo = self.__dict__.setdefault("_volume16", {})
+        key = (qn, sn, tuple(VOLUME_PAIR_LAYERS))
+        if key not in memo:
+            shapes = [(sn, 256, 64), (sn, 128, 64), (sn, 64, 64)] + ([(sn, 128, 64)] if "conv0" in VOLUME_PAIR_LAYERS else []) + \
+                ([(sn // 2, 128, 128)] if "conv2" in VOLUME_PAIR_LAYERS else [])
+            memo[key] = all(ops.conv16_direct_plan(qn, s, s, ci, co, 3, stats_rows=s ** 3, D=s) == 1 for s, ci, co in shapes)
+        return memo[key]
+
+    def feature_volumes(self, feats, ref_Ks, ref_poses, K_in, pose_in, h_in, w_in, sn):
+        dev = feats.device
+        lin = _linspace(sn, dev)
+        C = feats.shape[-1]
+        args = (feats, ref_Ks.contiguous(), ref_poses.contiguous(), K_in.contiguous(), pose_in.contiguous(), lin, h_in, w_in)
+        if feats.dim() == 5 and self.volume_pair_route(feats.shape[0], sn):
+            rng = self._pair_rng()
+            return ops.refiner_volume_kp_pairs(*args, rng_mean=(rng, rng.slot("volume.mean_in")), rng_std=(rng, rng.slot("volume.std")))
+        lead = (feats.shape[0],) if feats.dim() == 5 else ()
+        mean_in = torch.empty(lead + (sn ** 3, 2 * C), dtype=torch.float32, device=dev)
+        std = torch.empty(lead + (sn ** 3, C), dtype=torch.float32, device=dev)
+        return ops.refiner_volume_kp(*args, mean_in, std)
+
     def run_volume_net(self, mean_in, std, sn):
         pk = self._pack()
-        dev = mean_in.device
-        batched = mean_in.dim() == 3
+        pairs_in = isinstance(mean_in, ops.PairMap)
+        dev = mean_in.data.device if pairs_in else mean_in.device
+        batched = pairs_in or mean_in.dim() == 3
         qn = mean_in.shape[0] if batched else 1
         pn = 1 if qn > 1 else 0
 
@@ -217,21 +243,50 @@
             return torch.empty((qn, s, s, s, c), dtype=torch.float32, device=dev)
 
         vox = sn ** 3
-        cat = buf(sn, 128)
-        def embed(name, x, sl):
+        rng = self._pair_rng() if pairs_in else None
+        cat16 = pairs_in and "conv0" in VOLUME_PAIR_LAYERS
+        cat = ops.new_map16(qn * sn, sn, sn, 128, 3, dev, rng=(rng, rng.slot("volume.cat"))) if cat16 else buf(sn, 128)
+
+        def c16(layer, xin, y, stats_c=None, count=vox):
+            st = ops.new_stats(qn, stats_c, dev) if stats_c else None
+            ops.conv16_direct_multi([xin], layer.w16(3, layout=2), layer[1], relu=False, full=torch.float32, kd=3, stats=st,
+                                    rows_per_group=count if stats_c else 0, out_full=[y])
+            return ops.stats_finalize(st, count) if stats_c else None
+
+        def embed(name, x, c_off):
+            if pairs_in:
+                return embed16(name, x, c_off)
             y = buf(sn, 64)
             aff = c3(x, pk[name][0], y, stats_c=64, count=vox)
-            c3(y, pk[name][1], cat[..., sl], aff=aff)
+            c3(y, pk[name][1], cat[..., c_off:c_off + 64], aff=aff)
+
+        def embed16(name, x, c_off):
+            y0 = buf(sn, 64)
+            sc, sh = c16(pk[name][0], x, y0, stats_c=64)
+            mid = ops.affine_split16(y0.view(qn * sn, 1, sn, sn, 64), sc, sh, sn, True, False, 3, rng=(rng, rng.slot(f"volume.{name[2:]}.mid")))
+            if not cat16:
+                c16(pk[name][1], mid.view(qn, sn, sn, sn, 2, 64), cat[..., c_off:c_off + 64])
+                return
+            y1 = buf(sn, 64)
+            c16(pk[name][1], mid.view(qn, sn, sn, sn, 2, 64), y1)
+            ops.affine_split16_to(y1.view(qn * sn, 1, sn, sn, 64), None, None, 0, False, 3, cat, c_off)
 
         with self._mm("embed"):
-            embed("v_mean_embed", mean_in.view(qn, sn, sn, sn, 256), slice(0, 64))
-            embed("v_var_embed", std.view(qn, sn, sn, sn, 128), slice(64, 128))
+            embed("v_mean_embed", mean_in.view(qn, sn, sn, sn, 2, 256) if pairs_in else mean_in.view(qn, sn, sn, sn, 256), 0)
+            embed("v_var_embed", std.view(qn, sn, sn, sn, 2, 128) if pairs_in else std.view(qn, sn, sn, sn, 128), 64)
         x, aff, s = cat, None, sn
         with self._mm("stack"):
             for name, co, stride in (("v_conv0", 64, 1), ("v_conv1", 128, 2), ("v_conv2", 128, 1), ("v_conv3", 256, 2),
                                      ("v_conv4", 256, 1)):
                 s = s // stride
                 y = buf(s, co)
+                if name == "v_conv0" and cat16:
+                    x, aff = y, c16(pk[name], cat.view(qn, sn, sn, sn, 2, 128), y, stats_c=co)
+                    continue
+                if name == "v_conv2" and pairs_in and "conv2" in VOLUME_PAIR_LAYERS:
+                    xin = ops.affine_split16(x.view(qn * s, 1, s, s, 128), aff[0], aff[1], s, True, False, 3, rng=(rng, rng.slot("volume.conv2.in")))
+                    x, aff = y, c16(pk[name], xin.view(qn, s, s, s, 2, 128), y, stats_c=co, count=s ** 3)
+                    continue
                 x, aff = y, c3(x, pk[name], y, stride=stride, aff=aff, stats_c=co, count=s ** 3)
         s = s // 2
         y = buf(s, 512)
@@ -269,16 +324,10 @@
         else:
             imgs = torch.cat([ref_imgs, que_img], 0)
         feats = self.run_feature_net(imgs)
-        lin = _linspace(sn, dev)
-        C = feats.shape[-1]
-        lead = (qn,) if batched else ()
-        mean_in = torch.empty(lead + (sn ** 3, 2 * C), dtype=torch.float32, device=dev)
-        std = torch.empty(lead + (sn ** 3, C), dtype=torch.float32, device=dev)
         feats = feats.contiguous()
         if batched:
             feats = feats.view(qn, rfn + 1, *feats.shape[1:])
-        ops.refiner_volume_kp(feats, ref_Ks.contiguous(), ref_poses.contiguous(), K_in.contiguous(), pose_in.contiguous(),
-                              lin, h_in, w_in, mean_in, std)
+        mean_in, std = self.feature_volumes(feats, ref_Ks, ref_poses, K_in, pose_in, h_in, w_in, sn)
         return self.run_regressor(self.run_volume_net(mean_in, std, sn))
 
     def _step_from_feats(self, que_img, K_in, pose_in, ref_feats, ref_Ks, ref_poses):
@@ -289,16 +338,9 @@
         qf = self.run_feature_net(que_img)
         if batched:
             feats = torch.cat([ref_feats, qf[:, None]], 1).contiguous()
-            lead = (ref_feats.shape[0],)
         else:
             feats = torch.cat([ref_feats, qf], 0).contiguous()
-            lead = ()
-        lin = _linspace(sn, dev)
-        C = feats.shape[-1]
-        mean_in = torch.empty(lead + (sn ** 3, 2 * C), dtype=torch.float32, device=dev)
-        std = torch.empty(lead + (sn ** 3, C), dtype=torch.float32, device=dev)
-        ops.refiner_volume_kp(feats, ref_Ks.contiguous(), ref_poses.contiguous(), K_in.contiguous(), pose_in.contiguous(),
-                              lin, h_in, w_in, mean_in, std)
+        mean_in, std = self.feature_volumes(feats, ref_Ks, ref_poses, K_in, pose_in, h_in, w_in, sn)
         return self.run_regressor(self.run_volume_net(mean_in, std, sn))
 
     def forward(self, data):
diff --git a/gen6d_amd/ops.py b/gen6d_amd/ops.py
--- a/gen6d_amd/ops.py
+++ b/gen6d_amd/ops.py
@@ -642,7 +642,19 @@
     return hi, (w - hi.double()).to(torch.float16), 1.0 / S
 
 
+def conv16_fold_depth(w_taps):
+    co, taps, ci = w_taps.shape
+    if taps != 27:
+        raise ValueError("conv16_fold_depth: [Cout, 27, Cin] expected")
+    return w_taps.reshape(co, 3, 9, ci).permute(0, 2, 1, 3).reshape(co, 9, 3 * ci).contiguous()
+
+
 def conv16_pack(w_taps, mode, layout=1):
+    if layout == 2:
+        if mode != 3 or w_taps.shape[1] != 27:
+            raise ValueError("conv16_pack: the depth-folded layout takes 27-tap filters in mode 3 (fp16 pairs)")
+        f = conv16_pack(conv16_fold_depth(w_taps), mode, layout=1)
+        return Conv16Filters(f.data, 2, mode, f.acc_scale, f.Cout, 27, w_taps.shape[2])
     co, taps, ci = w_taps.shape
     bk = 32 if mode == 3 else 64
     co_true = co
@@ -845,15 +857,15 @@
     return fulls, pools
 
 
-def conv16_direct_plan(N, H, W, Cin, Cout, mode, stats_rows=0, full=torch.float32):
+def conv16_direct_plan(N, H, W, Cin, Cout, mode, stats_rows=0, full=torch.float32, D=None):
     pair = mode == 3
     code = {None: 0, "t16": 3 if pair else 1, torch.float32: 2}[full]
     any_ = 1 << 12
     ldf = 2 * Cout if code == 3 else Cout
-    seg = (_lib.G6dConv16Seg * 1)(_lib.G6dConv16Seg(in_=any_, out_full=any_ if code else None, out_pool=None, N=N, D=1, H=H, W=W,
+    seg = (_lib.G6dConv16Seg * 1)(_lib.G6dConv16Seg(in_=any_, out_full=any_ if code else None, out_pool=None, N=N, D=D or 1, H=H, W=W,
                                                     ld_in=(2 if pair else 1) * Cin, ld_full=ldf if code else 0, ld_pool=0))
-    rc = _lib.load().g6d_conv16_direct_plan(seg, 1, Cin, C.c_void_p(any_), 1, Cout, 1, code, 0, int(mode), C.c_void_p(any_ if stats_rows else 0),
-                                            int(stats_rows))
+    rc = _lib.load().g6d_conv16_direct_plan(seg, 1, Cin, C.c_void_p(any_), 2 if D else 1, Cout, 3 if D else 1, code, 0, int(mode),
+                                            C.c_void_p(any_ if stats_rows else 0), int(stats_rows))
     return rc if rc >= 0 else None
 
 
@@ -1040,6 +1052,28 @@
     return mean_in, std
 
 
+def refiner_volume_kp_pairs(feats, ref_Ks, ref_poses, K_in, pose_in, lin, h_in, w_in, rng_mean=None, rng_std=None):
+    _need_gpu(feats, ref_Ks, ref_poses, K_in, pose_in, lin)
+    if feats.dim() != 5:
+        raise ValueError("refiner_volume_kp_pairs: batched operands expected")
+    B, V, fh, fw, Cc = feats.shape
+    sn = lin.numel()
+    for t in (feats, ref_Ks, ref_poses, K_in, pose_in, lin):
+        if not t.is_contiguous() or t.dtype != torch.float32:
+            raise ValueError("refiner_volume_kp_pairs: operands must be contiguous float32")
+    if (tuple(ref_Ks.shape) != (B, V - 1, 3, 3) or tuple(ref_poses.shape) != (B, V - 1, 3, 4) or tuple(K_in.shape) != (B, 3, 3) or
+            tuple(pose_in.shape) != (B, 3, 4)):
+        raise ValueError("refiner_volume_kp_pairs: shape mismatch")
+    mean_in = torch.empty((B, sn, sn, sn, 2, 2 * Cc), dtype=torch.float16, device=feats.device)
+    std = torch.empty((B, sn, sn, sn, 2, Cc), dtype=torch.float16, device=feats.device)
+    ra_m, ra_s = _range_arg(None, -1, rng_mean), _range_arg(None, -1, rng_std)
+    _timed_hbm("refiner_volume", 4.0 * B * (V * fh * fw * Cc + 3 * sn ** 3 * Cc),
+               lambda: _lib.check(_lib.load().g6d_refiner_volume_kp_pairs(
+                   _ptr(feats), _ptr(ref_Ks), _ptr(ref_poses), _ptr(K_in), _ptr(pose_in), _ptr(lin), V - 1, fh, fw, Cc, int(h_in), int(w_in), sn,
+                   _ptr(mean_in), _ptr(std), B, ra_m, ra_s, _stream()), "g6d_refiner_volume_kp_pairs"))
+    return _wrap(mean_in, rng_mean), _wrap(std, rng_std)
+
+
 def cat1(ts, dim=0):
     return ts[0] if len(ts) == 1 else torch.cat(ts, dim)
 
diff --git a/include/gen6d_hip.h b/include/gen6d_hip.h
--- a/include/gen6d_hip.h
+++ b/include/gen6d_hip.h
@@ -192,6 +192,9 @@
 int g6d_refiner_volume_kp(const float* feats, const float* ref_Ks, const float* ref_poses, const float* K_in, const float* pose_in,
                           const float* lin, int rfn, int fh, int fw, int C, int h_in, int w_in, int sn, float* mean_in, float* stdv,
                           int batch, g6d_stream_t stream);
+int g6d_refiner_volume_kp_pairs(const float* feats, const float* ref_Ks, const float* ref_poses, const float* K_in, const float* pose_in,
+                                const float* lin, int rfn, int fh, int fw, int C, int h_in, int w_in, int sn, void* mean_in16, void* std16,
+                                int batch, const G6dRange16* range_mean, const G6dRange16* range_std, g6d_stream_t stream);
 
 int g6d_detector_assemble(const float* s0, const float* s1, const float* s2, int hc, int wc, int rfn,
                           const float* mu_sigma , float clip, int hs, int ws,
```

Measured after the change: 358.8 (median of 6 runs). 1.06x the previous value.
